# zalo/TetSim

Measured on AMD Instinct MI355X. Metric: tet_solves_per_sec, higher is better.
Workload: dtype f32; 1 GPU; Kuhn-6 cube lattice 55x55x55 cells (998250 tets, 175616 particles), polar-decomposition Jacobi, 20 substeps/frame, dt=1/1200 s; solver=polar_jacobi, arithmetic=fast, formulation=reference (rest shape carried from substep to substep, 148 B/tet), tets=998250, particles=175616, parallelism=single GPU

## Files before the change

### include/tetsim.h

```cpp
#ifndef TETSIM_H
#define TETSIM_H

#include <stdint.h>

#ifdef __cplusplus
extern "C" {
#endif

#define TETSIM_ABI_VERSION 5

typedef struct tetsim_body *tetsim_handle;

enum {
    TETSIM_OK = 0,
    TETSIM_EINVAL = 1,
    TETSIM_ENODEVICE = 2,
    TETSIM_EHIP = 3,
    TETSIM_ENOMEM = 4,
    TETSIM_ECOMM = 5,
    TETSIM_ESTATE = 6
};

enum {
    TETSIM_SOLVER_POLAR_JACOBI = 0,
// ... 170 lines not shown
int tetsim_set_body_params_device(tetsim_handle h, const void *rows, uint64_t row_stride, const void *body_mask, void *caller_stream);


enum { TETSIM_FIELD_POSITIONS = 0, TETSIM_FIELD_VELOCITIES = 1, TETSIM_FIELD_PREV_POSITIONS = 2,
       TETSIM_FIELD_QUATS = 3, TETSIM_FIELD_VISUAL_POSITIONS = 4, TETSIM_FIELD_VISUAL_NORMALS = 5,
       TETSIM_FIELD_VISUAL_VERTEX_NORMALS = 6 };
#define TETSIM_MAX_EXPORT_FIELDS 8
typedef struct TetSimDeviceField {
    int32_t field, reserved;
    void *dst;
    uint64_t row_stride;
} TetSimDeviceField;
int tetsim_export_device(tetsim_handle h, const TetSimDeviceField *fields, uint32_t count, void *consumer_stream);
int tetsim_import_device(tetsim_handle h, const void *pos, uint64_t pos_stride,
                         const void *vel, uint64_t vel_stride, void *producer_stream);


typedef struct tetsim_snapshot_s *tetsim_snapshot;
int tetsim_snapshot_create(tetsim_handle h, tetsim_snapshot *out);
int tetsim_snapshot_capture(tetsim_handle h, tetsim_snapshot s, const void *body_mask, void *caller_stream);
int tetsim_snapshot_restore(tetsim_handle h, tetsim_snapshot s, const void *body_mask, void *caller_stream);
void tetsim_snapshot_destroy(tetsim_snapshot s);


#define TETSIM_PLACE_WIDTH 16
enum { TETSIM_PLACE_Q = 0 , TETSIM_PLACE_PIVOT = 4 , TETSIM_PLACE_OFFSET = 7 ,
       TETSIM_PLACE_LINEAR = 10 , TETSIM_PLACE_ANGULAR = 13  };
enum { TETSIM_PLACE_KEEP_VELOCITY = 1u << 0 };
int tetsim_place_bodies_device(tetsim_handle h, const void *rows, uint64_t row_stride,
                               const void *body_mask, uint32_t flags, void *caller_stream);
int tetsim_place_bodies(tetsim_handle h, const float *rows, const uint8_t *body_mask, uint32_t flags);


#define TETSIM_OBS_WIDTH 20
enum { TETSIM_OBS_MASS = 0, TETSIM_OBS_COM = 1 , TETSIM_OBS_VCOM = 4 , TETSIM_OBS_VOLUME = 7,
       TETSIM_OBS_REST_VOLUME = 8, TETSIM_OBS_MIN_VOLUME_RATIO = 9, TETSIM_OBS_INVERTED_TETS = 10,
       TETSIM_OBS_AABB_MIN = 11 , TETSIM_OBS_AABB_MAX = 14 , TETSIM_OBS_MAX_SPEED2 = 17,
       TETSIM_OBS_NONFINITE = 18, TETSIM_OBS_RESERVED = 19  };
int tetsim_observe_bodies_device(tetsim_handle h, void *dst, uint64_t row_stride, void *caller_stream);
int tetsim_read_body_observations(tetsim_handle h, double *out);


#define TETSIM_POSE_WIDTH 48
#define TETSIM_POSE_SWEEPS 5
enum { TETSIM_POSE_MASS = 0, TETSIM_POSE_MX = 1 , TETSIM_POSE_MV = 4 , TETSIM_POSE_A = 7 ,
       TETSIM_POSE_L0 = 16 , TETSIM_POSE_G = 19 , TETSIM_POSE_Q0 = 25,
       TETSIM_POSE_COM = 26 , TETSIM_POSE_VCOM = 29 , TETSIM_POSE_Q = 32 , TETSIM_POSE_OMEGA = 36 ,
       TETSIM_POSE_L = 39 , TETSIM_POSE_RESIDUAL = 42, TETSIM_POSE_GAP = 43, TETSIM_POSE_RESERVED = 44  };
int tetsim_body_poses_device(tetsim_handle h, void *dst, uint64_t row_stride, void *caller_stream);
int tetsim_read_body_poses(tetsim_handle h, double *out);
int tetsim_prep_pose_table(const float *verts, uint32_t nv, const int32_t *tets, uint32_t nt,
                           const uint32_t *body_first_vert, const uint32_t *body_first_tet, uint32_t num_bodies,
                           double density, void *records_out, double *centres_out);


#define TETSIM_TOUCH_WIDTH 100
#define TETSIM_TOUCH_SLOT_WIDTH 12
#define TETSIM_TOUCH_PARTICLE_WIDTH 8
enum { TETSIM_TOUCH_TOUCHING = 0, TETSIM_TOUCH_MIN_SD = 1, TETSIM_TOUCH_MIN_SLOT = 2, TETSIM_TOUCH_SLOTS = 3,
       TETSIM_TOUCH_SLOT0 = 4  };
enum { TETSIM_TOUCH_SLOT_KIND = 0, TETSIM_TOUCH_SLOT_COUNT = 1, TETSIM_TOUCH_SLOT_MIN_SD = 2, TETSIM_TOUCH_SLOT_CENTROID = 3 ,
       TETSIM_TOUCH_SLOT_NORMAL = 6 , TETSIM_TOUCH_SLOT_REL_VEL = 9  };
enum { TETSIM_TOUCH_P_SD = 0, TETSIM_TOUCH_P_NORMAL = 1 , TETSIM_TOUCH_P_SLOT = 4, TETSIM_TOUCH_P_TOUCHES = 5,
       TETSIM_TOUCH_P_RESERVED = 6  };
int tetsim_touch_bodies_device(tetsim_handle h, double margin, void *dst, uint64_t row_stride, void *caller_stream);
int tetsim_read_body_touch(tetsim_handle h, double margin, double *out);
int tetsim_touch_particles_device(tetsim_handle h, double margin, void *dst, uint64_t row_stride, void *caller_stream);


#define TETSIM_RAY_INVALID (-1)
int tetsim_raycast_visual_device(tetsim_handle h,
        const void *rays,     uint64_t ray_stride,
        const void *ray_body,
        uint32_t count,
        void *hits,           uint64_t hit_stride,
        void *caller_stream);
int tetsim_visual_bounding_spheres_device(tetsim_handle h, void *dst, uint64_t row_stride, void *caller_stream);


int tetsim_raycast_visual_bvh_device(tetsim_handle h,
        const void *rays,     uint64_t ray_stride,
        const void *ray_body,
        uint32_t count,
        void *hits,           uint64_t hit_stride,
        void *caller_stream);


typedef struct TetSimPointQuery { double point[3], max_distance; } TetSimPointQuery;
typedef struct TetSimClosest    { int32_t found, body, triangle, region;
                                  double distance, point[3], v, w; } TetSimClosest;
#define TETSIM_CLOSEST_INVALID (-1)
int tetsim_closest_visual_device(tetsim_handle h,
        const void *queries,  uint64_t query_stride,
        const void *query_body,
        uint32_t count,
        void *out,            uint64_t out_stride,
        void *caller_stream);
int tetsim_closest_visual(tetsim_handle h, const TetSimPointQuery *queries, const int32_t *query_body, uint32_t count, TetSimClosest *out);


#define TETSIM_STRAIN_WIDTH 16
#define TETSIM_STRAIN_BODY_WIDTH 8
#define TETSIM_STRAIN_SWEEPS 4
enum { TETSIM_STRAIN_F = 0 , TETSIM_STRAIN_J = 9, TETSIM_STRAIN_DEV = 10,
       TETSIM_STRAIN_STRETCH = 11 , TETSIM_STRAIN_GREEN = 14, TETSIM_STRAIN_RESERVED = 15  };
int tetsim_tet_strain_device(tetsim_handle h, void *dst, uint64_t row_stride, void *caller_stream);
int tetsim_read_tet_strain(tetsim_handle h, float *out);
int tetsim_body_strain_device(tetsim_handle h, void *dst, uint64_t row_stride, void *caller_stream);
int tetsim_visual_strain_device(tetsim_handle h, int32_t channel, void *dst, uint64_t row_stride, void *caller_stream);
int tetsim_prep_strain_table(const float *verts, uint32_t nv, const int32_t *tets, uint32_t nt, double density, void *records_out);


int tetsim_profile(tetsim_handle h, uint32_t n, double dt, const TetSimParams *params, TetSimProfile *out);
int tetsim_time_kernels(tetsim_handle h, uint32_t reps, double dt, const TetSimParams *params, TetSimProfile *out);
int tetsim_time_step_n(tetsim_handle h, uint32_t n, double dt, const TetSimParams *params, double *ms_out);
int tetsim_measure_copy_bandwidth(int32_t device, uint64_t bytes, uint32_t reps, double *gbps_out);
int tetsim_measure_stream_bandwidth(int32_t device, uint64_t bytes, uint32_t reps, int32_t kind, double *gbps_out);


int tetsim_comm_unique_id(void *id128);
int tetsim_comm_init(tetsim_handle h, const void *id128, int32_t rank, int32_t nranks);
typedef struct TetSimCommInfo {
    int32_t rccl_ranks, rccl_rank;
    uint32_t neighbours;
    uint64_t send_bytes_per_substep, recv_bytes_per_substep, max_message_bytes;
    int32_t loopback;
    int32_t p2p;
} TetSimCommInfo;
int tetsim_comm_info(tetsim_handle h, TetSimCommInfo *out);
int tetsim_comm_selftest(tetsim_handle h);
int tetsim_comm_probe(tetsim_handle h, uint64_t bytes, uint32_t reps, int32_t use_graph, uint32_t per_graph,
                      double *host_us, double *total_us);
int tetsim_halo_probe(tetsim_handle h, uint32_t reps, double *min_us, double *median_us, double *max_us);
#define TETSIM_P2P_BLOB_BYTES 512
int tetsim_halo_p2p_export(tetsim_handle h, void *blob);
int tetsim_halo_p2p_connect(tetsim_handle h, const void *blobs, uint32_t count);
int tetsim_halo_p2p_probe(tetsim_handle h, uint32_t reps, double *min_us, double *median_us, double *max_us);
int tetsim_group_step_n(tetsim_handle *handles, uint32_t count, uint32_t n, double dt, const TetSimParams *params);
int tetsim_halo_exchange_local(tetsim_handle *handles, uint32_t count);
int tetsim_get_halo_plan(tetsim_handle h, int32_t *neigh ,
                         int32_t *send_counts, int32_t *recv_counts,
                         int32_t *send_ids, int32_t *recv_ids);
int tetsim_halo_export(tetsim_handle h, uint32_t n, float *out_xyzw);
int tetsim_halo_import(tetsim_handle h, uint32_t n, const float *in_xyzw);


int tetsim_prep_levels(const int32_t *tets, uint32_t nt, uint32_t nv, int32_t *level, uint32_t *num_levels);
int tetsim_prep_colours(const int32_t *tets, uint32_t nt, uint32_t nv, int32_t *colour, uint32_t *num_colours);
int tetsim_prep_clusters(const int32_t *tets, uint32_t nt, uint32_t nv, int32_t *order, int32_t *launch, int32_t *lane,
                         int32_t *step, uint32_t *num_launches, uint32_t *num_clusters);
int tetsim_prep_tiles(const float *verts, uint32_t nv, const int32_t *tets, uint32_t nt, const uint32_t *body_first_tet,
                      const uint32_t *body_first_vert, uint32_t bodies, int32_t *tile_tets, uint32_t *tile_off,
                      uint8_t *corner_slot, uint32_t *num_tiles);
int tetsim_prep_bvh(const float *positions, uint32_t nvis, const int32_t *tri_ids, uint32_t ntri, const int32_t *tri_body, uint32_t bodies,
                    uint32_t *tri_first, uint32_t *order, uint32_t *node_first, uint32_t *depth, uint32_t *node_range);
int tetsim_prep_slot_table(const int32_t *tets, uint32_t nt, uint32_t nv, int32_t ref_quirk,
                           int32_t *slots , uint32_t *dropped);
int tetsim_prep_call_tiles(const float *verts, uint32_t nv, const int32_t *tets, uint32_t nt, uint32_t sizes[4],
                           uint32_t *blk_vert_off, int32_t *blk_verts, uint32_t *vp_ell);
int tetsim_prep_call_schedule(const int32_t *blk_verts, const uint32_t *blk_vert_off, uint32_t nb, const uint32_t *vp_ell,
                              uint32_t vp_cols, uint32_t nv_pad, uint32_t nv_owned, uint32_t lag, uint32_t *entry,
                              uint32_t capacity, uint32_t *period, uint32_t *tail, int32_t *fell_back);
int tetsim_prep_check_call_schedule(const int32_t *blk_verts, const uint32_t *blk_vert_off, uint32_t nb, const uint32_t *vp_ell,
                                    uint32_t vp_cols, uint32_t nv_pad, uint32_t nv_owned, const uint32_t *entry, uint32_t period,
                                    uint32_t tail);
int tetsim_prep_ref_grab_texels(int32_t grab_id, uint32_t num_elems, uint32_t num_particles, int32_t out[2]);
int tetsim_prep_boundary_surface(const float *verts ,
                                 const int32_t *tets, uint32_t nt, uint32_t nv,
                                 float *vis_verts , int32_t *tri_ids ,
                                 uint32_t *nrows, uint32_t *ntri);
int tetsim_prep_rest(const float *verts, uint32_t nv, const int32_t *tets, uint32_t nt, double density,
                     float *inv_mass, float *inv_rest_pose, float *inv_rest_volume);

int tetsim_prep_partition(const float *verts , uint32_t nv, const int32_t *tets, uint32_t nt,
                          int32_t part_count, int32_t *vert_owner_out);
typedef struct TetSimPartQuality {
    uint32_t owned_particles;
    uint32_t ghost_particles;
    uint32_t boundary_particles;
    uint32_t local_elems;
    uint32_t owned_elems;
    uint32_t num_neighbours;
} TetSimPartQuality;
int tetsim_prep_partition_quality(const int32_t *tets, uint32_t nt, uint32_t nv, int32_t part_count,
                                  const int32_t *vert_owner, TetSimPartQuality *out);

typedef struct tetsim_plan_s *tetsim_plan;
typedef struct TetSimPlanSizes {
    uint32_t owned_particles, boundary_particles, local_particles, local_elems, owned_elems, num_neighbours;
} TetSimPlanSizes;
int tetsim_plan_create(const int32_t *tets, uint32_t nt, uint32_t nv, int32_t part_count, int32_t part_index,
                       const int32_t *vert_owner, tetsim_plan *out);
int tetsim_plan_create_deep(const int32_t *tets, uint32_t nt, uint32_t nv, int32_t part_count, int32_t part_index,
                            const int32_t *vert_owner, int32_t depth, tetsim_plan *out);
int tetsim_plan_layers(tetsim_plan p, uint32_t *first_layer_ghosts, uint8_t *tet_layer);
int tetsim_plan_neighbour_layer2(tetsim_plan p, uint32_t i, uint32_t *send_count, uint32_t *recv_start, uint32_t *recv_count);
int tetsim_plan_neighbour_layer2_ids(tetsim_plan p, uint32_t i, int32_t *send_local, int32_t *send_global, int32_t *recv_global);
void tetsim_plan_destroy(tetsim_plan p);
int tetsim_plan_sizes(tetsim_plan p, TetSimPlanSizes *out);
int tetsim_plan_arrays(tetsim_plan p, int32_t *local_to_global_vert, int32_t *local_to_global_tet, int32_t *local_tets);
int tetsim_plan_neighbour(tetsim_plan p, uint32_t i, int32_t *rank, uint32_t *send_count, uint32_t *recv_start,
                          uint32_t *recv_count, int32_t *send_is_contiguous);
int tetsim_plan_neighbour_ids(tetsim_plan p, uint32_t i, int32_t *send_local, int32_t *send_global, int32_t *recv_global);

int tetsim_abi_version(void);
typedef struct TetSimLibraryInfo {
    int32_t abi;
    int32_t ablation;
    uint32_t debug_env;
    char source_sha[20];
    char kernel_sha[20];
} TetSimLibraryInfo;
int tetsim_library_info(TetSimLibraryInfo *out);

typedef struct TetSimMeshArrays {
    uint32_t num_particles;
    uint32_t num_elems;
    uint32_t num_edges;
    uint32_t num_vis_verts;
    uint32_t num_vis_tris;
    uint32_t part_count;
    const float *verts;
    const int32_t *tets;
    const int32_t *edge_ids;
    const float *vis_verts;
    const int32_t *vis_tri_ids;
    const int32_t *tet_colour;
    const int32_t *vert_owner;
} TetSimMeshArrays;
typedef struct tetsim_mesh_file *tetsim_mesh;

int tetsim_mesh_write(const char *path, const TetSimMeshArrays *a);
int tetsim_mesh_open(const char *path, tetsim_mesh *out);
int tetsim_mesh_arrays(tetsim_mesh m, TetSimMeshArrays *out);
int tetsim_mesh_close(tetsim_mesh m);
int tetsim_create_from_file(const char *path, const TetSimOptions *opts, tetsim_handle *out);

#ifdef __cplusplus
}
#endif
#endif
```

### tetsim_amd/_capi.py

```python
import ctypes as C
import os

_HERE = os.path.dirname(os.path.abspath(__file__))
LIB_PATH = os.environ.get("TETSIM_HIP_LIB") or os.path.join(_HERE, "libtetsim_hip.so")

OK, EINVAL, ENODEVICE, EHIP, ENOMEM, ECOMM, ESTATE = range(7)
RAY_INVALID = -1
CLOSEST_INVALID = -1
SOLVER_POLAR_JACOBI, SOLVER_NEOHOOKEAN_GS = 0, 1
PRECISE, FAST = 0, 1
ORDER_ORIGINAL, ORDER_COLOURED, ORDER_CLUSTERED = 0, 1, 2
FLAG_REF_SLOT_TABLE, FLAG_REF_FIXED_BOUNDS, FLAG_GATHER_FORMULATION, FLAG_CONSTANT_REST_SHAPE, FLAG_REF_GRAB_TEXEL, FLAG_DEEP_GHOSTS = 1, 2, 4, 8, 16, 32
FLAG_REF_ROTATION_EXIT = 64
FLAG_LEAN_STATE = 128
K_TET, K_VERTEX, K_HALO, K_COUNT = 0, 1, 2, 3
COLLIDER_SPHERE, COLLIDER_CAPSULE, COLLIDER_BOX, COLLIDER_PLANE = 0, 1, 2, 3
MAX_COLLIDERS = 8
BODY_COLLIDER_FLOATS = 24
BODY_PARAMS_WIDTH = 10
BP_GRAVITY, BP_FRICTION, BP_DEV_COMPLIANCE, BP_VOL_COMPLIANCE, BP_BOUNDS_LO, BP_BOUNDS_HI = 0, 1, 2, 3, 4, 7
FIELD_POSITIONS, FIELD_VELOCITIES, FIELD_PREV_POSITIONS, FIELD_QUATS, FIELD_VISUAL_POSITIONS, FIELD_VISUAL_NORMALS, FIELD_VISUAL_VERTEX_NORMALS = range(7)
MAX_EXPORT_FIELDS = 8
OBS_WIDTH = 20
(OBS_MASS, OBS_COM, OBS_VCOM, OBS_VOLUME, OBS_REST_VOLUME, OBS_MIN_VOLUME_RATIO, OBS_INVERTED_TETS, OBS_AABB_MIN, OBS_AABB_MAX, OBS_MAX_SPEED2,
 OBS_NONFINITE, OBS_RESERVED) = 0, 1, 4, 7, 8, 9, 10, 11, 14, 17, 18, 19
POSE_WIDTH, POSE_SWEEPS = 48, 5
(POSE_MASS, POSE_MX, POSE_MV, POSE_A, POSE_L0, POSE_G, POSE_Q0, POSE_COM, POSE_VCOM, POSE_Q, POSE_OMEGA, POSE_L, POSE_RESIDUAL, POSE_GAP,
 POSE_RESERVED) = 0, 1, 4, 7, 16, 19, 25, 26, 29, 32, 36, 39, 42, 43, 44
TOUCH_WIDTH, TOUCH_SLOT_WIDTH, TOUCH_PARTICLE_WIDTH = 100, 12, 8
TOUCH_TOUCHING, TOUCH_MIN_SD, TOUCH_MIN_SLOT, TOUCH_SLOTS, TOUCH_SLOT0 = 0, 1, 2, 3, 4
TOUCH_SLOT_KIND, TOUCH_SLOT_COUNT, TOUCH_SLOT_MIN_SD, TOUCH_SLOT_CENTROID, TOUCH_SLOT_NORMAL, TOUCH_SLOT_REL_VEL = 0, 1, 2, 3, 6, 9
TOUCH_P_SD, TOUCH_P_NORMAL, TOUCH_P_SLOT, TOUCH_P_TOUCHES, TOUCH_P_RESERVED = 0, 1, 4, 5, 6
STRAIN_WIDTH, STRAIN_BODY_WIDTH, STRAIN_SWEEPS = 16, 8, 4
STRAIN_F, STRAIN_J, STRAIN_DEV, STRAIN_STRETCH, STRAIN_GREEN, STRAIN_RESERVED = 0, 9, 10, 11, 14, 15
PLACE_WIDTH = 16
PLACE_Q, PLACE_PIVOT, PLACE_OFFSET, PLACE_LINEAR, PLACE_ANGULAR = 0, 4, 7, 10, 13
PLACE_KEEP_VELOCITY = 1


class TetSimParams(C.Structure):
    _fields_ = [("gravity", C.c_double), ("friction", C.c_double), ("devCompliance", C.c_double),
                ("volCompliance", C.c_double), ("worldBounds", C.c_double * 6)]


class TetSimOptions(C.Structure):
    _fields_ = [("solver", C.c_int32), ("precision", C.c_int32), ("order", C.c_int32), ("flags", C.c_uint32),
                ("device", C.c_int32), ("density", C.c_double), ("part_count", C.c_int32),
                ("part_index", C.c_int32), ("vert_owner", C.POINTER(C.c_int32)), ("tet_colour", C.POINTER(C.c_int32))]


class TetSimMeshArrays(C.Structure):
    _fields_ = [("num_particles", C.c_uint32), ("num_elems", C.c_uint32), ("num_edges", C.c_uint32),
                ("num_vis_verts", C.c_uint32), ("num_vis_tris", C.c_uint32), ("part_count", C.c_uint32),
                ("verts", C.POINTER(C.c_float)), ("tets", C.POINTER(C.c_int32)), ("edge_ids", C.POINTER(C.c_int32)),
                ("vis_verts", C.POINTER(C.c_float)), ("vis_tri_ids", C.POINTER(C.c_int32)),
                ("tet_colour", C.POINTER(C.c_int32)), ("vert_owner", C.POINTER(C.c_int32))]


class TetSimInfo(C.Structure):
    _fields_ = [("num_particles", C.c_uint32), ("num_elems", C.c_uint32), ("owned_particles", C.c_uint32),
                ("local_particles", C.c_uint32), ("local_elems", C.c_uint32), ("owned_elems", C.c_uint32),
                ("num_levels", C.c_uint32), ("max_valence", C.c_uint32), ("dropped_slots", C.c_uint32),
                ("num_neighbours", C.c_uint32), ("device_bytes", C.c_uint64), ("solver", C.c_int32),
                ("precision", C.c_int32), ("order", C.c_int32), ("device", C.c_int32), ("flags", C.c_uint32),
                ("num_vis_verts", C.c_uint32), ("num_bodies", C.c_uint32), ("fused_particle_pass", C.c_uint32), ("total_vis_verts", C.c_uint32)]


class TetSimProfile(C.Structure):
    _fields_ = [("total_ms", C.c_double), ("kernel_ms", C.c_double * K_COUNT), ("launches", C.c_uint32 * K_COUNT),
                ("substeps", C.c_uint32), ("tets_per_tet_launch", C.c_uint32)]


class TetSimLibraryInfo(C.Structure):
    _fields_ = [("abi", C.c_int32), ("ablation", C.c_int32), ("debug_env", C.c_uint32), ("source_sha", C.c_char * 20),
                ("kernel_sha", C.c_char * 20)]


DEBUG_ENV_NAMES = ["TETSIM_DEBUG_LOOPBACK_HALO", "TETSIM_DEBUG_LOOPBACK_COPY", "TETSIM_DEBUG_ONE_STREAM", "TETSIM_DEBUG_GROUP_SYNC",
                   "TETSIM_DEBUG_HOSTPROF", "TETSIM_DEBUG_TRACE", "TETSIM_HALO_SYNC", "TETSIM_HALO_GRAPH", "TETSIM_DEBUG_LOOPBACK_DELAY_US", "TETSIM_NH_QUADS", "TETSIM_FUSED_PARTICLE_PASS",
                   "TETSIM_FRAME_KERNEL", "TETSIM_FRAME_LOCAL", "TETSIM_NH_FOLD", "TETSIM_HALO_ALIGNED_TILES", "TETSIM_HALO_FOLD_WAIT", "TETSIM_QUAD", "TETSIM_QUAD_POLL_DELAY", "TETSIM_NH_FRAME",
                   "TETSIM_NH_ONE_LAUNCH", "TETSIM_PJ_ONE_LAUNCH", "TETSIM_PJ_CALL_LAG"]


LAB_ENV_NAMES = ["TETSIM_DEBUG_TRACE", "TETSIM_NH_QUADS", "TETSIM_FRAME_LOCAL", "TETSIM_NH_FOLD", "TETSIM_HALO_ALIGNED_TILES", "TETSIM_QUAD_POLL_DELAY", "TETSIM_NH_FRAME"]


class TetSimCommInfo(C.Structure):
    _fields_ = [("rccl_ranks", C.c_int32), ("rccl_rank", C.c_int32), ("neighbours", C.c_uint32), ("send_bytes_per_substep", C.c_uint64),
                ("recv_bytes_per_substep", C.c_uint64), ("max_message_bytes", C.c_uint64), ("loopback", C.c_int32), ("p2p", C.c_int32)]


class TetSimPlanSizes(C.Structure):
    _fields_ = [("owned_particles", C.c_uint32), ("boundary_particles", C.c_uint32), ("local_particles", C.c_uint32),
                ("local_elems", C.c_uint32), ("owned_elems", C.c_uint32), ("num_neighbours", C.c_uint32)]


class TetSimPartQuality(C.Structure):
    _fields_ = [("owned_particles", C.c_uint32), ("ghost_particles", C.c_uint32), ("boundary_particles", C.c_uint32),
                ("local_elems", C.c_uint32), ("owned_elems", C.c_uint32), ("num_neighbours", C.c_uint32)]


class TetSimError(RuntimeError):
    def __init__(self, code, msg):
        super().__init__("tetsim error %d: %s" % (code, msg))
        self.code = code


class TetSimCollider(C.Structure):
    _fields_ = [("kind", C.c_int32), ("reserved", C.c_int32), ("a", C.c_double * 3), ("b", C.c_double * 3), ("axes", C.c_double * 9),
                ("radius", C.c_double), ("friction", C.c_double), ("velocity", C.c_double * 3)]


class TetSimRay(C.Structure):
    _fields_ = [("origin", C.c_double * 3), ("direction", C.c_double * 3), ("near", C.c_double), ("far", C.c_double)]


class TetSimRayHit(C.Structure):
    _fields_ = [("hit", C.c_int32), ("body", C.c_int32), ("triangle", C.c_int32), ("reserved", C.c_int32), ("distance", C.c_double),
                ("point", C.c_double * 3)]


class TetSimPointQuery(C.Structure):
    _fields_ = [("point", C.c_double * 3), ("max_distance", C.c_double)]


class TetSimClosest(C.Structure):
    _fields_ = [("found", C.c_int32), ("body", C.c_int32), ("triangle", C.c_int32), ("region", C.c_int32), ("distance", C.c_double),
                ("point", C.c_double * 3), ("v", C.c_double), ("w", C.c_double)]


class TetSimDeviceField(C.Structure):
    _fields_ = [("field", C.c_int32), ("reserved", C.c_int32), ("dst", C.c_void_p), ("row_stride", C.c_uint64)]


SYMBOLS = [
    "tetsim_abi_version", "tetsim_default_options", "tetsim_default_params", "tetsim_create", "tetsim_create_batch", "tetsim_get_batch_layout", "tetsim_destroy",
    "tetsim_last_error", "tetsim_get_info", "tetsim_step", "tetsim_step_n", "tetsim_sync",
    "tetsim_library_info", "tetsim_read_quats_pinned", "tetsim_state_size", "tetsim_save_state", "tetsim_load_state",
    "tetsim_read_positions", "tetsim_read_positions_pinned", "tetsim_read_prev_positions", "tetsim_read_velocities", "tetsim_read_quats",
    "tetsim_read_vol_error", "tetsim_write_state", "tetsim_get_owned_ids", "tetsim_get_local_tets",
    "tetsim_get_tet_order", "tetsim_get_level_offsets", "tetsim_read_inv_mass", "tetsim_set_visual_mesh", "tetsim_get_visual_ids", "tetsim_halo_refresh_final", "tetsim_group_refresh_final", "tetsim_halo_probe", "tetsim_halo_p2p_probe",
    "tetsim_read_visual_mesh", "tetsim_set_visual_triangles", "tetsim_read_visual_vertex_normals", "tetsim_visual_vertex_normals_from", "tetsim_group_read_visual_vertex_normals", "tetsim_set_grab", "tetsim_set_colliders",
    "tetsim_start_grab", "tetsim_nearest_particle", "tetsim_profile", "tetsim_time_kernels", "tetsim_time_step_n", "tetsim_measure_copy_bandwidth", "tetsim_measure_stream_bandwidth",
    "tetsim_comm_unique_id", "tetsim_comm_init", "tetsim_comm_info", "tetsim_comm_selftest", "tetsim_comm_probe", "tetsim_group_step_n", "tetsim_halo_exchange_local", "tetsim_get_halo_plan",
    "tetsim_halo_p2p_export", "tetsim_halo_p2p_connect",
    "tetsim_halo_export", "tetsim_halo_import", "tetsim_prep_levels", "tetsim_prep_colours", "tetsim_prep_clusters",
    "tetsim_prep_tiles", "tetsim_prep_slot_table", "tetsim_prep_call_tiles", "tetsim_prep_call_schedule", "tetsim_prep_check_call_schedule", "tetsim_prep_ref_grab_texels", "tetsim_prep_rest", "tetsim_prep_partition", "tetsim_prep_partition_quality", "tetsim_plan_create", "tetsim_plan_destroy", "tetsim_plan_sizes",
    "tetsim_plan_arrays", "tetsim_plan_neighbour", "tetsim_plan_neighbour_ids",
    "tetsim_plan_create_deep", "tetsim_plan_layers", "tetsim_plan_neighbour_layer2", "tetsim_plan_neighbour_layer2_ids",
    "tetsim_raycast_visual", "tetsim_start_grab_ray", "tetsim_read_visual_bounding_sphere", "tetsim_prep_boundary_surface",
    "tetsim_export_device", "tetsim_import_device",
    "tetsim_snapshot_create", "tetsim_snapshot_capture", "tetsim_snapshot_restore", "tetsim_snapshot_destroy",
    "tetsim_observe_bodies_device", "tetsim_read_body_observations",
    "tetsim_body_poses_device", "tetsim_read_body_poses", "tetsim_prep_pose_table",
    "tetsim_touch_bodies_device", "tetsim_read_body_touch", "tetsim_touch_particles_device",
    "tetsim_raycast_visual_device", "tetsim_visual_bounding_spheres_device", "tetsim_raycast_visual_bvh_device", "tetsim_prep_bvh",
    "tetsim_closest_visual_device", "tetsim_closest_visual",
    "tetsim_tet_strain_device", "tetsim_read_tet_strain", "tetsim_body_strain_device", "tetsim_visual_strain_device", "tetsim_prep_strain_table",
    "tetsim_set_body_grabs", "tetsim_set_body_grabs_device", "tetsim_nearest_particles_device",
    "tetsim_set_body_colliders", "tetsim_set_body_colliders_device",
    "tetsim_set_body_params", "tetsim_set_body_params_device",
    "tetsim_place_bodies_device", "tetsim_place_bodies",
    "tetsim_mesh_write", "tetsim_mesh_open", "tetsim_mesh_arrays", "tetsim_mesh_close", "tetsim_create_from_file",
]

OPTIONAL_SYMBOLS = ("tetsim_set_colliders", "tetsim_raycast_visual", "tetsim_start_grab_ray", "tetsim_read_visual_bounding_sphere", "tetsim_prep_boundary_surface",
                    "tetsim_export_device", "tetsim_import_device",
                    "tetsim_snapshot_create", "tetsim_snapshot_capture", "tetsim_snapshot_restore", "tetsim_snapshot_destroy",
                    "tetsim_observe_bodies_device", "tetsim_read_body_observations",
                    "tetsim_raycast_visual_device", "tetsim_visual_bounding_spheres_device",
                    "tetsim_tet_strain_device", "tetsim_read_tet_strain", "tetsim_body_strain_device", "tetsim_visual_strain_device", "tetsim_prep_strain_table",
                    "tetsim_set_body_grabs", "tetsim_set_body_grabs_device", "tetsim_nearest_particles_device",
                    "tetsim_set_body_colliders", "tetsim_set_body_colliders_device",
                    "tetsim_set_body_params", "tetsim_set_body_params_device",
                    "tetsim_place_bodies_device", "tetsim_place_bodies",
                    "tetsim_body_poses_device", "tetsim_read_body_poses", "tetsim_prep_pose_table",
                    "tetsim_raycast_visual_bvh_device", "tetsim_prep_bvh",
                    "tetsim_closest_visual_device", "tetsim_closest_visual",
                    "tetsim_touch_bodies_device", "tetsim_read_body_touch", "tetsim_touch_particles_device")

_lib = None


def lib():
    global _lib
    if _lib is not None:
        return _lib
    if not os.path.exists(LIB_PATH):
        raise ImportError("libtetsim_hip.so is not built: run `python -m tetsim_amd.build` "
                          "(the HIP extension is mandatory; there is no CPU fallback)")
    L = C.CDLL(LIB_PATH)
    H, fp, ip, dp = C.c_void_p, C.POINTER(C.c_float), C.POINTER(C.c_int32), C.POINTER(C.c_double)
    u32, i32, dbl = C.c_uint32, C.c_int32, C.c_double
    PP = C.POINTER(TetSimParams)
    L.tetsim_abi_version.restype = C.c_int
    L.tetsim_default_options.argtypes = [C.POINTER(TetSimOptions)]
    L.tetsim_default_options.restype = None
    L.tetsim_default_params.argtypes = [PP]
    L.tetsim_default_params.restype = None
    L.tetsim_create.argtypes = [fp, u32, ip, u32, C.POINTER(TetSimOptions), C.POINTER(H)]
    L.tetsim_create_batch.argtypes = [C.POINTER(fp), C.POINTER(u32), C.POINTER(ip), C.POINTER(u32), u32, C.POINTER(TetSimOptions), C.POINTER(H)]
    L.tetsim_get_batch_layout.argtypes = [H, C.POINTER(u32), C.POINTER(u32)]
    L.tetsim_destroy.argtypes = [H]
    L.tetsim_destroy.restype = None
    L.tetsim_comm_probe.argtypes = [H, C.c_uint64, u32, i32, u32, dp, dp]
    L.tetsim_nearest_particle.argtypes = [H, fp, ip, dp]
    L.tetsim_mesh_write.argtypes = [C.c_char_p, C.POINTER(TetSimMeshArrays)]
    L.tetsim_mesh_open.argtypes = [C.c_char_p, C.POINTER(H)]
    L.tetsim_mesh_arrays.argtypes = [H, C.POINTER(TetSimMeshArrays)]
    L.tetsim_mesh_close.argtypes = [H]
    L.tetsim_create_from_file.argtypes = [C.c_char_p, C.POINTER(TetSimOptions), C.POINTER(H)]
    L.tetsim_last_error.argtypes = [H]
    L.tetsim_last_error.restype = C.c_char_p
    L.tetsim_get_info.argtypes = [H, C.POINTER(TetSimInfo)]
    L.tetsim_step.argtypes = [H, dbl, PP]
    L.tetsim_step_n.argtypes = [H, u32, dbl, PP]
    L.tetsim_sync.argtypes = [H]
    for n in ("positions", "prev_positions", "velocities", "quats", "inv_mass"):
        getattr(L, "tetsim_read_" + n).argtypes = [H, fp]
    L.tetsim_read_positions_pinned.argtypes = [H, C.POINTER(fp)]
    L.tetsim_read_quats_pinned.argtypes = [H, C.POINTER(fp)]
    L.tetsim_library_info.argtypes = [C.POINTER(TetSimLibraryInfo)]
    L.tetsim_state_size.argtypes = [H, C.POINTER(C.c_uint64)]
    L.tetsim_save_state.argtypes = [H, C.c_void_p, C.c_uint64]
    L.tetsim_load_state.argtypes = [H, C.c_void_p, C.c_uint64]
    L.tetsim_read_vol_error.argtypes = [H, dp]
    L.tetsim_write_state.argtypes = [H, fp, fp]
    for n in ("owned_ids", "local_tets", "tet_order", "level_offsets"):
        getattr(L, "tetsim_get_" + n).argtypes = [H, ip]
    L.tetsim_set_visual_mesh.argtypes = [H, fp, u32, fp]
    L.tetsim_read_visual_mesh.argtypes = [H, fp, fp]
    L.tetsim_get_visual_ids.argtypes = [H, C.POINTER(C.c_int32)]
    L.tetsim_halo_refresh_final.argtypes = [H]
    L.tetsim_halo_probe.argtypes = [H, u32, C.POINTER(C.c_double), C.POINTER(C.c_double), C.POINTER(C.c_double)]
    L.tetsim_halo_p2p_probe.argtypes = [H, u32, C.POINTER(C.c_double), C.POINTER(C.c_double), C.POINTER(C.c_double)]
    L.tetsim_group_refresh_final.argtypes = [C.POINTER(H), u32]
    L.tetsim_set_visual_triangles.argtypes = [H, ip, u32]
    L.tetsim_read_visual_vertex_normals.argtypes = [H, fp]
    L.tetsim_visual_vertex_normals_from.argtypes = [H, fp, fp]
    L.tetsim_group_read_visual_vertex_normals.argtypes = [C.POINTER(H), u32, fp, fp]
    L.tetsim_set_grab.argtypes = [H, i32, fp]
    if hasattr(L, "tetsim_set_colliders"):
        L.tetsim_set_colliders.argtypes = [H, C.POINTER(TetSimCollider), u32]
    L.tetsim_start_grab.argtypes = [H, fp, ip]
    if hasattr(L, "tetsim_raycast_visual"):
        L.tetsim_raycast_visual.argtypes = [H, C.c_void_p, u32, C.c_void_p]
        L.tetsim_start_grab_ray.argtypes = [H, C.POINTER(TetSimRay), C.POINTER(TetSimRayHit), ip]
        L.tetsim_read_visual_bounding_sphere.argtypes = [H, dp, dp]
        L.tetsim_prep_boundary_surface.argtypes = [fp, ip, u32, u32, fp, ip, C.POINTER(u32), C.POINTER(u32)]
    if hasattr(L, "tetsim_export_device"):
        L.tetsim_export_device.argtypes = [H, C.POINTER(TetSimDeviceField), u32, C.c_void_p]
        L.tetsim_import_device.argtypes = [H, C.c_void_p, C.c_uint64, C.c_void_p, C.c_uint64, C.c_void_p]
    if hasattr(L, "tetsim_snapshot_create"):
        L.tetsim_snapshot_create.argtypes = [H, C.POINTER(H)]
        L.tetsim_snapshot_capture.argtypes = [H, H, C.c_void_p, C.c_void_p]
        L.tetsim_snapshot_restore.argtypes = [H, H, C.c_void_p, C.c_void_p]
        L.tetsim_snapshot_destroy.argtypes = [H]
        L.tetsim_snapshot_destroy.restype = None
    if hasattr(L, "tetsim_observe_bodies_device"):
        L.tetsim_observe_bodies_device.argtypes = [H, C.c_void_p, C.c_uint64, C.c_void_p]
        L.tetsim_read_body_observations.argtypes = [H, dp]
    if hasattr(L, "tetsim_raycast_visual_device"):
        L.tetsim_raycast_visual_device.argtypes = [H, C.c_void_p, C.c_uint64, C.c_void_p, u32, C.c_void_p, C.c_uint64, C.c_void_p]
        L.tetsim_visual_bounding_spheres_device.argtypes = [H, C.c_void_p, C.c_uint64, C.c_void_p]
    if hasattr(L, "tetsim_raycast_visual_bvh_device"):
        L.tetsim_raycast_visual_bvh_device.argtypes = [H, C.c_void_p, C.c_uint64, C.c_void_p, u32, C.c_void_p, C.c_uint64, C.c_void_p]
        L.tetsim_prep_bvh.argtypes = [fp, u32, ip, u32, ip, u32] + [C.POINTER(u32)] * 5
    if hasattr(L, "tetsim_closest_visual_device"):
        L.tetsim_closest_visual_device.argtypes = [H, C.c_void_p, C.c_uint64, C.c_void_p, u32, C.c_void_p, C.c_uint64, C.c_void_p]
        L.tetsim_closest_visual.argtypes = [H, C.c_void_p, C.c_void_p, u32, C.c_void_p]
    if hasattr(L, "tetsim_tet_strain_device"):
        L.tetsim_tet_strain_device.argtypes = [H, C.c_void_p, C.c_uint64, C.c_void_p]
        L.tetsim_read_tet_strain.argtypes = [H, fp]
        L.tetsim_body_strain_device.argtypes = [H, C.c_void_p, C.c_uint64, C.c_void_p]
        L.tetsim_visual_strain_device.argtypes = [H, i32, C.c_void_p, C.c_uint64, C.c_void_p]
        L.tetsim_prep_strain_table.argtypes = [fp, u32, ip, u32, dbl, C.c_void_p]
    if hasattr(L, "tetsim_set_body_grabs"):
        L.tetsim_set_body_grabs.argtypes = [H, ip, fp]
        L.tetsim_set_body_grabs_device.argtypes = [H, C.c_void_p, C.c_void_p, C.c_uint64, C.c_void_p, C.c_void_p]
        L.tetsim_nearest_particles_device.argtypes = [H, C.c_void_p, C.c_uint64, C.c_void_p, C.c_void_p, C.c_void_p]
    if hasattr(L, "tetsim_set_body_colliders"):
        L.tetsim_set_body_colliders.argtypes = [H, fp, u32]
        L.tetsim_set_body_colliders_device.argtypes = [H, C.c_void_p, C.c_uint64, u32, C.c_void_p, C.c_void_p]
    if hasattr(L, "tetsim_set_body_params"):
        L.tetsim_set_body_params.argtypes = [H, C.POINTER(C.c_double)]
        L.tetsim_set_body_params_device.argtypes = [H, C.c_void_p, C.c_uint64, C.c_void_p, C.c_void_p]
    if hasattr(L, "tetsim_place_bodies_device"):
        L.tetsim_place_bodies_device.argtypes = [H, C.c_void_p, C.c_uint64, C.c_void_p, u32, C.c_void_p]
        L.tetsim_place_bodies.argtypes = [H, fp, C.POINTER(C.c_uint8), u32]
    if hasattr(L, "tetsim_body_poses_device"):
        L.tetsim_body_poses_device.argtypes = [H, C.c_void_p, C.c_uint64, C.c_void_p]
        L.tetsim_read_body_poses.argtypes = [H, dp]
        L.tetsim_prep_pose_table.argtypes = [fp, u32, ip, u32, C.POINTER(u32), C.POINTER(u32), u32, dbl, C.c_void_p, dp]
    if hasattr(L, "tetsim_touch_bodies_device"):
        L.tetsim_touch_bodies_device.argtypes = [H, dbl, C.c_void_p, C.c_uint64, C.c_void_p]
        L.tetsim_read_body_touch.argtypes = [H, dbl, dp]
        L.tetsim_touch_particles_device.argtypes = [H, dbl, C.c_void_p, C.c_uint64, C.c_void_p]
    L.tetsim_profile.argtypes = [H, u32, dbl, PP, C.POINTER(TetSimProfile)]
    L.tetsim_time_kernels.argtypes = [H, u32, dbl, PP, C.POINTER(TetSimProfile)]
    L.tetsim_time_step_n.argtypes = [H, u32, dbl, PP, dp]
    L.tetsim_measure_copy_bandwidth.argtypes = [i32, C.c_uint64, u32, dp]
    L.tetsim_measure_stream_bandwidth.argtypes = [i32, C.c_uint64, u32, i32, dp]
    L.tetsim_comm_unique_id.argtypes = [C.c_void_p]
    L.tetsim_comm_init.argtypes = [H, C.c_void_p, i32, i32]
    L.tetsim_comm_selftest.argtypes = [H]
    L.tetsim_comm_info.argtypes = [H, C.POINTER(TetSimCommInfo)]
    L.tetsim_group_step_n.argtypes = [C.POINTER(H), u32, u32, dbl, PP]
    L.tetsim_halo_exchange_local.argtypes = [C.POINTER(H), u32]
    L.tetsim_halo_p2p_export.argtypes = [H, C.c_void_p]
    L.tetsim_halo_p2p_connect.argtypes = [H, C.c_void_p, u32]
    L.tetsim_get_halo_plan.argtypes = [H, ip, ip, ip, ip, ip]
    L.tetsim_halo_export.argtypes = [H, u32, fp]
    L.tetsim_halo_import.argtypes = [H, u32, fp]
    L.tetsim_prep_levels.argtypes = [ip, u32, u32, ip, C.POINTER(u32)]
    L.tetsim_prep_colours.argtypes = [ip, u32, u32, ip, C.POINTER(u32)]
    L.tetsim_prep_clusters.argtypes = [ip, u32, u32, ip, ip, ip, ip, C.POINTER(u32), C.POINTER(u32)]
    L.tetsim_prep_tiles.argtypes = [fp, u32, ip, u32, C.POINTER(u32), C.POINTER(u32), u32, ip, C.POINTER(u32), C.POINTER(C.c_uint8), C.POINTER(u32)]
    L.tetsim_prep_slot_table.argtypes = [ip, u32, u32, i32, ip, C.POINTER(u32)]
    up = C.POINTER(u32)
    L.tetsim_prep_call_tiles.argtypes = [fp, u32, ip, u32, up, up, ip, up]
    L.tetsim_prep_call_schedule.argtypes = [ip, up, u32, up, u32, u32, u32, u32, up, u32, up, up, ip]
    L.tetsim_prep_check_call_schedule.argtypes = [ip, up, u32, up, u32, u32, u32, up, u32, u32]
    L.tetsim_prep_ref_grab_texels.argtypes = [i32, u32, u32, ip]
    L.tetsim_prep_rest.argtypes = [fp, u32, ip, u32, dbl, fp, fp, fp]
    L.tetsim_prep_partition.argtypes = [fp, u32, ip, u32, i32, ip]
    L.tetsim_prep_partition_quality.argtypes = [ip, u32, u32, i32, ip, C.POINTER(TetSimPartQuality)]
    L.tetsim_plan_create.argtypes = [ip, u32, u32, i32, i32, ip, C.POINTER(H)]
    L.tetsim_plan_destroy.argtypes = [H]
    L.tetsim_plan_destroy.restype = None
    L.tetsim_plan_sizes.argtypes = [H, C.POINTER(TetSimPlanSizes)]
    L.tetsim_plan_arrays.argtypes = [H, ip, ip, ip]
    L.tetsim_plan_neighbour.argtypes = [H, u32, ip, C.POINTER(u32), C.POINTER(u32), C.POINTER(u32), ip]
    L.tetsim_plan_neighbour_ids.argtypes = [H, u32, ip, ip, ip]
    L.tetsim_plan_create_deep.argtypes = [ip, u32, u32, i32, i32, ip, i32, C.POINTER(H)]
    L.tetsim_plan_layers.argtypes = [H, C.POINTER(u32), C.POINTER(C.c_uint8)]
    L.tetsim_plan_neighbour_layer2.argtypes = [H, u32, C.POINTER(u32), C.POINTER(u32), C.POINTER(u32)]
    L.tetsim_plan_neighbour_layer2_ids.argtypes = [H, u32, ip, ip, ip]
    for s in SYMBOLS:
        if s in OPTIONAL_SYMBOLS and not hasattr(L, s):
            continue
        f = getattr(L, s)
        if s not in ("tetsim_default_options", "tetsim_default_params", "tetsim_destroy", "tetsim_last_error",
                     "tetsim_plan_destroy", "tetsim_snapshot_destroy"):
            f.restype = C.c_int
    _lib = L
    return L


def library_info():
    li = TetSimLibraryInfo()
    check(lib().tetsim_library_info(C.byref(li)))
    return {"abi": li.abi, "ablation": bool(li.ablation), "source_sha": li.source_sha.decode(), "kernel_sha": li.kernel_sha.decode(),
            "debug_env": [n for i, n in enumerate(DEBUG_ENV_NAMES) if li.debug_env >> i & 1], "path": LIB_PATH}


def check(rc, handle=None):
    if rc != OK:
        msg = lib().tetsim_last_error(handle)
        raise TetSimError(rc, msg.decode("utf-8", "replace") if msg else "")
```

### tetsim_amd/csrc/dev_common.h

```cpp
#pragma once
#include <hip/hip_ext.h>
#include <hip/hip_runtime.h>

#include "host_prep.h"

#include <cstddef>
#include <cstdint>

namespace tetsim {

constexpr uint32_t kMaxColliders = 8;
struct DevColliderF {
    float a[3], b[3], u[9], radius, friction, v[3];
    int32_t kind, pad;
};
struct DevColliderD {
    double a[3], b[3], u[9], radius, friction, v[3];
    int32_t kind, pad;
};

__host__ __device__ inline float ref_fixed_lo(int c) { return c == 1 ? -1.0f : -2.5f; }
__host__ __device__ inline float ref_fixed_hi(int c) { return c == 1 ? 10.0f : 2.5f; }
struct BodyParamsF { float gravity, friction, dev_compliance, vol_compliance, lo[3], hi[3], pad[2]; };
struct BodyParamsD { double gravity, friction, dev_compliance, vol_compliance, lo[3], hi[3]; };
static_assert(sizeof(BodyParamsF) == 48 && sizeof(BodyParamsD) == 80, "body parameter rows");

struct DevParams {
    float dt, gravity, friction;
    uint32_t body_grabs;
    float lo[3];
    uint32_t body_colliders;
    float hi[3];
    uint32_t body_params;
    float grab[3];
    int32_t grab_local;
    int32_t grab_local2;
    uint32_t epoch;
    int32_t poll_delay;
    uint32_t n_colliders;
    double d_dt, d_gravity, d_friction, d_dev_compliance, d_vol_compliance;
    double d_lo[3], d_hi[3];
    const uint32_t* grab_body;
    const int4* grab_rows;
    const uint32_t* bcol_count;
    const DevColliderF* bcol_f;
    const DevColliderD* bcol_d;
    const BodyParamsF* bp_f;
    const BodyParamsD* bp_d;
    const uint32_t* tet_body;
    DevColliderF col[kMaxColliders];
    DevColliderD d_col[kMaxColliders];
};
constexpr size_t kDevParamsHead = offsetof(DevParams, col);
static_assert(kDevParamsHead % 8 == 0 && offsetof(DevParams, d_col) % 8 == 0, "DevParams layout");
constexpr size_t kKernelArgLimit = 4096;
static_assert(sizeof(DevParams) <= 2560, "DevParams must leave room for the other by-value arguments of a launch");
__device__ __forceinline__ void store_params(DevParams* dst, const DevParams& v) {
    const uint2* s = reinterpret_cast<const uint2*>(&v);
    uint2* d = reinterpret_cast<uint2*>(dst);
#pragma unroll
    for (size_t i = 0; i < kDevParamsHead / 8; i++) d[i] = s[i];
    for (uint32_t k = 0; k < v.n_colliders && k < kMaxColliders; k++) { dst->col[k] = v.col[k]; dst->d_col[k] = v.d_col[k]; }
}

__device__ __forceinline__ void body_grab_pick(const DevParams& P, uint32_t v, bool& held, float& x, float& y, float& z) {
    if (P.body_grabs) {
        const int4 row = P.grab_rows[P.grab_body[v]];
        held = row.x == static_cast<int32_t>(v);
        if (held) { x = __int_as_float(row.y); y = __int_as_float(row.z); z = __int_as_float(row.w); }
    }
}
__device__ __forceinline__ uint32_t body_colliders_body(const DevParams& P, uint32_t v) { return P.body_colliders ? P.grab_body[v] : 0u; }
__device__ __forceinline__ void body_colliders_pick(const DevParams& P, uint32_t body, const DevColliderF** list, uint32_t* count) {
    *list = P.col; *count = P.n_colliders;
    if (P.body_colliders) { *list = P.bcol_f + static_cast<size_t>(body) * kMaxColliders; *count = P.bcol_count[body]; }
}
__device__ __forceinline__ void body_colliders_pick(const DevParams& P, uint32_t body, const DevColliderD** list, uint32_t* count) {
    *list = P.d_col; *count = P.n_colliders;
    if (P.body_colliders) { *list = P.bcol_d + static_cast<size_t>(body) * kMaxColliders; *count = P.bcol_count[body]; }
}

__device__ __forceinline__ const BodyParamsF* body_params_row(const DevParams& P, uint32_t body, float) { return P.bp_f + body; }
__device__ __forceinline__ const BodyParamsD* body_params_row(const DevParams& P, uint32_t body, double) { return P.bp_d + body; }
__device__ __forceinline__ uint32_t body_params_uniform(uint32_t body) { return static_cast<uint32_t>(__builtin_amdgcn_readfirstlane(static_cast<int32_t>(body))); }
struct PolarBodyParams { float gravity, friction, lo[3], hi[3]; };
template <bool kUniform>
__device__ __forceinline__ PolarBodyParams body_params_polar(const DevParams& P, uint32_t v) {
    PolarBodyParams o = {P.gravity, P.friction, {P.lo[0], P.lo[1], P.lo[2]}, {P.hi[0], P.hi[1], P.hi[2]}};
    if (P.body_params) {
        uint32_t body = P.grab_body[v];
        if constexpr (kUniform) body = body_params_uniform(body);
        const BodyParamsF* const r = body_params_row(P, body, 0.0f);
        o.gravity = r->gravity; o.friction = r->friction;
        for (int k = 0; k < 3; k++) { o.lo[k] = r->lo[k]; o.hi[k] = r->hi[k]; }
    }
    return o;
}

struct PJDev {
    uint32_t nv_local = 0, nv_owned = 0, nv_boundary = 0, nt = 0;
    uint32_t nt_pad = 0;
    uint32_t nv_pad = 0;
    uint32_t max_valence = 0;
    float4* pos_pred = nullptr;
    float4* pos_final = nullptr;
    float4* vel = nullptr;
    int4* tet_idx = nullptr;
    float4* elem = nullptr;
    float4* quat = nullptr;
    int32_t* slot_tab = nullptr;
    uint32_t* slot_cnt = nullptr;
    const DevParams* params = nullptr;
    float rot_exit_w2 = 1.0e-18f;
};

struct PJBlk {
    uint32_t nb = 0, nb_interior = 0, nt = 0, nv_local = 0, nv_owned = 0, nv_boundary = 0;
    const uint32_t* blk_tet_off = nullptr;
    const uint32_t* blk_vert_off = nullptr;
    const int32_t* blk_verts = nullptr;
    const uchar4* tet_lidx = nullptr;
    float4* rest_a = nullptr;
    float4* rest_b = nullptr;
    float4* rest_c = nullptr;
    float* rest_c1 = nullptr;
    const float* vol = nullptr;
    float4* quat = nullptr;
    const uint32_t* lc_range = nullptr;
    const uint2* lc_ent = nullptr;
    float4* partial = nullptr;
    const float* wsum = nullptr;
    const uint32_t* vp_ell = nullptr;
    uint32_t vp_cols = 0, nv_pad = 0;
    float4* pos_pred = nullptr;
    float4* pos_final = nullptr;
    float4* vel = nullptr;
    const float4* partial_prev = nullptr;
    const float4* fin_in = nullptr;
    float4* fin_out = nullptr;
    const uint32_t* slot_src = nullptr;
    const uint32_t* blk_maxsrc = nullptr;
    uint32_t ns_pad = 0;
    const DevParams* params = nullptr;
    const float4* ghost_alt = nullptr;
    const float4* ghost2 = nullptr;
    uint32_t n_ghost1 = 0xffffffffu;
    bool lean = false;
    bool lean_state = false;
    float rot_exit_w2 = 1.0e-18f;
    uint32_t epoch = 0;
    unsigned long long* trace = nullptr;
    unsigned long long* iter_hist = nullptr;
};

struct NHDev {
    uint32_t nv = 0, nt = 0;
    float4* pos = nullptr;
    float4* prev = nullptr;
    float4* vel = nullptr;
    int4* tet_idx = nullptr;
    float4* irp_a = nullptr;
    float4* irp_b = nullptr;
    float4* irp_c = nullptr;
    double* vol_err = nullptr;
    int32_t* order = nullptr;
    uint32_t* corner_slots = nullptr;
    const DevParams* params = nullptr;
};
constexpr uint32_t max_grid_blocks(uint32_t threads) { return 0xffffffffu / threads; }
struct PJCallSched { const uint32_t* entry = nullptr; uint32_t period = 0, tail = 0; };
constexpr uint32_t pjb_call_chunk(uint32_t period, uint32_t tail, uint32_t threads, uint32_t cap) {
    const uint32_t room = max_grid_blocks(threads) > tail ? max_grid_blocks(threads) - tail : 0u;
    const uint32_t fit = period ? room / period : cap;
    return fit < 1u ? 1u : fit < cap ? fit : cap;
}
constexpr uint32_t nh_call_blocks_per_sub(uint32_t blocks) { return (blocks + 7u) & ~7u; }
constexpr uint32_t call_chunk(uint32_t per_sub, uint32_t threads, uint32_t cap) {
    const uint32_t fit = per_sub ? max_grid_blocks(threads) / per_sub : cap;
    return fit < 1u ? 1u : fit < cap ? fit : cap;
}
static_assert(pjb_call_chunk(pjb_call_blocks_per_sub(2282u, 103823u, 256u), 0u, 256u, 8192u) == 6223u, "46-cell lattice: 2,696 blocks per substep");
static_assert(pjb_call_chunk(pjb_call_blocks_per_sub(2282u, 103823u, 256u), 2696u, 256u, 8192u) == 6222u, "... and a tail of a whole period takes one substep's room");
static_assert(call_chunk(nh_call_blocks_per_sub(2601u), 256u, 65000u / 8u) == 6432u, "55-cell lattice, clustered: 2,608 blocks per substep");

constexpr uint32_t kNHClusterVerts = 8, kNHClusterTets = 8;
struct NHClusterLaunch {
    uint32_t nsteps = 0, clusters = 0;
    uint32_t first[kNHClusterTets] = {}, count[kNHClusterTets] = {};
    const int32_t* slot_vid = nullptr;
    const uint8_t* first_mask = nullptr;
};

struct NHSweepColour {
    NHClusterLaunch L;
    const float* slot_im = nullptr;
    const uint2* delta = nullptr;
    const uint8_t* last_mask = nullptr;
    const uint2* delta_first = nullptr;
    uint32_t first_block = 0;
    uint32_t pad = 0;
};
struct NHSweep {
    const NHSweepColour* colours = nullptr;
    uint32_t ncolours = 0, blocks = 0;
    float4* exchange = nullptr;
    uint32_t* error = nullptr;
    uint32_t timeout_ms = 0;
};
void nh_launch_sweep1_fast(hipStream_t s, const NHDev& d, const NHSweep& w, bool fold, uint32_t sub_index, uint32_t epoch);
void nh_launch_call_fast(hipStream_t s, const NHDev& d, const NHSweep& w, uint32_t n);

void pj_launch_tet_precise(hipStream_t s, const PJDev& d, hipEvent_t e0 = nullptr, hipEvent_t e1 = nullptr);
void pj_launch_tet_fast(hipStream_t s, const PJDev& d, hipEvent_t e0 = nullptr, hipEvent_t e1 = nullptr);
void pj_launch_vertex_precise(hipStream_t s, const PJDev& d, uint32_t first, uint32_t count, hipEvent_t e0 = nullptr, hipEvent_t e1 = nullptr);
void pj_launch_vertex_fast(hipStream_t s, const PJDev& d, uint32_t first, uint32_t count, hipEvent_t e0 = nullptr, hipEvent_t e1 = nullptr);
void pj_launch_repredict_precise(hipStream_t s, const PJDev& d);
void pj_launch_repredict_fast(hipStream_t s, const PJDev& d);

void nh_launch_post_predict_precise(hipStream_t s, const NHDev& d);
void nh_launch_post_predict_fast(hipStream_t s, const NHDev& d);
void nh_launch_cluster_precise(hipStream_t s, const NHDev& d, const NHClusterLaunch& L, bool fold = false);
void nh_launch_cluster_fast(hipStream_t s, const NHDev& d, const NHClusterLaunch& L, bool fold = false);
struct NHFrameLaunch {
    const uint32_t* seg = nullptr;
    const uint32_t* first_vert = nullptr;
    uint32_t levels = 0, bodies = 0, block = 512;
    uint32_t max_body_particles = 0;
};
void nh_launch_frame_precise(hipStream_t s, const NHDev& d, const NHFrameLaunch& f, uint32_t n, const DevParams& params, DevParams* params_dev);
void nh_launch_frame_fast(hipStream_t s, const NHDev& d, const NHFrameLaunch& f, uint32_t n, const DevParams& params, DevParams* params_dev);
constexpr uint32_t kNHQuadLevelFast = 128, kNHQuadLevelPrecise = 64;
void nh_launch_level4_fast(hipStream_t s, const NHDev& d, uint32_t first, uint32_t count);
void nh_launch_level4_precise(hipStream_t s, const NHDev& d, uint32_t first, uint32_t count);
uint32_t nh_frame_lds_limit_precise();
uint32_t nh_frame_lds_limit_fast();
void nh_launch_post_predict_list_precise(hipStream_t s, const NHDev& d, const uint32_t* list, uint32_t n);
void nh_launch_post_predict_list_fast(hipStream_t s, const NHDev& d, const uint32_t* list, uint32_t n);
void pjb_launch_tet(hipStream_t s, const PJBlk& d, uint32_t tile_first, uint32_t tile_count, hipEvent_t e0 = nullptr,
                    hipEvent_t e1 = nullptr, uint32_t* raise_word = nullptr, uint32_t* clear_word = nullptr);
void pjb_launch_call(hipStream_t s, const PJBlk& d, const PJCallSched& sched, uint32_t n, uint32_t* err, uint32_t timeout_ms, const DevParams& params, DevParams* params_dev);
void pjb_launch_tet_fused(hipStream_t s, const PJBlk& d, hipEvent_t e0 = nullptr, hipEvent_t e1 = nullptr);
void pjb_launch_vertex(hipStream_t s, const PJBlk& d, uint32_t first, uint32_t count, hipEvent_t e0 = nullptr, hipEvent_t e1 = nullptr,
                       uint32_t* raise_word = nullptr, uint32_t* clear_word = nullptr);
void pjb_launch_repredict(hipStream_t s, const PJBlk& d);
void pjb_launch_recover_quats(hipStream_t s, const PJBlk& d, const float4* rest0_a, const float4* rest0_b, const float4* rest0_c);
void pjb_launch_frame(hipStream_t s, const PJBlk& d, uint32_t n, const int32_t* block_tile, uint32_t blocks, bool local, float4* pbuf0, float4* pbuf1,
                      uint32_t* err, uint32_t timeout_ms, const DevParams& params, DevParams* params_dev, hipEvent_t e0 = nullptr, hipEvent_t e1 = nullptr);
void pjq_launch_frame(hipStream_t s, const PJBlk& d, uint32_t n, const int32_t* block_tile, uint32_t blocks, bool local, float4* pbuf0, float4* pbuf1,
                      uint32_t* err, uint32_t timeout_ms, const DevParams& params, DevParams* params_dev, hipEvent_t e0 = nullptr, hipEvent_t e1 = nullptr);
void pjq_launch_tet(hipStream_t s, const PJBlk& d, hipEvent_t e0 = nullptr, hipEvent_t e1 = nullptr);
void pjq_launch_vertex(hipStream_t s, const PJBlk& d, hipEvent_t e0 = nullptr, hipEvent_t e1 = nullptr);
uint32_t pjq_frame_capacity(uint32_t* compute_units);
uint32_t pjb_frame_capacity(int mode, uint32_t* compute_units);
void pjb_wait_capacity(int mode, uint32_t* vertex_waves, uint32_t* hwait_blocks);
inline int pjb_mode(const PJBlk& d) { return d.lean ? 1 : d.lean_state ? 2 : 0; }
uint32_t pjb_probe_xcd(hipStream_t s, uint32_t blocks);
struct PJSync {
    uint32_t* flag = nullptr;
    uint32_t* error = nullptr;
    uint32_t timeout_ms = 0;
};
constexpr uint32_t kMaxPeers = 8;
struct PJPeer {
    float4* ghost[kMaxPeers] = {};
    const uint32_t* slots = nullptr;
    uint32_t cols = 0, stride = 0, n = 0;
    float4* fin[kMaxPeers] = {};
    float4* ghost2[kMaxPeers] = {};
    const uint32_t* slots2 = nullptr;
    uint32_t cols2 = 0;
};
struct PJPeerSync {
    uint32_t* raise[kMaxPeers] = {};
    uint32_t* wait[kMaxPeers] = {};
    uint32_t n_raise = 0, n_wait = 0;
    uint32_t delay_us = 0;
};
void pjb_launch_wait(hipStream_t s, const PJSync& y);
void pjb_launch_wait_peers(hipStream_t s, const PJSync& y, const PJPeerSync& w);
struct PJClear { uint32_t* word[kMaxPeers + 1] = {}; uint32_t n = 0; };
void pjb_launch_vertex_peer(hipStream_t s, const PJBlk& d, uint32_t first, uint32_t count, const PJPeer& peer, uint32_t* raise_word, const PJClear& clr = PJClear());
void pjb_launch_tet_hwait(hipStream_t s, const PJBlk& d, uint32_t tile_first, uint32_t tile_count, const PJSync& yv, const PJPeerSync& w, const float4* ghosts);
// ... 66 lines not shown
```

### tetsim_amd/csrc/host_prep.cpp

```cpp
#include "host_prep.h"

#include <algorithm>
#include <cmath>
#include <numeric>

namespace tetsim {

namespace {
inline float fround(double x) { return static_cast<float>(x); }

inline void edge_matrix(const float* verts, const int32_t* t, float m[9]) {
    for (int k = 0; k < 3; k++)
        for (int c = 0; c < 3; c++)
            m[3 * k + c] = fround(static_cast<double>(verts[3 * t[k + 1] + c]) - static_cast<double>(verts[3 * t[0] + c]));
}
inline double det3(const float* A) {
    double a11 = A[0], a12 = A[3], a13 = A[6];
    double a21 = A[1], a22 = A[4], a23 = A[7];
    double a31 = A[2], a32 = A[5], a33 = A[8];
    return a11 * a22 * a33 + a12 * a23 * a31 + a13 * a21 * a32 - a13 * a22 * a31 - a12 * a21 * a33 - a11 * a23 * a32;
}
}

void prep_rest(const float* verts, uint32_t nv, const int32_t* tets, uint32_t nt, double density,
// ... 237 lines not shown
            kept++;
        }
    inc.dropped = static_cast<uint32_t>(4ull * nt - kept);
    return inc;
}

uint32_t prep_slot_table(const int32_t* tets, uint32_t nt, uint32_t nv, bool ref_quirk, int32_t* slots) {
    std::fill(slots, slots + static_cast<size_t>(nv) * kRefSlots, -1);
    uint32_t dropped = 0;
    for (uint32_t e = 0; e < nt; e++)
        for (int k = 0; k < 4; k++) {
            int32_t* row = &slots[static_cast<size_t>(tets[4 * e + k]) * kRefSlots];
            bool placed = false;
            for (int s = 0; s < kRefSlots; s++) {
                const bool empty = ref_quirk ? (row[s] <= 0) : (row[s] < 0);
                if (empty) {
                    if (row[s] == 0) dropped++;
                    row[s] = static_cast<int32_t>(4 * e + k);
                    placed = true;
                    break;
                }
            }
            if (!placed) dropped++;
        }
    return dropped;
}

namespace {
inline uint32_t spread3(uint32_t x) {
    x &= 0x3ffu;
    x = (x | (x << 16)) & 0x030000ffu;
    x = (x | (x << 8)) & 0x0300f00fu;
    x = (x | (x << 4)) & 0x030c30c3u;
    x = (x | (x << 2)) & 0x09249249u;
    return x;
}
}

namespace {
struct Quantiser {
    float lo[3], inv;
    Quantiser(const float* xyz, uint32_t n) {
        float hi[3] = {-1e30f, -1e30f, -1e30f};
        lo[0] = lo[1] = lo[2] = 1e30f;
        for (uint32_t v = 0; v < n; v++)
            for (int c = 0; c < 3; c++) { lo[c] = std::min(lo[c], xyz[3 * v + c]); hi[c] = std::max(hi[c], xyz[3 * v + c]); }
        float ext = 1e-30f;
        for (int c = 0; c < 3; c++) ext = std::max(ext, hi[c] - lo[c]);
        inv = 1024.0f / ext;
    }
    uint32_t code(float x, float y, float z) const {
        const float p[3] = {x, y, z};
        uint32_t c = 0;
        for (int a = 0; a < 3; a++) {
            const uint32_t qv = static_cast<uint32_t>(std::min(1023.0f, std::max(0.0f, (p[a] - lo[a]) * inv)));
            c |= spread3(qv) << a;
        }
        return c;
    }
};
}

std::vector<uint32_t> morton_vertex_order(const float* xyz, uint32_t n, uint32_t first, uint32_t count) {
    std::vector<uint32_t> order(n);
    std::iota(order.begin(), order.end(), 0u);
    if (count < 2) return order;
    const Quantiser Q(xyz, n);
    std::vector<uint64_t> key(count);
    for (uint32_t i = 0; i < count; i++) {
        const uint32_t v = first + i;
        key[i] = (static_cast<uint64_t>(Q.code(xyz[3 * v], xyz[3 * v + 1], xyz[3 * v + 2])) << 32) | v;
    }
    std::sort(key.begin(), key.end());
    for (uint32_t i = 0; i < count; i++) order[first + i] = static_cast<uint32_t>(key[i] & 0xffffffffu);
    return order;
}

void build_blocks(const float* verts, const int32_t* tets, uint32_t nt, uint32_t nv, uint32_t nv_sum,
                  const Incidence& inc, BlockPlan* out, const uint32_t* body_first_tet, const uint32_t* body_first_vert, uint32_t bodies,
                  uint32_t nv_boundary, const uint8_t* tet_class, uint32_t nv_owned, uint32_t tile) {
    BlockPlan& B = *out;
    B = BlockPlan();
    B.tile = tile;
    if (nv_owned > nv_sum) nv_owned = nv_sum;
    const uint32_t kMaxTets = tile, kMaxVerts = tile;
    const uint32_t one_t[2] = {0u, nt}, one_v[2] = {0u, nv};
    if (!body_first_tet || !body_first_vert || bodies == 0) { body_first_tet = one_t; body_first_vert = one_v; bodies = 1; }
    std::vector<uint64_t> key(nt);
    std::vector<uint32_t> body_of_pos(nt);
    B.tet_perm.resize(nt);
    for (uint32_t b = 0; b < bodies; b++) {
        const uint32_t tb = body_first_tet[b], te = body_first_tet[b + 1], vb = body_first_vert[b], ve = body_first_vert[b + 1];
        const Quantiser Q(verts + 3ull * vb, ve - vb);
        for (uint32_t e = tb; e < te; e++) {
            float m[3] = {0.0f, 0.0f, 0.0f};
            for (int k = 0; k < 4; k++)
                for (int c = 0; c < 3; c++) m[c] += verts[3 * tets[4 * e + k] + c];
            key[e] = (static_cast<uint64_t>(Q.code(0.25f * m[0], 0.25f * m[1], 0.25f * m[2])) << 32) | (e - tb);
            if (tet_class) key[e] |= static_cast<uint64_t>(tet_class[e] & 3u) << 62;
        }
        std::sort(key.begin() + tb, key.begin() + te);
        for (uint32_t i = tb; i < te; i++) { B.tet_perm[i] = static_cast<int32_t>(tb + (key[i] & 0xffffffffu)); body_of_pos[i] = b; }
    }

    std::vector<uint8_t> live(4ull * nt, 0);
    for (int32_t enc : inc.slot) live[enc] = 1;

    std::vector<int32_t> slot_of(nv, -1);
    std::vector<int32_t> touched;
    struct Run { uint32_t begin, end; bool ghost; uint8_t cls; };
    auto cls_of = [&](uint32_t sorted_pos) -> uint8_t { return tet_class ? tet_class[B.tet_perm[sorted_pos]] : 0; };
    std::vector<Run> runs;
    {
        uint32_t i = 0;
        while (i < nt) {
            const uint32_t t0 = i;
            touched.clear();
            bool ghost = false;
            while (i < nt && i - t0 < kMaxTets && body_of_pos[i] == body_of_pos[t0] && cls_of(i) == cls_of(t0)) {
                const int32_t* t = &tets[4 * B.tet_perm[i]];
                uint32_t fresh = 0;
                for (int k = 0; k < 4; k++) {
                    bool seen = slot_of[t[k]] >= 0;
                    for (int j = 0; j < k && !seen; j++) seen = t[j] == t[k];
                    if (!seen) fresh++;
                }
                if (touched.size() + fresh > kMaxVerts) break;
                for (int k = 0; k < 4; k++)
                    if (slot_of[t[k]] < 0) {
                        slot_of[t[k]] = 0; touched.push_back(t[k]);
                        ghost |= static_cast<uint32_t>(t[k]) >= nv_owned || static_cast<uint32_t>(t[k]) < nv_boundary;
                    }
                i++;
            }
            for (int32_t v : touched) slot_of[v] = -1;
            runs.push_back({t0, i, ghost, cls_of(t0)});
        }
    }
    std::stable_sort(runs.begin(), runs.end(), [](const Run& a, const Run& b) { return a.cls != b.cls ? a.cls < b.cls : a.ghost < b.ghost; });
    {
        std::vector<int32_t> perm2(nt);
        uint32_t o = 0;
        for (Run& r : runs) {
            std::copy(B.tet_perm.begin() + r.begin, B.tet_perm.begin() + r.end, perm2.begin() + o);
            const uint32_t len = r.end - r.begin;
            r.begin = o; r.end = o + len;
            o += len;
        }
        B.tet_perm.swap(perm2);
    }

    B.tet_lidx.resize(4ull * nt);
    B.lc_ent.resize(4ull * nt);
    B.blk_tet_off.push_back(0);
    B.blk_vert_off.push_back(0);
    std::vector<std::vector<uint32_t>> vert_partials(nv_sum);
    std::vector<std::vector<uint32_t>> vert_staged(nv_sum);
    for (const Run& r : runs) {
        const uint32_t t0 = r.begin, i = r.end;
        if (!r.ghost && r.cls == 0) B.num_interior_blocks++;
        if (r.cls <= 1) B.num_first_blocks++;
        touched.clear();
        for (uint32_t j = t0; j < i; j++)
            for (int k = 0; k < 4; k++) {
                const int32_t v = tets[4 * B.tet_perm[j] + k];
                if (slot_of[v] < 0) { slot_of[v] = 0; touched.push_back(v); }
            }
        std::sort(touched.begin(), touched.end());
        for (size_t u = 0; u < touched.size(); u++) slot_of[touched[u]] = static_cast<int32_t>(u);
        for (uint32_t j = t0; j < i; j++)
            for (int k = 0; k < 4; k++) B.tet_lidx[4ull * j + k] = static_cast<uint8_t>(slot_of[tets[4 * B.tet_perm[j] + k]]);
        const uint32_t ntb = i - t0, nu = static_cast<uint32_t>(touched.size());
        const uint32_t v0 = B.blk_vert_off.back();
        std::vector<uint32_t> cnt(nu + 1, 0);
        for (uint32_t j = 0; j < ntb; j++)
            for (int k = 0; k < 4; k++)
                if (live[4ull * B.tet_perm[t0 + j] + k]) cnt[B.tet_lidx[4ull * (t0 + j) + k] + 1]++;
        for (uint32_t u = 0; u < nu; u++) cnt[u + 1] += cnt[u];
        for (uint32_t u = 0; u < nu; u++) B.lc_range.push_back(cnt[u] | (cnt[u + 1] << 16));
        std::vector<uint32_t> fillp(cnt.begin(), cnt.end() - 1);
        for (uint32_t j = 0; j < ntb; j++)
            for (int k = 0; k < 4; k++)
                if (live[4ull * B.tet_perm[t0 + j] + k]) {
                    const uint32_t u = B.tet_lidx[4ull * (t0 + j) + k];
                    B.lc_ent[4ull * t0 + fillp[u]++] = static_cast<uint16_t>(kMaxTets * k + j);
                }
        for (uint32_t u = 0; u < nu; u++) {
            const int32_t v = touched[u];
            B.blk_verts.push_back(v);
            if (static_cast<uint32_t>(v) < nv_sum && cnt[u + 1] > cnt[u]) vert_partials[v].push_back(v0 + u);
            else if (static_cast<uint32_t>(v) < nv_sum) vert_staged[v].push_back(v0 + u);
            slot_of[v] = -1;
        }
        B.blk_tet_off.push_back(i);
        B.blk_vert_off.push_back(v0 + nu);
        B.max_tile_verts = std::max(B.max_tile_verts, nu);
    }
    B.num_blocks = static_cast<uint32_t>(B.blk_tet_off.size() - 1);
    B.vp_off.assign(nv_sum + 1, 0);
    for (uint32_t v = 0; v < nv_sum; v++) {
        B.vp_off[v + 1] = B.vp_off[v] + static_cast<uint32_t>(vert_partials[v].size());
        B.max_partials = std::max<uint32_t>(B.max_partials, static_cast<uint32_t>(vert_partials[v].size()));
    }
    B.vp_idx.reserve(B.vp_off[nv_sum]);
    for (uint32_t v = 0; v < nv_sum; v++) B.vp_idx.insert(B.vp_idx.end(), vert_partials[v].begin(), vert_partials[v].end());
    B.nv_pad = (nv_sum + 63u) & ~63u;
    B.vp_cols = 0;
    for (uint32_t v = 0; v < nv_sum; v++) B.vp_cols = std::max<uint32_t>(B.vp_cols, static_cast<uint32_t>(vert_partials[v].size() + vert_staged[v].size()));
    B.vp_ell.assign(static_cast<size_t>(std::max(B.vp_cols, 1u)) * B.nv_pad, 0xffffffffu);
    for (uint32_t v = 0; v < nv_sum; v++) {
        const size_t live = vert_partials[v].size();
        for (size_t j = 0; j < live; j++) B.vp_ell[j * B.nv_pad + v] = vert_partials[v][j];
        for (size_t j = 0; j < vert_staged[v].size(); j++) B.vp_ell[(live + j) * B.nv_pad + v] = vert_staged[v][j];
    }
    const uint32_t ns = static_cast<uint32_t>(B.blk_verts.size());
    B.ns_pad = (ns + 63u) & ~63u;
    B.slot_src.assign(static_cast<size_t>(std::max(B.max_partials, 1u)) * B.ns_pad, 0xffffffffu);
    B.blk_maxsrc.assign(B.num_blocks, 0);
    for (uint32_t v = 0; v < nv_sum; v++)
        if (vert_partials[v].empty()) B.every_owned_particle_has_a_partial = false;
    for (uint32_t b = 0; b < B.num_blocks; b++)
        for (uint32_t g = B.blk_vert_off[b]; g < B.blk_vert_off[b + 1]; g++) {
            const uint32_t v = static_cast<uint32_t>(B.blk_verts[g]);
            if (v >= nv_sum) continue;
            const std::vector<uint32_t>& list = vert_partials[v];
            for (size_t j = 0; j < list.size(); j++) B.slot_src[j * B.ns_pad + g] = list[j];
            B.blk_maxsrc[b] = std::max<uint32_t>(B.blk_maxsrc[b], static_cast<uint32_t>(list.size()));
            if (!list.empty() && list[0] == g) B.lc_range[g] |= 1u << 15;
        }
}

namespace {
struct SchedDeps {
    uint32_t per_xcd = 0, tet_blocks = 0, npb = 0, plain_period = 0;
    std::vector<std::vector<uint32_t>> tiles_of_pb, pbs_of_tile;
};
SchedDeps sched_deps(const int32_t* blk_verts, const uint32_t* blk_vert_off, uint32_t nb, const uint32_t* vp_ell, uint32_t vp_cols, uint32_t nv_pad,
                     uint32_t nv_owned, uint32_t tile) {
    SchedDeps D;
    D.per_xcd = (nb + 7u) / 8u; D.tet_blocks = D.per_xcd * 8u; D.npb = (nv_owned + tile - 1u) / tile;
    D.plain_period = pjb_call_blocks_per_sub(nb, nv_owned, tile);
    D.tiles_of_pb.resize(D.npb); D.pbs_of_tile.resize(nb);
    for (uint32_t v = 0; v < nv_owned; v++)
        for (uint32_t j = 0; j < vp_cols; j++) {
            const uint32_t idx = vp_ell[static_cast<size_t>(j) * nv_pad + v];
            if (idx == 0xffffffffu) continue;
            const uint32_t b = static_cast<uint32_t>(std::upper_bound(blk_vert_off, blk_vert_off + nb + 1, idx) - blk_vert_off) - 1u;
            if (b < nb) D.tiles_of_pb[v / tile].push_back(b);
        }
    for (uint32_t b = 0; b < nb; b++)
        for (uint32_t g = blk_vert_off[b]; g < blk_vert_off[b + 1]; g++)
            if (static_cast<uint32_t>(blk_verts[g]) < nv_owned) D.pbs_of_tile[b].push_back(static_cast<uint32_t>(blk_verts[g]) / tile);
    auto uniq = [](std::vector<uint32_t>& v) { std::sort(v.begin(), v.end()); v.erase(std::unique(v.begin(), v.end()), v.end()); };
    for (auto& v : D.tiles_of_pb) uniq(v);
    for (auto& v : D.pbs_of_tile) uniq(v);
    return D;
}
inline uint32_t sched_tile_of(uint32_t r, uint32_t per_xcd) { return (r & 7u) * per_xcd + (r >> 3); }
void sched_plain(const SchedDeps& D, uint32_t nb, CallSchedule* out) {
    out->period = D.plain_period;
    out->tail = 0; out->lag = 0;
    out->entry.assign(out->period, sched_entry(kSchedEmpty, 0));
    for (uint32_t r = 0; r < D.tet_blocks; r++)
        if (sched_tile_of(r, D.per_xcd) < nb) out->entry[r] = sched_entry(kSchedTile, r);
    for (uint32_t k = 0; k < D.npb; k++) out->entry[D.tet_blocks + k] = sched_entry(kSchedParticles, k);
}
struct SchedPass { std::vector<uint32_t> entry, ready, left; uint32_t head_end = 0; bool stuck = false; };
SchedPass sched_pass(const SchedDeps& D, uint32_t nb, uint32_t lag, const std::vector<uint32_t>& head_at) {
    constexpr uint32_t none = 0xffffffffu;
    SchedPass R;
    R.ready.assign(D.npb, none);
    std::vector<uint32_t> need(D.npb), head, queue;
    std::vector<uint8_t> head_placed(D.npb, 0);
    for (uint32_t k = 0; k < D.npb; k++) {
        need[k] = static_cast<uint32_t>(D.tiles_of_pb[k].size());
        if (head_at[k] != none) head.push_back(k);
        if (need[k] == 0) { R.ready[k] = 0; if (head_at[k] == none) queue.push_back(k); }
    }
    std::stable_sort(head.begin(), head.end(), [&](uint32_t a, uint32_t b) { return head_at[a] < head_at[b]; });
    std::vector<std::vector<uint32_t>> pbs_by_tile(nb);
    for (uint32_t k = 0; k < D.npb; k++) for (uint32_t b : D.tiles_of_pb[k]) pbs_by_tile[b].push_back(k);
    size_t hi = 0, qi = 0;
    uint32_t col_next[8] = {}, tiles_left = D.tet_blocks;
    const uint64_t limit = 4ull * (D.tet_blocks + D.npb) + 64ull * (static_cast<uint64_t>(lag) + 1ull) + 64ull;
    for (uint32_t p = 0;; p++) {
        if (tiles_left == 0 && hi == head.size() && (p & 7u) == 0u) break;
        if (p >= limit) { R.stuck = true; break; }
        const uint32_t x = p & 7u;
        if (hi < head.size() && head_at[head[hi]] <= p) {
            const uint32_t k = head[hi++];
            R.entry.push_back(sched_entry(kSchedParticles, k, true));
            head_placed[k] = 1; R.head_end = p + 1u;
            continue;
        }
        if (qi < queue.size() && R.ready[queue[qi]] <= p) { R.entry.push_back(sched_entry(kSchedParticles, queue[qi++])); continue; }
        if (col_next[x] < D.per_xcd) {
            const uint32_t r = 8u * col_next[x] + x, b = sched_tile_of(r, D.per_xcd);
            bool held = false;
            if (b < nb) for (uint32_t k : D.pbs_of_tile[b]) held = held || (head_at[k] != none && !head_placed[k]);
            if (!held) {
                col_next[x]++; tiles_left--;
                R.entry.push_back(b < nb ? sched_entry(kSchedTile, r) : sched_entry(kSchedEmpty, 0));
                if (b < nb) for (uint32_t k : pbs_by_tile[b])
                    if (--need[k] == 0) { R.ready[k] = p + 8u * lag; if (head_at[k] == none) queue.push_back(k); }
                continue;
            }
        }
        R.entry.push_back(sched_entry(kSchedEmpty, 0));
    }
    R.left.assign(queue.begin() + static_cast<std::ptrdiff_t>(qi), queue.end());
    return R;
}
}

std::string check_call_schedule(const int32_t* blk_verts, const uint32_t* blk_vert_off, uint32_t nb, const uint32_t* vp_ell, uint32_t vp_cols,
                                uint32_t nv_pad, uint32_t nv_owned, const uint32_t* entry, uint32_t period, uint32_t tail, uint32_t tile) {
    constexpr uint32_t none = 0xffffffffu;
    const SchedDeps D = sched_deps(blk_verts, blk_vert_off, nb, vp_ell, vp_cols, nv_pad, nv_owned, tile);
    if (period == 0 || period % 8u != 0u) return "the period is not a positive multiple of 8";
    if (period < D.plain_period) return "the period is shorter than a substep's blocks";
    std::vector<uint64_t> at_tile(nb, none), at_pb(D.npb, none);
    uint32_t col_seen[8] = {}, wrapped_end = 0;
    for (uint32_t p = 0; p < period; p++) {
        const uint32_t kind = entry[p] >> 30, index = entry[p] & kSchedIndexMask;
        const bool wrapped = (entry[p] & kSchedWrapped) != 0u;
        if (kind == kSchedEmpty) continue;
        if (kind == kSchedTile) {
            const uint32_t b = sched_tile_of(index, D.per_xcd);
            if (index >= D.tet_blocks || b >= nb) return "entry " + std::to_string(p) + " names a tile that does not exist";
            if ((index & 7u) != (p & 7u)) return "tile block " + std::to_string(index) + " is not on its XCD";
            if (wrapped) return "tile block " + std::to_string(index) + " is wrapped";
            if ((index >> 3) < col_seen[p & 7u]) return "tile block " + std::to_string(index) + " is out of its XCD's order";
            col_seen[p & 7u] = (index >> 3) + 1u;
            if (at_tile[b] != none) return "tile " + std::to_string(b) + " appears twice";
            at_tile[b] = p;
        } else if (kind == kSchedParticles) {
            if (index >= D.npb) return "entry " + std::to_string(p) + " names a particle block that does not exist";
            if (at_pb[index] != none) return "particle block " + std::to_string(index) + " appears twice";
            at_pb[index] = static_cast<uint64_t>(p) + (wrapped ? period : 0u);
            if (wrapped) wrapped_end = p + 1u;
        } else return "entry " + std::to_string(p) + " has no kind";
    }
    for (uint32_t b = 0; b < nb; b++) if (at_tile[b] == none) return "tile " + std::to_string(b) + " is missing";
    for (uint32_t k = 0; k < D.npb; k++) if (at_pb[k] == none) return "particle block " + std::to_string(k) + " is missing";
    if (tail < wrapped_end || tail > period) return "the tail does not cover the wrapped entries";
    for (uint32_t k = 0; k < D.npb; k++)
        for (uint32_t b : D.tiles_of_pb[k])
            if (!(at_tile[b] < at_pb[k])) return "particle block " + std::to_string(k) + " does not follow tile " + std::to_string(b) + " of its lists";
    for (uint32_t b = 0; b < nb; b++)
        for (uint32_t k : D.pbs_of_tile[b])
            if (!(at_pb[k] < at_tile[b] + period)) return "tile " + std::to_string(b) + " of the next substep does not follow particle block " + std::to_string(k);
    return "";
}

void build_call_schedule(const int32_t* blk_verts, const uint32_t* blk_vert_off, uint32_t nb, const uint32_t* vp_ell, uint32_t vp_cols,
                         uint32_t nv_pad, uint32_t nv_owned, uint32_t lag, CallSchedule* out, uint32_t tile) {
    constexpr uint32_t none = 0xffffffffu;
    const SchedDeps D = sched_deps(blk_verts, blk_vert_off, nb, vp_ell, vp_cols, nv_pad, nv_owned, tile);
    *out = CallSchedule();
    auto plain = [&](const std::string& why) {
        sched_plain(D, nb, out);
        out->fell_back = !why.empty(); out->why = why;
    };
    if (lag == 0 || nb == 0) return plain("");
    if (static_cast<uint64_t>(lag) * 8u >= D.plain_period) return plain("lag " + std::to_string(lag) + ": a whole substep or more");
    std::vector<uint32_t> head_at(D.npb, none);
    SchedPass R;
    bool settled = false;
    for (int pass = 0; pass < 64 && !settled; pass++) {
        R = sched_pass(D, nb, lag, head_at);
        if (R.stuck) return plain("lag " + std::to_string(lag) + ": the layout does not close");
        const uint32_t period = static_cast<uint32_t>(R.entry.size());
        settled = R.left.empty();
        for (uint32_t k : R.left) head_at[k] = 0;
        for (uint32_t k = 0; k < D.npb; k++)
            if (head_at[k] != none && !settled) head_at[k] = R.ready[k] != none && R.ready[k] > period ? R.ready[k] - period : 0u;
    }
    if (!settled) return plain("lag " + std::to_string(lag) + ": the wrapped blocks do not settle");
    out->entry = R.entry;
    out->period = static_cast<uint32_t>(R.entry.size());
    out->tail = R.head_end;
// ... 138 lines not shown
```

### tetsim_amd/csrc/host_prep.h

```cpp
#pragma once
#include <cstdint>
#include <string>
#include <vector>

namespace tetsim {

constexpr int kRefSlots = 36;

void prep_rest(const float* verts, uint32_t nv, const int32_t* tets, uint32_t nt, double density,
               float* inv_mass, float* inv_rest_pose, float* inv_rest_volume);

float pj_inv_rest_volume(const float* verts, const int32_t* tet);

uint32_t prep_levels(const int32_t* tets, uint32_t nt, uint32_t nv, int32_t* level);
uint32_t prep_colours(const int32_t* tets, uint32_t nt, uint32_t nv, int32_t* colour);
constexpr uint32_t kClusterTets = 8, kClusterVerts = 8;
struct ClusterPlan {
    std::vector<int32_t> pre;
    std::vector<uint32_t> exec_pos;
    std::vector<uint32_t> corner_slots;
    std::vector<uint32_t> launch_off;
    std::vector<uint32_t> step_off;
    std::vector<uint32_t> step_first, step_count;
    std::vector<uint32_t> vid_off;
    std::vector<int32_t> slot_vid;
    uint32_t num_clusters = 0;
};
ClusterPlan prep_clusters(const int32_t* tets, uint32_t nt, uint32_t nv);
uint32_t prep_slot_table(const int32_t* tets, uint32_t nt, uint32_t nv, bool ref_quirk, int32_t* slots);

struct Incidence {
    std::vector<uint32_t> offset;
    std::vector<int32_t> slot;
    uint32_t max_valence = 0;
    uint32_t dropped = 0;
};
Incidence build_incidence(const int32_t* tets, uint32_t nt, uint32_t nv, bool ref_quirk, bool ref_cap);

struct Partition {
    uint32_t nv_global = 0, nt_global = 0;
    int part_count = 1, part_index = 0;
    std::vector<int32_t> local_to_global_vert;
    uint32_t n_owned = 0, n_boundary = 0;
    std::vector<int32_t> local_to_global_tet;
    std::vector<int32_t> local_tets;
    uint32_t owned_tets = 0;
    struct Neighbour {
        int rank;
        std::vector<int32_t> send_local;
        std::vector<int32_t> send_global;
        uint32_t recv_start = 0, recv_count = 0;
        std::vector<int32_t> recv_global;
        bool send_contiguous = false;
        std::vector<int32_t> send2_local, send2_global;
        uint32_t recv2_start = 0, recv2_count = 0;
        std::vector<int32_t> recv2_global;
    };
    std::vector<Neighbour> neigh;
    int depth = 1;
    uint32_t n_ghost1 = 0;
    std::vector<uint8_t> tet_layer;
};
std::string prep_partition(const float* verts, uint32_t nv, const int32_t* tets, uint32_t nt, int parts, int32_t* out_owner);
struct PartQuality {
    uint32_t owned_particles = 0, ghost_particles = 0, boundary_particles = 0;
    uint32_t local_elems = 0, owned_elems = 0;
    uint32_t num_neighbours = 0;
};
std::string partition_quality(const int32_t* tets, uint32_t nt, uint32_t nv, int parts, const int32_t* owner, PartQuality* out);
std::string build_partition(const int32_t* tets, uint32_t nt, uint32_t nv, int part_count, int part_index,
                            const int32_t* vert_owner, Partition* out, int depth = 1);

std::vector<uint32_t> morton_vertex_order(const float* xyz, uint32_t n, uint32_t first, uint32_t count);

#ifndef TETSIM_TILE
#define TETSIM_TILE 256
#endif
constexpr uint32_t kBlockTile = TETSIM_TILE;
constexpr uint32_t kQuadTile = 64;
constexpr int32_t kQuadPollDelay = 0;
constexpr uint32_t kQuadMaxPartials = 12;
struct BlockPlan {
    uint32_t num_blocks = 0;
    uint32_t tile = kBlockTile;
    std::vector<int32_t> tet_perm;
    std::vector<uint32_t> blk_tet_off;
    std::vector<uint32_t> blk_vert_off;
    std::vector<int32_t> blk_verts;
    std::vector<uint8_t> tet_lidx;
    std::vector<uint32_t> lc_range;
    std::vector<uint16_t> lc_ent;
    std::vector<uint32_t> vp_off;
    std::vector<uint32_t> vp_idx;
    std::vector<uint32_t> vp_ell;
    uint32_t vp_cols = 0;
    std::vector<uint32_t> slot_src;
    std::vector<uint32_t> blk_maxsrc;
    uint32_t ns_pad = 0;
    bool every_owned_particle_has_a_partial = true;
    uint32_t nv_pad = 0;
    uint32_t max_tile_verts = 0, max_partials = 0;
    uint32_t num_interior_blocks = 0;
    uint32_t num_first_blocks = 0;
};
void build_blocks(const float* verts, const int32_t* tets, uint32_t nt, uint32_t nv, uint32_t nv_sum,
                  const Incidence& inc, BlockPlan* out, const uint32_t* body_first_tet = nullptr,
                  const uint32_t* body_first_vert = nullptr, uint32_t bodies = 1, uint32_t nv_boundary = 0,
                  const uint8_t* tet_class = nullptr, uint32_t nv_owned = 0xffffffffu, uint32_t tile = kBlockTile);

constexpr uint32_t kSchedTile = 0u, kSchedParticles = 1u, kSchedEmpty = 2u, kSchedWrapped = 1u << 29, kSchedIndexMask = (1u << 29) - 1u;
constexpr uint32_t sched_entry(uint32_t kind, uint32_t index, bool wrapped = false) { return kind << 30 | (wrapped ? kSchedWrapped : 0u) | index; }
constexpr uint32_t pjb_call_blocks_per_sub(uint32_t nb, uint32_t nv_owned, uint32_t threads) {
    return (((nb + 7u) & ~7u) + (nv_owned + threads - 1u) / threads + 7u) & ~7u;
}
constexpr uint32_t kPJCallLagDefault = 0;
struct CallSchedule {
    std::vector<uint32_t> entry;
    uint32_t period = 0, tail = 0;
    uint32_t lag = 0;
    bool fell_back = false;
    std::string why;
};
void build_call_schedule(const int32_t* blk_verts, const uint32_t* blk_vert_off, uint32_t nb, const uint32_t* vp_ell, uint32_t vp_cols,
                         uint32_t nv_pad, uint32_t nv_owned, uint32_t lag, CallSchedule* out, uint32_t tile = kBlockTile);
std::string check_call_schedule(const int32_t* blk_verts, const uint32_t* blk_vert_off, uint32_t nb, const uint32_t* vp_ell, uint32_t vp_cols,
                                uint32_t nv_pad, uint32_t nv_owned, const uint32_t* entry, uint32_t period, uint32_t tail, uint32_t tile = kBlockTile);

std::string validate_mesh(const float* verts, uint32_t nv, const int32_t* tets, uint32_t nt, bool forbid_repeats);

}
```

### tetsim_amd/csrc/pj_blocked.hip

```cpp
#define TETSIM_FAST 1
#include <cstdio>
#include <algorithm>
#include <cstdlib>
#include <type_traits>
#include <vector>

#include "collide.h"
#include "dev_common.h"
#include "dev_store.h"
#include "host_prep.h"
#include "pj_lab.h"

namespace tetsim {
namespace {

#include "pj_math.inc"
#include "pj_blocked_lab.inc"


__device__ __forceinline__ uint32_t xcd_tile(uint32_t b, uint32_t tiles_per_xcd) { return (b & 7u) * tiles_per_xcd + (b >> 3); }

struct VertexOut { f3 p, vel, pred; };
template <bool kUniformBody, bool kTable = true>
__device__ __forceinline__ VertexOut pjb_vertex_update(f3 acc, float wsum, f3 prev, const DevParams& P, uint32_t v) {
    const float rw = __builtin_amdgcn_rcpf(wsum);
    f3 p = F3(acc.x * rw, acc.y * rw, acc.z * rw);
    bool grabbed = static_cast<int32_t>(v) == P.grab_local || static_cast<int32_t>(v) == P.grab_local2;
    if (grabbed) p = F3(P.grab[0], P.grab[1], P.grab[2]);
    body_grab_pick(P, v, grabbed, p.x, p.y, p.z);
    PolarBodyParams B = {P.gravity, P.friction, {P.lo[0], P.lo[1], P.lo[2]}, {P.hi[0], P.hi[1], P.hi[2]}};
    if constexpr (kTable) B = body_params_polar<kUniformBody>(P, v);
    p.x = fminf(fmaxf(p.x, B.lo[0]), B.hi[0]);
    p.y = fminf(fmaxf(p.y, B.lo[1]), B.hi[1]);
    p.z = fminf(fmaxf(p.z, B.lo[2]), B.hi[2]);
    if (p.y < 0.0f) {
        p.y = 0.0f;
        const float Fx = prev.x - p.x, Fz = prev.z - p.z;
        const float fr = fminf(1.0f, P.dt * B.friction);
        p.x = fmaf(Fx, fr, p.x);
        p.z = fmaf(Fz, fr, p.z);
    }
    if (any_colliders(P)) collide_particle_f32<true>(p.x, p.y, p.z, prev.x, prev.y, prev.z, P, v, !grabbed);
    const float dt = P.dt;
    const float rdt = __builtin_amdgcn_rcpf(dt);
    VertexOut o;
    o.p = p;
    const float gx = dt * 0.0f, gy = dt * B.gravity, gz = dt * 0.0f;
    o.vel = F3(fmaf(rdt, p.x - prev.x, gx), fmaf(rdt, p.y - prev.y, gy), fmaf(rdt, p.z - prev.z, gz));
    o.pred = F3(fmaf(dt, o.vel.x, p.x), fmaf(dt, o.vel.y, p.y), fmaf(dt, o.vel.z, p.z));
    return o;
}

constexpr uint32_t kTile = kBlockTile;

__device__ __forceinline__ f3 lean_fourth_corner(const f3 r[4]) {
    return F3(-((r[0].x + r[1].x) + r[2].x), -((r[0].y + r[1].y) + r[2].y), -((r[0].z + r[1].z) + r[2].z));
}
struct PJHaloWait { const PJPeerSync* w; const uint32_t* vflag; uint32_t* error; uint32_t timeout_ms; const float4* ghosts; };
constexpr int kModeCarried = 0, kModeConstantRest = 1, kModeLeanState = 2;
inline int blk_mode(const PJBlk& d) { return pjb_mode(d); }
struct PJPoll { uint32_t block, want; uint32_t* error; uint32_t timeout_ms; };
template <int kMode, bool kFused, bool kAlt = false, bool kHaloWait = false, bool kPoll = false>
__device__ __forceinline__ void pjb_tet_body(const PJBlk& d, uint32_t tile_first, uint32_t tile_count, uint32_t tiles_per_xcd TETSIM_DBG_PARAM,
                                             [[maybe_unused]] const PJHaloWait* hw = nullptr, const uint32_t stamp = 0u, [[maybe_unused]] const PJPoll* poll = nullptr) {
    __shared__ float4 s_pos[kTile];
    __shared__ float s_gx[4 * kTile];
    __shared__ float s_gy[4 * kTile];
    __shared__ float s_gz[4 * kTile];
    __shared__ uint2 s_ent[kTile];

    constexpr bool kLean = kMode == kModeConstantRest;
    uint32_t block_index = blockIdx.x;
    if constexpr (kPoll) block_index = poll->block;
    const uint32_t rel = xcd_tile(block_index, tiles_per_xcd);
    if (rel >= tile_count) return;
    const uint32_t b = tile_first + rel;
    const uint32_t tid = threadIdx.x;
    TETSIM_LAB_TILE_BEGIN();
    TETSIM_POLL_TILE(0);
    const uint32_t t0 = d.blk_tet_off[b], ntb = d.blk_tet_off[b + 1] - t0;
    const uint32_t v0 = d.blk_vert_off[b], nu = d.blk_vert_off[b + 1] - v0;

    const bool has_slot = tid < nu, has_tet = tid < ntb;
    const uint32_t slot = v0 + (has_slot ? tid : 0u), e = t0 + (has_tet ? tid : 0u);
    const uint32_t vid = static_cast<uint32_t>(d.blk_verts[slot]);
    const uint32_t range = has_slot ? d.lc_range[slot] : 0u;
    uint32_t src[8];
    uint32_t src8 = 0xffffffffu;
    [[maybe_unused]] uint32_t maxsrc = 0;
    if constexpr (kFused) {
        maxsrc = d.blk_maxsrc[b];
        const uint32_t* col = d.slot_src + slot;
#pragma unroll
        for (uint32_t j = 0; j < 8u; j++) src[j] = (j < maxsrc) ? col[static_cast<size_t>(j) * d.ns_pad] : 0xffffffffu;
        if (maxsrc > 8u) src8 = col[8ull * d.ns_pad];
    }
    const uchar4 li = d.tet_lidx[e];
    auto rec4 = [](const float4* a, uint32_t i) { if constexpr (kPoll) return load_coherent(a, i); else return a[i]; };
    float4 ra = make_float4(0.0f, 0.0f, 0.0f, 0.0f), rb = ra, rc = ra, q_old = make_float4(0.0f, 0.0f, 0.0f, 1.0f);
    auto load_record = [&]() {
        ra = rec4(d.rest_a, e); rb = rec4(d.rest_b, e);
        if constexpr (kMode == kModeLeanState) { if constexpr (kPoll) rc.x = load_coherent1(d.rest_c1, e); else rc.x = d.rest_c1[e]; }
        else { rc = rec4(d.rest_c, e); q_old = rec4(d.quat, e); }
    };
    bool record_late = false;
    if constexpr (kPoll) record_late = poll->want != 0u;
    if (!record_late) load_record();
    const float V = d.vol[e];
    const uint2 ent_row = d.lc_ent[e];
    float4 pos_stage;
    if constexpr (kFused) {
        f3 g[8];
#pragma unroll
        for (uint32_t j = 0; j < 8u; j++) {
            const float4 t = d.partial_prev[src[j] == 0xffffffffu ? 0u : src[j]];
            g[j] = src[j] == 0xffffffffu ? F3(0.0f, 0.0f, 0.0f) : xyz(t);
        }
        const float4 t8 = d.partial_prev[src8 == 0xffffffffu ? 0u : src8];
        const float4 prev4 = d.fin_in[vid];
        const float wsum = d.wsum[vid];
        f3 acc = F3(0.0f, 0.0f, 0.0f);
#pragma unroll
        for (uint32_t j = 0; j < 8u; j++) { acc.x += g[j].x; acc.y += g[j].y; acc.z += g[j].z; }
        if (src8 != 0xffffffffu) { acc.x += t8.x; acc.y += t8.y; acc.z += t8.z; }
        if (maxsrc > 9u) {
            const uint32_t* col = d.slot_src + slot;
            for (uint32_t j = 9u; j < maxsrc; j++) {
                const uint32_t sj = col[static_cast<size_t>(j) * d.ns_pad];
                const float4 tj = d.partial_prev[sj == 0xffffffffu ? 0u : sj];
                if (sj != 0xffffffffu) { acc.x += tj.x; acc.y += tj.y; acc.z += tj.z; }
            }
        }
        const VertexOut o = pjb_vertex_update<true>(acc, wsum, xyz(prev4), *d.params, vid);
        pos_stage = make_float4(o.pred.x, o.pred.y, o.pred.z, 0.0f);
        if (has_slot && ((range >> 15) & 1u)) {
            store_wt(d.fin_out, vid, make_float4(o.p.x, o.p.y, o.p.z, 0.0f));
            if (d.vel) store_wt(d.vel, vid, make_float4(o.vel.x, o.vel.y, o.vel.z, 0.0f));
        }
    } else if constexpr (kHaloWait) {
        if (tid < 64u) {
            const PJPeerSync& w = *hw->w;
            const uint32_t* word = tid == 0u ? hw->vflag : (tid <= w.n_wait ? w.wait[tid - 1u] : nullptr);
            bool pending = word != nullptr;
            const long long t0 = wall_clock64(), limit = 100000ll * hw->timeout_ms;
            while (true) {
                if (pending) pending = __hip_atomic_load(word, __ATOMIC_RELAXED, __HIP_MEMORY_SCOPE_SYSTEM) == 0u;
                if (__builtin_amdgcn_ballot_w64(pending) == 0ull) break;
                __builtin_amdgcn_s_sleep(16);
                if (limit && wall_clock64() - t0 > limit) { if (tid == 0) __hip_atomic_store(hw->error, 1u, __ATOMIC_RELAXED, __HIP_MEMORY_SCOPE_SYSTEM); break; }
            }
            if (w.delay_us && w.n_wait) { const long long d0 = wall_clock64(); while (wall_clock64() - d0 < 100ll * w.delay_us) __builtin_amdgcn_s_sleep(8); }
        }
        __syncthreads();
        const bool ghost = vid >= d.nv_owned;
        const float4 own = load_coherent(d.pos_pred, ghost ? 0u : vid), gh = load_coherent(hw->ghosts, ghost ? vid - d.nv_owned : 0u);
        pos_stage = ghost ? gh : own;
    } else if constexpr (kAlt) {
        const uint32_t g = vid - d.nv_owned;
        const float4* src = vid >= d.nv_owned ? (g < d.n_ghost1 ? d.ghost_alt + g : d.ghost2 + (g - d.n_ghost1)) : d.pos_pred + vid;
        pos_stage = *src;
    } else if constexpr (kPoll) {
        TETSIM_POLL_BEGIN();
        TETSIM_POLL_TILE(1);
        pos_stage = load_coherent(d.pos_pred, vid);
        if (poll->want != 0u) {
            bool pend = has_slot && __float_as_uint(pos_stage.w) != poll->want;
            if (__builtin_amdgcn_ballot_w64(pend) != 0ull) {
                const long long t0 = wall_clock64(), limit = 100000ll * poll->timeout_ms;
                do {
                    __builtin_amdgcn_s_sleep(TETSIM_POLL_SLEEP);
                    TETSIM_POLL_LOOK();
                    asm volatile("" ::: "memory");
                    if (pend) { pos_stage = load_coherent(d.pos_pred, vid); pend = __float_as_uint(pos_stage.w) != poll->want; }
                    if (limit && pend && wall_clock64() - t0 > limit) { __hip_atomic_store(poll->error, 1u, __ATOMIC_RELAXED, __HIP_MEMORY_SCOPE_SYSTEM); pend = false; }
                } while (__builtin_amdgcn_ballot_w64(pend) != 0ull);
            }
            TETSIM_POLL_TILE(2);
            __syncthreads();
            TETSIM_POLL_TILE(3);
            load_record();
        }
        TETSIM_POLL_TILE_SAVE();
    } else {
        pos_stage = d.pos_pred[vid];
    }
    if (has_slot) s_pos[tid] = pos_stage;
    if (has_tet) s_ent[tid] = ent_row;
    TETSIM_STAMP(1);
    __builtin_amdgcn_s_waitcnt(0x0F70);
    __syncthreads();
    TETSIM_STAMP(2);

    if (has_tet) {
        f3 cur[4], rest[4], goal[4];
        cur[0] = xyz(s_pos[li.x]); cur[1] = xyz(s_pos[li.y]); cur[2] = xyz(s_pos[li.z]); cur[3] = xyz(s_pos[li.w]);
        rest[0] = F3(ra.x, ra.y, ra.z); rest[1] = F3(ra.w, rb.x, rb.y);
        rest[2] = F3(rb.z, rb.w, rc.x); rest[3] = F3(rc.y, rc.z, rc.w);
        if constexpr (kMode == kModeLeanState) rest[3] = lean_fourth_corner(rest);
        float4 q_new;
        f3 cc;
        TETSIM_LAB_SOLVE_TET(cur, rest, q_old, q_new, goal, cc);
        TETSIM_STAMP(3);
        const f3 vcc = cc * V;
#pragma unroll
        for (int k = 0; k < 4; k++) {
            s_gx[k * kTile + tid] = fmaf(goal[k].x, V, vcc.x);
            s_gy[k * kTile + tid] = fmaf(goal[k].y, V, vcc.y);
            s_gz[k * kTile + tid] = fmaf(goal[k].z, V, vcc.z);
        }
        if constexpr (kMode != kModeLeanState) store_wt(d.quat, e, q_new);
        if (!kLean && TETSIM_DBG_STORE_REST) {
            store_wt(d.rest_a, e, make_float4(goal[0].x, goal[0].y, goal[0].z, goal[1].x));
            store_wt(d.rest_b, e, make_float4(goal[1].y, goal[1].z, goal[2].x, goal[2].y));
            if constexpr (kMode == kModeLeanState) store_wt1(d.rest_c1, e, goal[2].z);
            else store_wt(d.rest_c, e, make_float4(goal[2].z, goal[3].x, goal[3].y, goal[3].z));
        }
    }
    TETSIM_STAMP(4);
    if constexpr (kPoll) __builtin_amdgcn_s_waitcnt(0x0F70);
    __syncthreads();
    TETSIM_STAMP(5);

    if (tid < nu) {
        const uint32_t first = range & 0x7ffu, last = range >> 16;
        const uint16_t* ent = reinterpret_cast<const uint16_t*>(s_ent);
        auto plane = [](const float* base, uint32_t byte_off) { return *reinterpret_cast<const float*>(reinterpret_cast<const char*>(base) + byte_off); };
        float4 acc = make_float4(0.0f, 0.0f, 0.0f, 0.0f);
        uint32_t i = first;
        for (; i + 4u <= last; i += 4u) {
            uint32_t o[4];
            float gx[4], gy[4], gz[4];
#pragma unroll
            for (uint32_t j = 0; j < 4u; j++) o[j] = static_cast<uint32_t>(ent[i + j]) << 2;
#pragma unroll
            for (uint32_t j = 0; j < 4u; j++) { gx[j] = plane(s_gx, o[j]); gy[j] = plane(s_gy, o[j]); gz[j] = plane(s_gz, o[j]); }
#pragma unroll
            for (uint32_t j = 0; j < 4u; j++) { acc.x += gx[j]; acc.y += gy[j]; acc.z += gz[j]; }
        }
        for (; i < last; i++) {
            const uint32_t o = static_cast<uint32_t>(ent[i]) << 2;
            acc.x += plane(s_gx, o); acc.y += plane(s_gy, o); acc.z += plane(s_gz, o);
        }
        acc.w = __uint_as_float(stamp);
        store_wt(d.partial, v0 + tid, acc);
    }
    TETSIM_STAMP(6);
    TETSIM_POLL_TILE(4);
}

__global__ __launch_bounds__(kTile, 2) void pjb_tet_kernel(PJBlk d, uint32_t tile_first, uint32_t tile_count,
                                                        uint32_t tiles_per_xcd TETSIM_DBG_PARAM) {
    pjb_tet_body<kModeCarried, false>(d, tile_first, tile_count, tiles_per_xcd TETSIM_DBG_ARG);
}
__global__ __launch_bounds__(kTile, 2) void pjb_tet_kernel_constant_rest(PJBlk d, uint32_t tile_first, uint32_t tile_count,
                                                                      uint32_t tiles_per_xcd TETSIM_DBG_PARAM) {
    pjb_tet_body<kModeConstantRest, false>(d, tile_first, tile_count, tiles_per_xcd TETSIM_DBG_ARG);
}
__global__ __launch_bounds__(kTile, 2) void pjb_tet_kernel_lean(PJBlk d, uint32_t tile_first, uint32_t tile_count,
                                                             uint32_t tiles_per_xcd TETSIM_DBG_PARAM) {
    pjb_tet_body<kModeLeanState, false>(d, tile_first, tile_count, tiles_per_xcd TETSIM_DBG_ARG);
}
__device__ __forceinline__ void clear_then_raise(uint32_t* clear, uint32_t* sig) {
    if (blockIdx.x == 0 && threadIdx.x == 0) {
        if (clear) __hip_atomic_store(clear, 0u, __ATOMIC_RELAXED, __HIP_MEMORY_SCOPE_AGENT);
        if (sig) __hip_atomic_store(sig, 1u, __ATOMIC_RELEASE, __HIP_MEMORY_SCOPE_AGENT);
    }
}
struct TetRaise { uint32_t* sig; uint32_t* clear; };
struct TetAlt { uint32_t unused; };
struct TetHwait { PJPeerSync w; const uint32_t* vflag; uint32_t* error; uint32_t timeout_ms; const float4* ghosts; };
struct TetFused { uint32_t unused; };
template <int kMode, class Extra>
__global__ __launch_bounds__(kTile, 2) void pjb_tet_kernel_x(PJBlk d, uint32_t tile_first, uint32_t tile_count, uint32_t tiles_per_xcd, Extra x TETSIM_DBG_PARAM) {
    if constexpr (std::is_same_v<Extra, TetRaise>) {
        clear_then_raise(x.clear, x.sig);
        pjb_tet_body<kMode, false>(d, tile_first, tile_count, tiles_per_xcd TETSIM_DBG_ARG);
    } else if constexpr (std::is_same_v<Extra, TetAlt>) {
        pjb_tet_body<kMode, false, true>(d, tile_first, tile_count, tiles_per_xcd TETSIM_DBG_ARG);
    } else if constexpr (std::is_same_v<Extra, TetHwait>) {
        if (blockIdx.x == 0 && threadIdx.x < x.w.n_raise) __hip_atomic_store(x.w.raise[threadIdx.x], 1u, __ATOMIC_RELEASE, __HIP_MEMORY_SCOPE_SYSTEM);
        const PJHaloWait hw = {&x.w, x.vflag, x.error, x.timeout_ms, x.ghosts};
        pjb_tet_body<kMode, false, false, true>(d, tile_first, tile_count, tiles_per_xcd TETSIM_DBG_ARG, &hw);
    } else {
        pjb_tet_body<kMode, true>(d, tile_first, tile_count, tiles_per_xcd TETSIM_DBG_ARG);
    }
}
template <class Extra>
void launch_tet_x(hipStream_t s, const PJBlk& d, uint32_t tile_first, uint32_t tile_count, const Extra& x, hipEvent_t e0 = nullptr, hipEvent_t e1 = nullptr) {
    if (tile_count == 0) return;
    const uint32_t per_xcd = (tile_count + 7u) / 8u;
    const int mode = blk_mode(d);
    auto* kernel = mode == kModeConstantRest ? pjb_tet_kernel_x<kModeConstantRest, Extra> : mode == kModeLeanState ? pjb_tet_kernel_x<kModeLeanState, Extra> : pjb_tet_kernel_x<kModeCarried, Extra>;
    if (e0) hipExtLaunchKernelGGL(kernel, dim3(per_xcd * 8u), dim3(kTile), 0, s, e0, e1, 0, d, tile_first, tile_count, per_xcd, x TETSIM_DBG_LAUNCH);
    else hipLaunchKernelGGL(kernel, dim3(per_xcd * 8u), dim3(kTile), 0, s, d, tile_first, tile_count, per_xcd, x TETSIM_DBG_LAUNCH);
}

constexpr int kFrameIters = TETSIM_LAB_FRAME_ITERS;
template <int kMode, bool kLocal>
__device__ __forceinline__ void pjb_frame_body(const PJBlk& d, const DevParams& P, const uint32_t n, const int32_t* const block_tile, float4* const pbuf0, float4* const pbuf1,
                                               uint32_t* const err, const uint32_t timeout_ms) {
    __shared__ float4 s_pos[kTile];
    __shared__ float s_gx[4 * kTile];
    __shared__ float s_gy[4 * kTile];
    __shared__ float s_gz[4 * kTile];
    __shared__ uint2 s_ent[kTile];

    constexpr bool kLean = kMode == kModeConstantRest;
    const int32_t bt = block_tile[blockIdx.x];
    if (bt < 0) return;
    const uint32_t b = static_cast<uint32_t>(bt);
    const uint32_t tid = threadIdx.x;
    TETSIM_LAB_FRAME_BEGIN();
    const uint32_t t0 = d.blk_tet_off[b], ntb = d.blk_tet_off[b + 1] - t0;
    const uint32_t v0 = d.blk_vert_off[b], nu = d.blk_vert_off[b + 1] - v0;
    const bool has_slot = tid < nu, has_tet = tid < ntb;
    const uint32_t slot = v0 + (has_slot ? tid : 0u), e = t0 + (has_tet ? tid : 0u);
    const uint32_t vid = static_cast<uint32_t>(d.blk_verts[slot]);
    const uint32_t range = has_slot ? d.lc_range[slot] : 0u;
    const uint32_t maxsrc = d.blk_maxsrc[b];
    uint32_t src[9];
    {
        const uint32_t* col = d.slot_src + slot;
#pragma unroll
        for (uint32_t j = 0; j < 9u; j++) src[j] = (has_slot && j < maxsrc) ? col[static_cast<size_t>(j) * d.ns_pad] : 0xffffffffu;
    }
    const uchar4 li = d.tet_lidx[e];
    const float4 ra = d.rest_a[e], rb = d.rest_b[e];
    float4 rc = make_float4(0.0f, 0.0f, 0.0f, 0.0f), q = make_float4(0.0f, 0.0f, 0.0f, 1.0f);
    if constexpr (kMode == kModeLeanState) rc.x = d.rest_c1[e];
    else { rc = d.rest_c[e]; q = d.quat[e]; }
    const float V = d.vol[e];
    s_ent[tid] = has_tet ? d.lc_ent[e] : make_uint2(0u, 0u);
    f3 rest[4];
    rest[0] = F3(ra.x, ra.y, ra.z); rest[1] = F3(ra.w, rb.x, rb.y);
    rest[2] = F3(rb.z, rb.w, rc.x); rest[3] = F3(rc.y, rc.z, rc.w);
    f3 prev = xyz(d.pos_final[vid]);
    const float wsum = d.wsum[vid];
    f3 stage = xyz(d.pos_pred[vid]);
    const uint32_t epoch = d.epoch ? d.epoch : P.epoch;
    const uint32_t first = range & 0x7ffu, last = range >> 16;
    const bool owner = has_slot && ((range >> 15) & 1u);
    float4* const pbuf[2] = {pbuf0, pbuf1};
    const long long limit = 100000ll * timeout_ms;

    auto gather_update = [&](const uint32_t s) -> VertexOut {
        const float4* buf = pbuf[s & 1u];
        const uint32_t expect = epoch + s;
        f3 g[9];
        uint32_t pend = 0;
#pragma unroll
        for (uint32_t j = 0; j < 9u; j++) { g[j] = F3(0.0f, 0.0f, 0.0f); pend |= (src[j] != 0xffffffffu ? 1u : 0u) << j; }
        const long long w0 = limit ? wall_clock64() : 0ll;
        while (__builtin_amdgcn_ballot_w64(pend != 0u) != 0ull) {
            float4 t[9];
#pragma unroll
            for (uint32_t j = 0; j < 9u; j++)
                if ((pend >> j) & 1u) t[j] = kLocal ? load_l2(buf, src[j]) : load_coherent(buf, src[j]);
            FRAME_POLL();
#pragma unroll
            for (uint32_t j = 0; j < 9u; j++)
                if (((pend >> j) & 1u) && __float_as_uint(t[j].w) == expect) { g[j] = xyz(t[j]); pend &= ~(1u << j); }
            if (limit && pend != 0u && wall_clock64() - w0 > limit) {
                __hip_atomic_store(err, 1u, __ATOMIC_RELAXED, __HIP_MEMORY_SCOPE_SYSTEM);
                pend = 0u;
            }
        }
        f3 acc = F3(0.0f, 0.0f, 0.0f);
#pragma unroll
        for (uint32_t j = 0; j < 8u; j++) { acc.x += g[j].x; acc.y += g[j].y; acc.z += g[j].z; }
        if (src[8] != 0xffffffffu) { acc.x += g[8].x; acc.y += g[8].y; acc.z += g[8].z; }
        if (maxsrc > 9u) {
            const uint32_t* col = d.slot_src + slot;
            for (uint32_t j = 9u; j < maxsrc; j++) {
                const uint32_t sj = has_slot ? col[static_cast<size_t>(j) * d.ns_pad] : 0xffffffffu;
                bool miss = sj != 0xffffffffu;
                f3 gj = F3(0.0f, 0.0f, 0.0f);
                while (__builtin_amdgcn_ballot_w64(miss) != 0ull) {
                    if (miss) {
                        const float4 t = kLocal ? load_l2(buf, sj) : load_coherent(buf, sj);
                        if (__float_as_uint(t.w) == expect) { gj = xyz(t); miss = false; }
                    }
                    if (limit && miss && wall_clock64() - w0 > limit) {
                        __hip_atomic_store(err, 1u, __ATOMIC_RELAXED, __HIP_MEMORY_SCOPE_SYSTEM);
                        miss = false;
                    }
                }
                acc.x += gj.x; acc.y += gj.y; acc.z += gj.z;
            }
        }
        return pjb_vertex_update<true>(acc, wsum, prev, P, vid);
    };

    for (uint32_t s = 0; s < n; s++) {
        FRAME_STAMP(0);
        if (s > 0u) {
            const VertexOut o = gather_update(s - 1u);
            prev = o.p;
            stage = o.pred;
        }
        FRAME_STAMP(1);
        if (has_slot) s_pos[tid] = make_float4(stage.x, stage.y, stage.z, 0.0f);
        __syncthreads();
        FRAME_STAMP(2);
        if (has_tet) {
            f3 cur[4], r[4], goal[4];
            cur[0] = xyz(s_pos[li.x]); cur[1] = xyz(s_pos[li.y]); cur[2] = xyz(s_pos[li.z]); cur[3] = xyz(s_pos[li.w]);
#pragma unroll
            for (int k = 0; k < 4; k++) r[k] = rest[k];
            if constexpr (kMode == kModeLeanState) r[3] = lean_fourth_corner(rest);
            float4 q_new;
            f3 cc;
            pj_solve_tet(cur, r, q, q_new, goal, kFrameIters, true, kLean, !kLean, &cc, d.rot_exit_w2);
            if constexpr (kMode != kModeLeanState) q = q_new;
            if (!kLean) {
#pragma unroll
                for (int k = 0; k < 4; k++) rest[k] = goal[k];
            }
            const f3 vcc = cc * V;
#pragma unroll
            for (int k = 0; k < 4; k++) {
                s_gx[k * kTile + tid] = fmaf(goal[k].x, V, vcc.x);
                s_gy[k * kTile + tid] = fmaf(goal[k].y, V, vcc.y);
                s_gz[k * kTile + tid] = fmaf(goal[k].z, V, vcc.z);
            }
        }
        FRAME_STAMP(3);
        __syncthreads();
        FRAME_STAMP(4);
        if (has_slot) {
            const uint16_t* ent = reinterpret_cast<const uint16_t*>(s_ent);
            auto plane = [](const float* base, uint32_t byte_off) { return *reinterpret_cast<const float*>(reinterpret_cast<const char*>(base) + byte_off); };
            float4 acc = make_float4(0.0f, 0.0f, 0.0f, 0.0f);
            uint32_t i = first;
            for (; i + 4u <= last; i += 4u) {
                uint32_t o[4];
                float gx[4], gy[4], gz[4];
#pragma unroll
                for (uint32_t j = 0; j < 4u; j++) o[j] = static_cast<uint32_t>(ent[i + j]) << 2;
#pragma unroll
                for (uint32_t j = 0; j < 4u; j++) { gx[j] = plane(s_gx, o[j]); gy[j] = plane(s_gy, o[j]); gz[j] = plane(s_gz, o[j]); }
#pragma unroll
                for (uint32_t j = 0; j < 4u; j++) { acc.x += gx[j]; acc.y += gy[j]; acc.z += gz[j]; }
            }
            for (; i < last; i++) {
                const uint32_t o = static_cast<uint32_t>(ent[i]) << 2;
                acc.x += plane(s_gx, o); acc.y += plane(s_gy, o); acc.z += plane(s_gz, o);
            }
            acc.w = __uint_as_float(epoch + s);
            if constexpr (kLocal) store_plain(pbuf[s & 1u], v0 + tid, acc);
            else store_wt(pbuf[s & 1u], v0 + tid, acc);
        }
        FRAME_STAMP(5);
    }
    const VertexOut o = gather_update(n - 1u);
    TETSIM_LAB_FRAME_END();
    if (owner) {
        store_wt(d.pos_final, vid, make_float4(o.p.x, o.p.y, o.p.z, 0.0f));
        store_wt(d.vel, vid, make_float4(o.vel.x, o.vel.y, o.vel.z, 0.0f));
        store_wt(d.pos_pred, vid, make_float4(o.pred.x, o.pred.y, o.pred.z, 0.0f));
    }
    if (has_tet) {
        if constexpr (kMode != kModeLeanState) store_wt(d.quat, e, q);
        if (!kLean) {
            store_wt(d.rest_a, e, make_float4(rest[0].x, rest[0].y, rest[0].z, rest[1].x));
            store_wt(d.rest_b, e, make_float4(rest[1].y, rest[1].z, rest[2].x, rest[2].y));
            if constexpr (kMode == kModeLeanState) store_wt1(d.rest_c1, e, rest[2].z);
            else store_wt(d.rest_c, e, make_float4(rest[2].z, rest[3].x, rest[3].y, rest[3].z));
        }
    }
}
#define TETSIM_FRAME_KERNEL(name, mode, local)                                                                                         \
    __global__ __launch_bounds__(kTile, 2) void name(PJBlk d, uint32_t n, const int32_t* block_tile, float4* pbuf0, float4* pbuf1, uint32_t* err, \
                                                     uint32_t timeout_ms, DevParams pv, DevParams* pdev) {                             \
        if (blockIdx.x == 0u && threadIdx.x == 0u) store_params(pdev, pv);              \
        pjb_frame_body<mode, local>(d, pv, n, block_tile, pbuf0, pbuf1, err, timeout_ms);                                              \
    }
TETSIM_FRAME_KERNEL(pjb_frame_kernel, kModeCarried, false)
TETSIM_FRAME_KERNEL(pjb_frame_kernel_constant_rest, kModeConstantRest, false)
TETSIM_FRAME_KERNEL(pjb_frame_kernel_lean, kModeLeanState, false)
TETSIM_FRAME_KERNEL(pjb_frame_kernel_local, kModeCarried, true)
TETSIM_FRAME_KERNEL(pjb_frame_kernel_constant_rest_local, kModeConstantRest, true)
TETSIM_FRAME_KERNEL(pjb_frame_kernel_lean_local, kModeLeanState, true)
#undef TETSIM_FRAME_KERNEL
__global__ void pjb_probe_xcd_kernel(uint32_t* out) {
    if (threadIdx.x == 0) out[blockIdx.x] = __builtin_amdgcn_s_getreg(20 | (0 << 6) | (3 << 11));
}

__device__ __forceinline__ void await_done(const PJSync& y) {
    if (threadIdx.x == 0) {
        const long long t0 = wall_clock64(), limit = 100000ll * y.timeout_ms;
        while (__hip_atomic_load(y.flag, __ATOMIC_ACQUIRE, __HIP_MEMORY_SCOPE_AGENT) == 0u) {
            __builtin_amdgcn_s_sleep(4);
            if (limit && wall_clock64() - t0 > limit) {
                __hip_atomic_store(y.error, 1u, __ATOMIC_RELAXED, __HIP_MEMORY_SCOPE_SYSTEM);
                return;
            }
        }
        __hip_atomic_store(y.flag, 0u, __ATOMIC_RELAXED, __HIP_MEMORY_SCOPE_AGENT);
    }
}

template <bool kPeer = false, bool kCoherent = false>
__device__ __forceinline__ void pjb_vertex_body(const PJBlk& d, uint32_t first, uint32_t count, const PJPeer* peer = nullptr) {
    const uint32_t i = blockIdx.x * 64u + threadIdx.x;
    if (i >= count) return;
    const uint32_t v = first + i;

    float4 acc = make_float4(0.0f, 0.0f, 0.0f, 0.0f);
    const uint32_t* col = d.vp_ell + v;
    for (uint32_t j0 = 0; j0 < d.vp_cols; j0 += 8u) {
        uint32_t idx[8];
        float4 g[8];
#pragma unroll
        for (uint32_t j = 0; j < 8u; j++) idx[j] = (j0 + j < d.vp_cols) ? col[static_cast<size_t>(j0 + j) * d.nv_pad] : 0xffffffffu;
#pragma unroll
        for (uint32_t j = 0; j < 8u; j++) {
            if constexpr (kCoherent) { const float4 t = load_coherent(d.partial, idx[j] != 0xffffffffu ? idx[j] : 0u); g[j] = idx[j] != 0xffffffffu ? t : make_float4(0.0f, 0.0f, 0.0f, 0.0f); }
            else g[j] = idx[j] != 0xffffffffu ? d.partial[idx[j]] : make_float4(0.0f, 0.0f, 0.0f, 0.0f);
        }
#pragma unroll
        for (uint32_t j = 0; j < 8u; j++) { acc.x += g[j].x; acc.y += g[j].y; acc.z += g[j].z; }
        if (__all(idx[7] == 0xffffffffu)) break;
    }
    const VertexOut o = pjb_vertex_update<false>(xyz(acc), d.wsum[v], xyz(d.fin_in[v]), *d.params, v);
    store_wt(d.fin_out, v, make_float4(o.p.x, o.p.y, o.p.z, 0.0f));
    if (d.vel) store_wt(d.vel, v, make_float4(o.vel.x, o.vel.y, o.vel.z, 0.0f));
    store_wt(d.pos_pred, v, make_float4(o.pred.x, o.pred.y, o.pred.z, 0.0f));
    if constexpr (kPeer) {
        const float4 pred4 = make_float4(o.pred.x, o.pred.y, o.pred.z, 0.0f), fin4 = make_float4(o.p.x, o.p.y, o.p.z, 0.0f);
        const uint32_t* col = peer->slots + v;
        for (uint32_t c = 0; c < peer->cols; c++) {
            const uint32_t e = col[static_cast<size_t>(c) * peer->stride];
            for (uint32_t k = 0; k < peer->n; k++) {
                if (peer->ghost[k] && e != 0xffffffffu && (e >> 24) == k) store_wt(peer->ghost[k], e & 0xffffffu, pred4);
                if (peer->fin[k] && e != 0xffffffffu && (e >> 24) == k) store_wt(peer->fin[k], e & 0xffffffu, fin4);
            }
        }
        if (peer->slots2) {
            const uint32_t* col2 = peer->slots2 + v;
            for (uint32_t c = 0; c < peer->cols2; c++) {
                const uint32_t e = col2[static_cast<size_t>(c) * peer->stride];
                for (uint32_t k = 0; k < peer->n; k++)
                    if (peer->ghost2[k] && e != 0xffffffffu && (e >> 24) == k) store_wt(peer->ghost2[k], e & 0xffffffu, pred4);
            }
        }
    }
}

__global__ __launch_bounds__(64) void pjb_vertex_kernel(PJBlk d, uint32_t first, uint32_t count) { pjb_vertex_body(d, first, count); }

template <int kMode>
__global__ __launch_bounds__(kTile, 2) void pjb_call_kernel(PJBlk d, uint32_t n_sub, uint32_t tile_count, uint32_t tiles_per_xcd, const uint32_t* __restrict__ sched, uint32_t period,
                                                           uint32_t* err, uint32_t timeout_ms, DevParams pv, DevParams* pdev TETSIM_DBG_PARAM) {
    const uint32_t turn = blockIdx.x / period, entry = sched[blockIdx.x - turn * period];
    if (blockIdx.x == 0u && threadIdx.x == 0u) store_params(pdev, pv);
    const uint32_t back = (entry & kSchedWrapped) ? 1u : 0u, kind = entry >> 30, r = entry & kSchedIndexMask;
    if (kind == kSchedEmpty || turn < back || turn - back >= n_sub) return;
    const uint32_t sub = turn - back;
    const uint32_t stamp = (d.epoch ? d.epoch : pv.epoch) + sub + 1u;
    TETSIM_LAB_CALL_MARK(sub, n_sub);
    if (kind == kSchedTile) {
        const PJPoll poll = {r, sub ? stamp - 1u : 0u, err, timeout_ms};
        pjb_tet_body<kMode, false, false, false, true>(d, 0u, tile_count, tiles_per_xcd TETSIM_DBG_ARG, nullptr, stamp, &poll);
        return;
    }
    const uint32_t v = r * kTile + threadIdx.x;
    if (v >= d.nv_owned) return;
    TETSIM_POLL_BEGIN();
    TETSIM_POLL_PB(0);
    float4 acc = make_float4(0.0f, 0.0f, 0.0f, 0.0f);
    const uint32_t* col = d.vp_ell + v;
    const long long limit = 100000ll * timeout_ms;
    const float wsum = d.wsum[v];
    float4 prev = load_coherent(d.fin_in, v);
    for (uint32_t j0 = 0; j0 < d.vp_cols; j0 += 8u) {
        uint32_t idx[8];
        float4 g[8];
#pragma unroll
        for (uint32_t j = 0; j < 8u; j++) idx[j] = (j0 + j < d.vp_cols) ? col[static_cast<size_t>(j0 + j) * d.nv_pad] : 0xffffffffu;
        uint32_t pend = 0;
        TETSIM_POLL_PB_FIRST(j0);
#pragma unroll
        for (uint32_t j = 0; j < 8u; j++) {
            const float4 t = load_coherent(d.partial, idx[j] != 0xffffffffu ? idx[j] : 0u);
            g[j] = idx[j] != 0xffffffffu ? t : make_float4(0.0f, 0.0f, 0.0f, 0.0f);
            pend |= (idx[j] != 0xffffffffu && __float_as_uint(t.w) != stamp ? 1u : 0u) << j;
        }
        if (__builtin_amdgcn_ballot_w64(pend != 0u) != 0ull) {
            const long long t0 = wall_clock64();
            do {
                __builtin_amdgcn_s_sleep(TETSIM_POLL_SLEEP);
                TETSIM_POLL_LOOK();
                asm volatile("" ::: "memory");
#pragma unroll
                for (uint32_t j = 0; j < 8u; j++)
                    if ((pend >> j) & 1u) {
                        const float4 t = load_coherent(d.partial, idx[j]);
                        if (__float_as_uint(t.w) == stamp) { g[j] = t; pend &= ~(1u << j); }
                    }
                if (limit && pend != 0u && wall_clock64() - t0 > limit) {
// ... 223 lines not shown
```

### tetsim_amd/csrc/tetsim_create.hip

```cpp
#include "body.h"

namespace tetsim {

int create_polar(tetsim_body* h, const float* verts, uint32_t nv, const int32_t* tets, uint32_t nt) {
    const TetSimOptions& o = h->opt;
    const bool ref_table = (o.flags & TETSIM_FLAG_REF_SLOT_TABLE) != 0;
    std::vector<int32_t> ltets;
    std::vector<int32_t> l2g_v, l2g_t;
    uint32_t nvl = nv, nvo = nv, nvb = 0, ntl = nt;
    h->partitioned = o.part_count > 1;
    h->deep = h->partitioned && (o.flags & TETSIM_FLAG_DEEP_GHOSTS);
    {
        const char* sy = getenv("TETSIM_HALO_SYNC");
        const char* gr = getenv("TETSIM_HALO_GRAPH");
        h->halo_use_flags = !(sy && sy[0] == 'e');
        h->halo_use_graph = !(gr && gr[0] == '0');
    }
    if ((o.flags & TETSIM_FLAG_DEEP_GHOSTS) && !(h->partitioned && h->fast && !(o.flags & TETSIM_FLAG_GATHER_FORMULATION)))
        return fail(h, TETSIM_EINVAL, "TETSIM_FLAG_DEEP_GHOSTS needs a partitioned POLAR_JACOBI body in the blocked FAST formulation");
    uint32_t nvg1 = 0;
    if (h->partitioned) {
        std::string e = build_partition(tets, nt, nv, o.part_count, o.part_index, o.vert_owner, &h->part, h->deep ? 2 : 1);
        if (!e.empty()) return fail(h, TETSIM_EINVAL, e);
        if (h->deep) {
// ... 4 lines not shown
        }
        const Partition& P = h->part;
        ltets = P.local_tets;
        l2g_v = P.local_to_global_vert;
        l2g_t = P.local_to_global_tet;
        nvl = static_cast<uint32_t>(l2g_v.size());
        nvo = P.n_owned;
        nvb = P.n_boundary;
        ntl = static_cast<uint32_t>(l2g_t.size());
        h->g2l_owned.assign(nv, -1);
        for (uint32_t i = 0; i < nvo; i++) h->g2l_owned[l2g_v[i]] = static_cast<int32_t>(i);
        h->info.owned_elems = P.owned_tets;
    } else {
        ltets.assign(tets, tets + 4ull * nt);
        h->info.owned_elems = nt;
    }
    const bool batch = is_batch(h);
    const uint32_t bodies = batch ? static_cast<uint32_t>(h->batch_first_vert.size() - 1) : 1u;
    {
        std::vector<float> lv(3ull * nvl);
        for (uint32_t i = 0; i < nvl; i++) {
            const uint32_t g = h->partitioned ? static_cast<uint32_t>(l2g_v[i]) : i;
            lv[3 * i] = verts[3 * g]; lv[3 * i + 1] = verts[3 * g + 1]; lv[3 * i + 2] = verts[3 * g + 2];
        }
        if (!batch) h->dev2api = morton_vertex_order(lv.data(), nvl, nvb, nvo - nvb);
        else {
            h->dev2api.resize(nvl);
            for (uint32_t b = 0; b < bodies; b++) {
                const uint32_t vb = h->batch_first_vert[b], n = h->batch_first_vert[b + 1] - vb;
                const std::vector<uint32_t> ord = morton_vertex_order(lv.data() + 3ull * vb, n, 0, n);
                for (uint32_t i = 0; i < n; i++) h->dev2api[vb + i] = vb + ord[i];
            }
        }
        h->api2dev.resize(nvl);
        for (uint32_t dv = 0; dv < nvl; dv++) h->api2dev[h->dev2api[dv]] = dv;
        for (auto& id : ltets) id = static_cast<int32_t>(h->api2dev[id]);
    }
    Incidence inc;
    if (!batch) {
        const bool quirk_here = ref_table && ntl > 0 && (!h->partitioned || l2g_t[0] == 0);
        inc = build_incidence(ltets.data(), ntl, nvl, quirk_here, ref_table);
    } else {
        inc.offset.assign(nvl + 1, 0);
        for (uint32_t b = 0; b < bodies; b++) {
            const uint32_t vb = h->batch_first_vert[b], nvb_ = h->batch_first_vert[b + 1] - vb;
            const uint32_t tb = h->batch_first_tet[b], ntb_ = h->batch_first_tet[b + 1] - tb;
            std::vector<int32_t> bt(ltets.begin() + 4ull * tb, ltets.begin() + 4ull * (tb + ntb_));
            for (auto& id : bt) id -= static_cast<int32_t>(vb);
            const Incidence bi = build_incidence(bt.data(), ntb_, nvb_, ref_table && ntb_ > 0, ref_table);
            const uint32_t base = static_cast<uint32_t>(inc.slot.size());
            for (uint32_t v = 0; v < nvb_; v++) inc.offset[vb + v + 1] = base + bi.offset[v + 1];
            for (int32_t enc : bi.slot) inc.slot.push_back(enc + static_cast<int32_t>(4u * tb));
            inc.max_valence = std::max(inc.max_valence, bi.max_valence);
            inc.dropped += bi.dropped;
        }
    }
    uint32_t maxv = 0;
    for (uint32_t v = 0; v < nvo + nvg1; v++) maxv = std::max(maxv, inc.offset[v + 1] - inc.offset[v]);

    PJDev& d = h->pj;
    d.nv_local = nvl; d.nv_owned = nvo; d.nv_boundary = nvb; d.nt = ntl;
    d.nt_pad = (ntl + 63u) & ~63u;
    d.nv_pad = (nvo + 63u) & ~63u;
    d.max_valence = maxv;
    h->info.owned_particles = nvo;
    h->info.local_particles = nvl;
    h->info.local_elems = ntl;
    h->info.max_valence = maxv;
    h->info.dropped_slots = inc.dropped;

    int rc;
    if ((rc = dev_alloc(h, &d.pos_pred, nvl))) return rc;
    if ((rc = dev_alloc(h, &d.pos_final, nvl))) return rc;
    if ((rc = dev_alloc(h, &d.vel, nvl))) return rc;
    d.params = h->d_params;
    d.rot_exit_w2 = (h->fast && !(o.flags & TETSIM_FLAG_REF_ROTATION_EXIT)) ? 1.0e-12f : 1.0e-18f;

    std::vector<float4> pos(nvl);
    std::vector<float> lverts(3ull * nvl);
    for (uint32_t i = 0; i < nvl; i++) {
        const uint32_t a = h->dev2api[i];
        const uint32_t g = h->partitioned ? static_cast<uint32_t>(l2g_v[a]) : a;
        pos[i] = make_float4(verts[3 * g], verts[3 * g + 1], verts[3 * g + 2], 0.0f);
        lverts[3 * i] = verts[3 * g]; lverts[3 * i + 1] = verts[3 * g + 1]; lverts[3 * i + 2] = verts[3 * g + 2];
    }
    if ((rc = upload(h, d.pos_pred, pos))) return rc;
    if ((rc = upload(h, d.pos_final, pos))) return rc;
    h->final_ghosts_fresh = true;
    HIPCHK(h, hipMemset(d.vel, 0, std::max<size_t>(nvl, 1) * sizeof(float4)));

    auto rest_weight = [&](uint32_t local_tet) {
        const uint32_t ge = h->partitioned ? static_cast<uint32_t>(l2g_t[local_tet]) : local_tet;
        return 1.0f / pj_inv_rest_volume(verts, &tets[4 * ge]);
    };

    h->blocked = h->fast && !(o.flags & TETSIM_FLAG_GATHER_FORMULATION);
    if ((o.flags & TETSIM_FLAG_CONSTANT_REST_SHAPE) && !h->blocked)
        return fail(h, TETSIM_EINVAL, "TETSIM_FLAG_CONSTANT_REST_SHAPE needs POLAR_JACOBI + TETSIM_FAST without TETSIM_FLAG_GATHER_FORMULATION");
    if ((o.flags & TETSIM_FLAG_LEAN_STATE) && !h->blocked)
        return fail(h, TETSIM_EINVAL, "TETSIM_FLAG_LEAN_STATE needs POLAR_JACOBI + TETSIM_FAST without TETSIM_FLAG_GATHER_FORMULATION");
    const bool lean_state = (o.flags & TETSIM_FLAG_LEAN_STATE) != 0;
    if (h->blocked) {
        BlockPlan B;
        std::vector<uint8_t> tet_class;
        if (h->partitioned) {
            const char* e = lab_env("TETSIM_HALO_ALIGNED_TILES");
            const bool aligned = !(e && e[0] == '0');
            tet_class.assign(ntl, 0);
            for (uint32_t i = 0; i < ntl; i++) {
                if (h->deep && h->part.tet_layer[i]) { tet_class[i] = 2; continue; }
                if (!aligned) continue;
                for (int c = 0; c < 4; c++) {
                    const uint32_t v = static_cast<uint32_t>(ltets[4ull * i + c]);
                    if (v < nvb || v >= nvo) tet_class[i] = 1;
                }
            }
        }
        static const bool allow_quad = [] { const char* e = getenv("TETSIM_QUAD"); return !(e && e[0] == '0'); }();
        uint32_t quad_cus = 0, quad_per_cu = 0;
        bool quad = allow_quad && !h->partitioned && !(o.flags & (TETSIM_FLAG_CONSTANT_REST_SHAPE | TETSIM_FLAG_LEAN_STATE)) && ntl > 0 && nvo == nvl;
        if (quad) {
            quad_per_cu = pjq_frame_capacity(&quad_cus);
            quad = quad_per_cu != 0u && (static_cast<uint64_t>(ntl) + kQuadTile - 1u) / kQuadTile <= static_cast<uint64_t>(quad_per_cu) * quad_cus / 2u;
        }
        for (;;) {
            build_blocks(lverts.data(), ltets.data(), ntl, nvl, nvo + nvg1, inc, &B, batch ? h->batch_first_tet.data() : nullptr,
                         batch ? h->batch_first_vert.data() : nullptr, bodies, nvb, h->partitioned ? tet_class.data() : nullptr, nvo, quad ? kQuadTile : kBlockTile);
            if (!quad || (B.every_owned_particle_has_a_partial && B.max_partials <= kQuadMaxPartials && B.num_blocks <= quad_per_cu * quad_cus / 2u)) break;
            quad = false;
        }
        h->quad = quad;
        h->tet_perm = B.tet_perm;
        h->nb_first = B.num_first_blocks;
        for (uint32_t b = 0; b < B.num_interior_blocks; b++)
            for (uint32_t e = B.blk_tet_off[b]; e < B.blk_tet_off[b + 1]; e++)
                for (int c = 0; c < 4; c++) {
                    const uint32_t v = static_cast<uint32_t>(ltets[4ull * static_cast<uint32_t>(B.tet_perm[e]) + c]);
                    if (v < nvb || v >= nvo) return fail(h, TETSIM_ESTATE, "internal error in the tile plan: an interior tile touches a boundary or a ghost particle");
                }
        PJBlk& k = h->blk;
        h->interior_tets = B.blk_tet_off[B.num_interior_blocks];
        k.nb = B.num_blocks; k.nb_interior = B.num_interior_blocks; k.nt = ntl; k.nv_local = nvl; k.nv_owned = nvo; k.nv_boundary = nvb;
        {
            const char* fw = getenv("TETSIM_HALO_FOLD_WAIT");
            h->fold_possible = !(fw && fw[0] == '0') && h->partitioned && B.num_interior_blocks > 0 && B.num_interior_blocks < B.num_blocks && nvo > nvb;
            if (h->fold_possible) pjb_wait_capacity((o.flags & TETSIM_FLAG_CONSTANT_REST_SHAPE) ? 1 : lean_state ? 2 : 0, &h->fold_wave_limit, &h->fold_tile_limit);
            h->fold_wait = h->fold_possible && fw && fw[0] == '1';
            h->fold_halo = h->fold_wait;
        }
        k.pos_pred = d.pos_pred; k.pos_final = d.pos_final; k.vel = d.vel; k.params = h->d_params;
        k.lean = (o.flags & TETSIM_FLAG_CONSTANT_REST_SHAPE) != 0;
        k.lean_state = lean_state;
        k.rot_exit_w2 = d.rot_exit_w2;
        uint32_t *bto, *bvo, *lcr, *vpe;
        int32_t* bv;
        uchar4* lidx;
        float* vol;
        uint2* lce;
        const size_t nslots = B.blk_verts.size();
        if ((rc = dev_alloc(h, &bto, B.blk_tet_off.size()))) return rc;
        if ((rc = dev_alloc(h, &bvo, B.blk_vert_off.size()))) return rc;
        if ((rc = dev_alloc(h, &bv, nslots))) return rc;
        if (ntl >= kStoreWtMaxIndex || nslots >= kStoreWtMaxIndex || nvl >= kStoreWtMaxIndex)
            return fail(h, TETSIM_EINVAL, "body too large for one handle (2^27 tets / particles / partial sums: 32-bit store offsets, dev_store.h); partition it");
        if ((rc = dev_alloc(h, &lidx, ntl))) return rc;
        if ((rc = dev_alloc(h, &k.rest_a, ntl))) return rc;
        if ((rc = dev_alloc(h, &k.rest_b, ntl))) return rc;
        if (lean_state) {
            if ((rc = dev_alloc(h, &k.rest_c1, ntl))) return rc;
            if ((rc = dev_alloc(h, &h->rest0_a, ntl))) return rc;
            if ((rc = dev_alloc(h, &h->rest0_b, ntl))) return rc;
            if ((rc = dev_alloc(h, &h->rest0_c, ntl))) return rc;
        } else if ((rc = dev_alloc(h, &k.rest_c, ntl))) return rc;
        if ((rc = dev_alloc(h, &vol, ntl))) return rc;
        if ((rc = dev_alloc(h, &k.quat, ntl))) return rc;
        if ((rc = dev_alloc(h, &lcr, nslots))) return rc;
        if ((rc = dev_alloc(h, &lce, ntl))) return rc;
        if ((rc = dev_alloc(h, &k.partial, nslots))) return rc;
        if ((rc = dev_alloc(h, &vpe, B.vp_ell.size()))) return rc;
        std::vector<float4> ra(ntl), rb(ntl), rcv(ntl), quat(ntl, make_float4(0, 0, 0, 1));
        std::vector<float> volh(ntl);
        std::vector<uchar4> lidxh(ntl);
        std::vector<uint2> lceh(ntl);
        for (uint32_t i = 0; i < ntl; i++) {
            const uint32_t lt = static_cast<uint32_t>(B.tet_perm[i]);
            const int32_t* c = &ltets[4 * lt];
            const float4 p0 = pos[c[0]], p1 = pos[c[1]], p2 = pos[c[2]], p3 = pos[c[3]];
            float4 r0 = p0, r1 = p1, r2 = p2, r3 = p3;
            {
                const float cx = (((p0.x + p1.x) + p2.x) + p3.x) * 0.25f, cy = (((p0.y + p1.y) + p2.y) + p3.y) * 0.25f,
                            cz = (((p0.z + p1.z) + p2.z) + p3.z) * 0.25f;
                r0 = make_float4(p0.x - cx, p0.y - cy, p0.z - cz, 0.0f); r1 = make_float4(p1.x - cx, p1.y - cy, p1.z - cz, 0.0f);
                r2 = make_float4(p2.x - cx, p2.y - cy, p2.z - cz, 0.0f); r3 = make_float4(p3.x - cx, p3.y - cy, p3.z - cz, 0.0f);
            }
            ra[i] = make_float4(r0.x, r0.y, r0.z, r1.x);
            rb[i] = make_float4(r1.y, r1.z, r2.x, r2.y);
            rcv[i] = make_float4(r2.z, r3.x, r3.y, r3.z);
            volh[i] = rest_weight(lt);
            lidxh[i] = make_uchar4(B.tet_lidx[4ull * i], B.tet_lidx[4ull * i + 1], B.tet_lidx[4ull * i + 2], B.tet_lidx[4ull * i + 3]);
            const uint16_t* en = &B.lc_ent[4ull * i];
            lceh[i] = make_uint2(en[0] | (static_cast<uint32_t>(en[1]) << 16), en[2] | (static_cast<uint32_t>(en[3]) << 16));
        }
        std::vector<float> wsum(std::max<size_t>(B.nv_pad, 1), 0.0f);
        {
            std::vector<float> slot_w(nslots, 0.0f);
            for (uint32_t b = 0; b < B.num_blocks; b++) {
                const uint32_t t0 = B.blk_tet_off[b], v0 = B.blk_vert_off[b], nu = B.blk_vert_off[b + 1] - v0;
                for (uint32_t u = 0; u < nu; u++) {
                    const uint32_t first = B.lc_range[v0 + u] & 0x7ffu, last = B.lc_range[v0 + u] >> 16;
                    float w = 0.0f;
                    for (uint32_t i = first; i < last; i++) w += volh[t0 + (B.lc_ent[4ull * t0 + i] % B.tile)];
                    slot_w[v0 + u] = w;
                }
            }
            for (uint32_t v = 0; v < nvo + nvg1; v++) {
                float w = 0.0f;
                for (uint32_t j = 0; j < B.max_partials; j++) {
                    const uint32_t idx = B.vp_ell[static_cast<size_t>(j) * B.nv_pad + v];
                    if (idx != 0xffffffffu) w += slot_w[idx];
                }
                wsum[v] = w;
            }
        }
        float* dws;
        if ((rc = dev_alloc(h, &dws, wsum.size()))) return rc;
        if ((rc = upload(h, dws, wsum))) return rc;
        k.wsum = dws;
        static const bool allow_fused = [] { const char* e = getenv("TETSIM_FUSED_PARTICLE_PASS"); return !(e && e[0] == '0'); }();
        static const bool force_fused = [] { const char* e = getenv("TETSIM_FUSED_PARTICLE_PASS"); return e && e[0] == '1'; }();
        h->fused = allow_fused && !h->quad && !h->partitioned && nvo == nvl && B.every_owned_particle_has_a_partial && ntl > 0 &&
                   (B.num_blocks < 2048u || force_fused);
        k.fin_in = d.pos_final; k.fin_out = d.pos_final;
        h->info.fused_particle_pass = h->fused ? 1u : 0u;
        {
            const char* e = getenv("TETSIM_PJ_ONE_LAUNCH");
            h->pj_one_launch = !(e && e[0] == '0') && !h->fused && !h->quad && !h->partitioned && nvo == nvl && ntl > 0 && B.num_blocks > 0;
            if (h->pj_one_launch) {
                h->info.fused_particle_pass = 5u;
                if ((rc = dev_alloc(h, &h->d_substep_err, 1))) return rc;
                HIPCHK(h, hipMemset(h->d_substep_err, 0, sizeof(uint32_t)));
                const char* lag_env = getenv("TETSIM_PJ_CALL_LAG");
                const uint32_t lag = lag_env ? static_cast<uint32_t>(std::min<unsigned long>(strtoul(lag_env, nullptr, 10), 1ul << 24)) : kPJCallLagDefault;
                CallSchedule S;
                build_call_schedule(B.blk_verts.data(), B.blk_vert_off.data(), B.num_blocks, B.vp_ell.data(), B.vp_cols, B.nv_pad, nvo, lag, &S);
                if (S.fell_back) fprintf(stderr, "[tetsim] TETSIM_PJ_CALL_LAG=%u ignored (%s): the call runs in the plain order\n", lag, S.why.c_str());
                uint32_t* dsched;
                if ((rc = dev_alloc(h, &dsched, S.entry.size()))) return rc;
                if ((rc = upload(h, dsched, S.entry))) return rc;
                h->call_sched.entry = dsched; h->call_sched.period = S.period; h->call_sched.tail = S.tail;
            }
        }
        if (h->fused || h->quad) {
            uint32_t *dsrc, *dmax;
            if ((rc = dev_alloc(h, &dsrc, B.slot_src.size()))) return rc;
            if ((rc = dev_alloc(h, &dmax, B.blk_maxsrc.size()))) return rc;
            if ((rc = dev_alloc(h, &h->partial_b, nslots))) return rc;
            if ((rc = upload(h, dsrc, B.slot_src))) return rc;
            if ((rc = upload(h, dmax, B.blk_maxsrc))) return rc;
            HIPCHK(h, hipMemset(h->partial_b, 0, std::max<size_t>(nslots, 1) * sizeof(float4)));
            h->partial_slots = nslots;
            if (h->fused) {
                if ((rc = dev_alloc(h, &h->pos_final_b, nvl))) return rc;
                if ((rc = upload(h, h->pos_final_b, pos))) return rc;
            }
            k.slot_src = dsrc; k.blk_maxsrc = dmax; k.ns_pad = B.ns_pad;
            static const bool allow_frame = [] { const char* e = getenv("TETSIM_FRAME_KERNEL"); return !(e && e[0] == '0'); }();
            uint32_t cus = 0;
            const uint32_t per_cu = !allow_frame ? 0u : h->quad ? pjq_frame_capacity(&cus) : pjb_frame_capacity(pjb_mode(k), &cus);
            const uint32_t nbk = B.num_blocks;
            std::vector<int32_t> block_tile;
            const uint32_t slots = per_cu * cus, exclusive_max = slots - slots / 10u;
            if (per_cu != 0u && nbk != 0u && nbk <= (h->partitioned ? slots / 2u : exclusive_max)) {
                h->frame_exclusive = nbk > slots / 2u;
                static const bool allow_local = [] { const char* e = lab_env("TETSIM_FRAME_LOCAL"); return !(e && e[0] == '0'); }();
                static int xcd_rule[64] = {};
                int& rule = xcd_rule[o.device & 63];
                if (allow_local && rule == 0) rule = pjb_probe_xcd(h->stream, 256) == 8u ? 1 : 2;
                std::vector<std::vector<uint32_t>> groups(bodies);
                for (uint32_t b = 0; b < nbk; b++) {
                    const uint32_t body = batch ? body_of_tet(h, static_cast<uint32_t>(B.tet_perm[B.blk_tet_off[b]])) : 0u;
                    groups[std::min(body, bodies - 1u)].push_back(b);
                }
                const uint32_t budget = per_cu * (cus / 8u) / 2u;
                std::vector<uint32_t> by_size(bodies);
                for (uint32_t g = 0; g < bodies; g++) by_size[g] = g;
                std::stable_sort(by_size.begin(), by_size.end(), [&](uint32_t a, uint32_t c) { return groups[a].size() > groups[c].size(); });
                std::vector<std::vector<uint32_t>> on_xcd(8);
                bool local = allow_local && rule == 1 && cus % 8u == 0u;
                for (uint32_t g : by_size) {
                    if (!local) break;
                    uint32_t best = 0;
                    for (uint32_t x = 1; x < 8u; x++) if (on_xcd[x].size() < on_xcd[best].size()) best = x;
                    if (on_xcd[best].size() + groups[g].size() > budget) { local = false; break; }
                    on_xcd[best].insert(on_xcd[best].end(), groups[g].begin(), groups[g].end());
                }
                if (!local) {
                    for (auto& v : on_xcd) v.clear();
                    for (uint32_t b = 0; b < nbk; b++) on_xcd[b & 7u].push_back(b);
                }
                uint32_t most = 0;
                for (auto& v : on_xcd) most = std::max<uint32_t>(most, static_cast<uint32_t>(v.size()));
                block_tile.assign(8ull * most, -1);
                for (uint32_t x = 0; x < 8u; x++)
                    for (uint32_t j = 0; j < on_xcd[x].size(); j++) block_tile[8ull * j + x] = static_cast<int32_t>(on_xcd[x][j]);
                h->frame = true;
                frame_turn_enter(h);
                h->frame_local = local;
                h->frame_blocks = static_cast<uint32_t>(block_tile.size());
            }
            if (h->frame) {
                if ((rc = dev_alloc(h, &h->d_block_tile, block_tile.size()))) return rc;
                if ((rc = upload(h, h->d_block_tile, block_tile))) return rc;
                if ((rc = dev_alloc(h, &h->d_frame_err, 1))) return rc;
                HIPCHK(h, hipMemset(h->d_frame_err, 0, sizeof(uint32_t)));
                h->info.fused_particle_pass = h->quad ? 3u : 2u;
            }
        }
        if ((rc = upload(h, bto, B.blk_tet_off))) return rc;
        if ((rc = upload(h, bvo, B.blk_vert_off))) return rc;
        if ((rc = upload(h, bv, B.blk_verts))) return rc;
        if ((rc = upload(h, lidx, lidxh))) return rc;
        if ((rc = upload(h, k.rest_a, ra))) return rc;
        if ((rc = upload(h, k.rest_b, rb))) return rc;
        if (lean_state) {
            std::vector<float> rc1(ntl);
            for (uint32_t i = 0; i < ntl; i++) rc1[i] = rcv[i].x;
            if ((rc = upload(h, k.rest_c1, rc1))) return rc;
            if ((rc = upload(h, h->rest0_a, ra))) return rc;
            if ((rc = upload(h, h->rest0_b, rb))) return rc;
            if ((rc = upload(h, h->rest0_c, rcv))) return rc;
        } else if ((rc = upload(h, k.rest_c, rcv))) return rc;
        if ((rc = upload(h, vol, volh))) return rc;
        if ((rc = upload(h, k.quat, quat))) return rc;
        if ((rc = upload(h, lcr, B.lc_range))) return rc;
        if ((rc = upload(h, lce, lceh))) return rc;
        if ((rc = upload(h, vpe, B.vp_ell))) return rc;
        HIPCHK(h, hipMemset(k.partial, 0, std::max<size_t>(nslots, 1) * sizeof(float4)));
        k.blk_tet_off = bto; k.blk_vert_off = bvo; k.blk_verts = bv; k.tet_lidx = lidx; k.vol = vol;
        k.lc_range = lcr; k.lc_ent = lce; k.vp_ell = vpe; k.vp_cols = B.vp_cols; k.nv_pad = B.nv_pad;
        d.quat = k.quat;
#ifdef TETSIM_ABLATION
        if (lab_env("TETSIM_DEBUG_ITER_HIST")) {
            if ((rc = dev_alloc(h, &k.iter_hist, 278))) return rc;
            HIPCHK(h, hipMemset(k.iter_hist, 0, 278 * sizeof(unsigned long long)));
        }
#endif
        if (lab_env("TETSIM_DEBUG_TRACE") || lab_env("TETSIM_DEBUG_POLL_TRACE")) {
            const size_t rows = lab_env("TETSIM_DEBUG_POLL_TRACE") ? 2ull * B.num_blocks + (nvo + kBlockTile - 1u) / kBlockTile : B.num_blocks;
            if ((rc = dev_alloc(h, &k.trace, 8ull * rows))) return rc;
            HIPCHK(h, hipMemset(k.trace, 0, 8ull * rows * sizeof(unsigned long long)));
        }
    } else {
        if ((rc = dev_alloc(h, &d.tet_idx, ntl))) return rc;
        if ((rc = dev_alloc(h, &d.elem, 4ull * d.nt_pad))) return rc;
        if ((rc = dev_alloc(h, &d.quat, ntl))) return rc;
        if ((rc = dev_alloc(h, &d.slot_tab, static_cast<size_t>(std::max(maxv, 1u)) * d.nv_pad))) return rc;
        if ((rc = dev_alloc(h, &d.slot_cnt, d.nv_pad))) return rc;
        std::vector<int4> idx(ntl);
        std::vector<float4> elem(4ull * d.nt_pad, make_float4(0, 0, 0, 0)), quat(ntl, make_float4(0, 0, 0, 1));
        for (uint32_t e = 0; e < ntl; e++) {
            const int32_t* lt = &ltets[4 * e];
            idx[e] = make_int4(lt[0], lt[1], lt[2], lt[3]);
            const float w = rest_weight(e);
            for (int k = 0; k < 4; k++) {
                const float4 p = pos[lt[k]];
                elem[static_cast<size_t>(k) * d.nt_pad + e] = make_float4(p.x, p.y, p.z, w);
            }
        }
        if ((rc = upload(h, d.tet_idx, idx))) return rc;
        if ((rc = upload(h, d.elem, elem))) return rc;
        if ((rc = upload(h, d.quat, quat))) return rc;

        std::vector<int32_t> tab(static_cast<size_t>(std::max(maxv, 1u)) * d.nv_pad, 0);
        std::vector<uint32_t> cnt(d.nv_pad, 0);
        for (uint32_t v = 0; v < nvo; v++) {
            const uint32_t c = inc.offset[v + 1] - inc.offset[v];
            cnt[v] = c;
            for (uint32_t sl = 0; sl < c; sl++) {
                const int32_t enc = inc.slot[inc.offset[v] + sl];
                tab[static_cast<size_t>(sl) * d.nv_pad + v] = static_cast<int32_t>((enc & 3) * d.nt_pad + (enc >> 2));
            }
        }
        if ((rc = upload(h, d.slot_tab, tab))) return rc;
        if ((rc = upload(h, d.slot_cnt, cnt))) return rc;
    }

    if (h->partitioned) {
        for (const auto& nb : h->part.neigh) {
            NeighDev nd;
            nd.rank = nb.rank;
            nd.send_count = static_cast<uint32_t>(nb.send_local.size());
            nd.recv_start = nb.recv_start;
            nd.recv_count = nb.recv_count;
            nd.contiguous = nb.send_contiguous;
            nd.send_first = nd.send_count ? static_cast<uint32_t>(nb.send_local[0]) : 0;
            nd.send_global = nb.send_global;
            nd.recv_global = nb.recv_global;
            nd.send_local = nb.send_local;
            if (nd.send_count) {
                if ((rc = dev_alloc(h, &nd.send_idx, nd.send_count))) return rc;
                if ((rc = dev_alloc(h, &nd.send_buf, nd.send_count))) return rc;
                if ((rc = upload(h, nd.send_idx, nb.send_local))) return rc;
            }
            h->neigh.push_back(std::move(nd));
        }
        h->info.num_neighbours = static_cast<uint32_t>(h->neigh.size());
    }
    return 0;
}

int create_neohookean(tetsim_body* h, const float* verts, uint32_t nv, const int32_t* tets, uint32_t nt) {
    const TetSimOptions& o = h->opt;
    if (o.part_count > 1) return fail(h, TETSIM_EINVAL, "NEOHOOKEAN_GS does not partition (one halo per colour would be needed); use POLAR_JACOBI");
    std::vector<int32_t> pre(nt);
    for (uint32_t e = 0; e < nt; e++) pre[e] = static_cast<int32_t>(e);
    if (o.order == TETSIM_ORDER_COLOURED) {
        std::vector<int32_t> colour(nt);
        if (h->tet_colour.size() == nt) colour = h->tet_colour;
        else prep_colours(tets, nt, nv, colour.data());
        std::stable_sort(pre.begin(), pre.end(), [&](int32_t a, int32_t b) { return colour[a] < colour[b]; });
    }
    ClusterPlan plan;
    const bool clustered = o.order == TETSIM_ORDER_CLUSTERED;
    if (clustered) {
        plan = prep_clusters(tets, nt, nv);
        pre = plan.pre;
    }
    std::vector<int32_t> ptets(4ull * nt);
    for (uint32_t i = 0; i < nt; i++) std::memcpy(&ptets[4 * i], &tets[4 * pre[i]], 4 * sizeof(int32_t));
    std::vector<float> irp(9ull * nt), irv(nt);
    h->h_inv_mass.assign(nv, 0.0f);
    prep_rest(verts, nv, ptets.data(), nt, o.density, h->h_inv_mass.data(), irp.data(), irv.data());
    std::vector<int32_t> pos_in(nt);
    std::vector<uint32_t> body_of;
    uint32_t nl = 0;
    if (clustered) {
        nl = static_cast<uint32_t>(plan.launch_off.size() - 1);
        for (uint32_t i = 0; i < nt; i++) pos_in[i] = static_cast<int32_t>(plan.exec_pos[i]);
        h->level_off = plan.launch_off;
    } else {
        std::vector<int32_t> level(nt);
        nl = prep_levels(ptets.data(), nt, nv, level.data());
        for (uint32_t i = 0; i < nt; i++) pos_in[i] = static_cast<int32_t>(i);
        body_of.resize(nt);
        for (uint32_t i = 0; i < nt; i++) body_of[i] = body_of_tet(h, static_cast<uint32_t>(pre[i]));
        std::stable_sort(pos_in.begin(), pos_in.end(), [&](int32_t a, int32_t b) { return level[a] != level[b] ? level[a] < level[b] : body_of[a] < body_of[b]; });
        h->level_off.assign(nl + 1, 0);
        for (uint32_t i = 0; i < nt; i++) h->level_off[level[i] + 1]++;
        for (uint32_t l = 0; l < nl; l++) h->level_off[l + 1] += h->level_off[l];
    }
    h->order.resize(nt);
    std::vector<int32_t> seq(nt);
    for (uint32_t i = 0; i < nt; i++) seq[i] = pre[i];
    h->order = seq;
    h->info.num_levels = nl;
    h->info.owned_particles = h->info.local_particles = nv;
    h->info.local_elems = h->info.owned_elems = nt;

    if (nv >= kStoreWtMaxIndex) return fail(h, TETSIM_EINVAL, "more than 2^27 particles (32-bit store offsets, dev_store.h)");
    NHDev& d = h->nh;
    d.nv = nv; d.nt = nt;
    int rc;
    if ((rc = dev_alloc(h, &d.pos, nv))) return rc;
    if ((rc = dev_alloc(h, &d.prev, nv))) return rc;
    if ((rc = dev_alloc(h, &d.vel, nv))) return rc;
    if ((rc = dev_alloc(h, &d.tet_idx, nt))) return rc;
    if ((rc = dev_alloc(h, &d.irp_a, nt))) return rc;
    if ((rc = dev_alloc(h, &d.irp_b, nt))) return rc;
    if ((rc = dev_alloc(h, &d.irp_c, nt))) return rc;
    if ((rc = dev_alloc(h, &d.vol_err, nt))) return rc;
    if ((rc = dev_alloc(h, &d.order, nt))) return rc;
    d.params = h->d_params;

    std::vector<float4> pos(nv);
    for (uint32_t i = 0; i < nv; i++) pos[i] = make_float4(verts[3 * i], verts[3 * i + 1], verts[3 * i + 2], h->h_inv_mass[i]);
    if ((rc = upload(h, d.pos, pos))) return rc;
    if ((rc = upload(h, d.prev, pos))) return rc;
    HIPCHK(h, hipMemset(d.vel, 0, std::max<size_t>(nv, 1) * sizeof(float4)));
    HIPCHK(h, hipMemset(d.vol_err, 0, std::max<size_t>(nt, 1) * sizeof(double)));
    std::vector<int4> idx(nt);
    std::vector<float4> a(nt), b(nt), c(nt);
    std::vector<int32_t> ord(nt);
    for (uint32_t s = 0; s < nt; s++) {
        const uint32_t i = static_cast<uint32_t>(pos_in[s]);
        const int32_t* t = &ptets[4 * i];
        idx[s] = make_int4(t[0], t[1], t[2], t[3]);
        const float* m = &irp[9 * i];
        a[s] = make_float4(m[0], m[1], m[2], m[3]);
        b[s] = make_float4(m[4], m[5], m[6], m[7]);
        c[s] = make_float4(m[8], irv[i], 0.0f, 0.0f);
        ord[s] = static_cast<int32_t>(i);
// ... 167 lines not shown
```

### tetsim_amd/csrc/tetsim_host.cpp

```cpp
#include "body.h"

using namespace tetsim;

namespace tetsim {
void build_strain_table(const float* verts, uint32_t nv, const int32_t* tets, uint32_t nt, double density, StrainRec* out) {
    std::vector<float> inv_mass(nv), irp(9ull * nt), irv(nt);
    prep_rest(verts, nv, tets, nt, density, inv_mass.data(), irp.data(), irv.data());
    for (uint32_t e = 0; e < nt; e++) {
        StrainRec& r = out[e];
        const int32_t* t = &tets[4ull * e];
        const double v0 = rest_volume(verts, t);
        bool finite = true;
        for (uint32_t k = 0; k < 9u; k++) {
            r.b[k] = irp[9ull * e + k];
            finite = finite && std::isfinite(r.b[k]);
        }
        for (uint32_t k = 0; k < 4u; k++) r.id[k] = t[k];
        r.degenerate = (v0 == 0.0 || !finite) ? 1u : 0u;
        r.v0_abs = std::fabs(v0);
    }
}
void build_pose_table(const float* verts, uint32_t nv, const int32_t* tets, uint32_t nt, const uint32_t* first_vert, uint32_t bodies, double density,
                      PoseRec* out, double* centres) {
    for (uint32_t i = 0; i < nv; i++) out[i].m = 0.0;
    for (uint32_t e = 0; e < nt; e++) {
        const int32_t* t = &tets[4ull * e];
        const double w = (density * rest_volume(verts, t)) / 4.0;
        for (uint32_t k = 0; k < 4u; k++) out[t[k]].m = out[t[k]].m + w;
    }
    for (uint32_t b = 0; b < bodies; b++) {
        double m0 = 0.0, s[3] = {0.0, 0.0, 0.0}, c0[3] = {0.0, 0.0, 0.0};
        for (uint32_t i = first_vert[b]; i < first_vert[b + 1]; i++) {
            m0 = m0 + out[i].m;
            for (uint32_t k = 0; k < 3u; k++) s[k] = s[k] + out[i].m * static_cast<double>(verts[3ull * i + k]);
        }
        if (m0 != 0.0)
            for (uint32_t k = 0; k < 3u; k++) c0[k] = s[k] / m0;
        for (uint32_t i = first_vert[b]; i < first_vert[b + 1]; i++)
            for (uint32_t k = 0; k < 3u; k++) out[i].q[k] = static_cast<double>(verts[3ull * i + k]) - c0[k];
        if (centres)
            for (uint32_t k = 0; k < 3u; k++) centres[3ull * b + k] = c0[k];
    }
}
}

extern "C" {

struct tetsim_mesh_file { tetsim::MeshFile* m; };

int tetsim_mesh_write(const char* path, const TetSimMeshArrays* a) {
    if (!a) return fail(nullptr, TETSIM_EINVAL, "arrays is null");
    const std::string e = mesh_write(path, *a);
    return e.empty() ? TETSIM_OK : fail(nullptr, TETSIM_EINVAL, e);
}
int tetsim_mesh_open(const char* path, tetsim_mesh* out) {
    if (!out) return fail(nullptr, TETSIM_EINVAL, "out is null");
    *out = nullptr;
    tetsim::MeshFile* m = nullptr;
    const std::string e = mesh_open(path, &m);
    if (!e.empty()) return fail(nullptr, TETSIM_EINVAL, e);
    *out = new tetsim_mesh_file{m};
    return TETSIM_OK;
}
int tetsim_mesh_arrays(tetsim_mesh m, TetSimMeshArrays* out) {
    if (!m || !out) return fail(nullptr, TETSIM_EINVAL, "null argument");
    *out = mesh_arrays(m->m);
    return TETSIM_OK;
}
int tetsim_mesh_close(tetsim_mesh m) {
    if (!m) return TETSIM_OK;
    mesh_close(m->m);
    delete m;
    return TETSIM_OK;
}

int tetsim_prep_levels(const int32_t* tets, uint32_t nt, uint32_t nv, int32_t* level, uint32_t* num_levels) {
    if ((nt && (!tets || !level)) || !num_levels) return TETSIM_EINVAL;
    std::string e = validate_mesh(reinterpret_cast<const float*>(tets), nv ? nv : 1, tets, nt, false);
    if (!e.empty()) return fail(nullptr, TETSIM_EINVAL, e);
    *num_levels = prep_levels(tets, nt, nv, level);
    return 0;
}
int tetsim_prep_colours(const int32_t* tets, uint32_t nt, uint32_t nv, int32_t* colour, uint32_t* num_colours) {
    if ((nt && (!tets || !colour)) || !num_colours) return TETSIM_EINVAL;
    std::string e = validate_mesh(reinterpret_cast<const float*>(tets), nv ? nv : 1, tets, nt, false);
    if (!e.empty()) return fail(nullptr, TETSIM_EINVAL, e);
    *num_colours = prep_colours(tets, nt, nv, colour);
    return 0;
}
int tetsim_prep_clusters(const int32_t* tets, uint32_t nt, uint32_t nv, int32_t* order, int32_t* launch, int32_t* lane, int32_t* step,
                         uint32_t* num_launches, uint32_t* num_clusters) {
    if ((nt && (!tets || !order || !launch || !lane || !step)) || !num_launches) return TETSIM_EINVAL;
    std::string e = validate_mesh(reinterpret_cast<const float*>(tets), nv ? nv : 1, tets, nt, false);
    if (!e.empty()) return fail(nullptr, TETSIM_EINVAL, e);
    const ClusterPlan P = prep_clusters(tets, nt, nv);
    for (uint32_t i = 0; i < nt; i++) order[i] = P.pre[i];
    const uint32_t nl = static_cast<uint32_t>(P.launch_off.size() - 1);
    for (uint32_t l = 0; l < nl; l++)
        for (uint32_t j = P.step_off[l]; j < P.step_off[l + 1]; j++)
            for (uint32_t i = 0; i < P.step_count[j]; i++) {
                const uint32_t pos = P.exec_pos[P.step_first[j] + i];
                launch[pos] = static_cast<int32_t>(l);
                lane[pos] = static_cast<int32_t>(i);
                step[pos] = static_cast<int32_t>(j - P.step_off[l]);
            }
    *num_launches = nl;
    if (num_clusters) *num_clusters = P.num_clusters;
    return 0;
}
int tetsim_prep_tiles(const float* verts, uint32_t nv, const int32_t* tets, uint32_t nt, const uint32_t* body_first_tet,
                      const uint32_t* body_first_vert, uint32_t bodies, int32_t* tile_tets, uint32_t* tile_off, uint8_t* corner_slot,
                      uint32_t* num_tiles) {
    if (!num_tiles) return TETSIM_EINVAL;
    std::string e = validate_mesh(verts, nv, tets, nt, false);
    if (!e.empty()) return fail(nullptr, TETSIM_EINVAL, e);
    if (body_first_tet && body_first_vert && bodies) {
        if (body_first_tet[0] != 0 || body_first_vert[0] != 0 || body_first_tet[bodies] != nt || body_first_vert[bodies] != nv)
            return fail(nullptr, TETSIM_EINVAL, "body ranges must cover the whole mesh");
        for (uint32_t b = 0; b < bodies; b++) {
            if (body_first_tet[b] > body_first_tet[b + 1] || body_first_vert[b] >= body_first_vert[b + 1]) return fail(nullptr, TETSIM_EINVAL, "body ranges must ascend");
            for (uint64_t i = 4ull * body_first_tet[b]; i < 4ull * body_first_tet[b + 1]; i++)
                if (static_cast<uint32_t>(tets[i]) < body_first_vert[b] || static_cast<uint32_t>(tets[i]) >= body_first_vert[b + 1])
                    return fail(nullptr, TETSIM_EINVAL, "a tet references a particle of another body");
        }
    }
    const Incidence inc = build_incidence(tets, nt, nv, false, false);
    BlockPlan B;
    build_blocks(verts, tets, nt, nv, nv, inc, &B, body_first_tet, body_first_vert, bodies);
    *num_tiles = B.num_blocks;
    if (tile_tets) std::copy(B.tet_perm.begin(), B.tet_perm.end(), tile_tets);
    if (tile_off) std::copy(B.blk_tet_off.begin(), B.blk_tet_off.end(), tile_off);
    if (corner_slot) std::copy(B.tet_lidx.begin(), B.tet_lidx.end(), corner_slot);
    return 0;
}
int tetsim_prep_slot_table(const int32_t* tets, uint32_t nt, uint32_t nv, int32_t ref_quirk, int32_t* slots, uint32_t* dropped) {
    if ((nt && !tets) || !slots) return TETSIM_EINVAL;
    std::string e = validate_mesh(reinterpret_cast<const float*>(tets), nv ? nv : 1, tets, nt, false);
    if (!e.empty()) return fail(nullptr, TETSIM_EINVAL, e);
    const uint32_t d = prep_slot_table(tets, nt, nv, ref_quirk != 0, slots);
    if (dropped) *dropped = d;
    return 0;
}
int tetsim_prep_call_tiles(const float* verts, uint32_t nv, const int32_t* tets, uint32_t nt, uint32_t sizes[4], uint32_t* blk_vert_off,
                           int32_t* blk_verts, uint32_t* vp_ell) {
    if (!sizes) return TETSIM_EINVAL;
    std::string e = validate_mesh(verts, nv, tets, nt, false);
    if (!e.empty()) return fail(nullptr, TETSIM_EINVAL, e);
    const std::vector<uint32_t> order = morton_vertex_order(verts, nv, 0, nv);
    std::vector<int32_t> to_dev(nv), ltets(4ull * nt);
    std::vector<float> lverts(3ull * nv);
    for (uint32_t i = 0; i < nv; i++) {
        to_dev[order[i]] = static_cast<int32_t>(i);
        for (int c = 0; c < 3; c++) lverts[3ull * i + c] = verts[3ull * order[i] + c];
    }
    for (uint64_t i = 0; i < 4ull * nt; i++) ltets[i] = to_dev[tets[i]];
    const Incidence inc = build_incidence(ltets.data(), nt, nv, false, false);
    BlockPlan B;
    build_blocks(lverts.data(), ltets.data(), nt, nv, nv, inc, &B);
    sizes[0] = B.num_blocks; sizes[1] = static_cast<uint32_t>(B.blk_verts.size()); sizes[2] = B.vp_cols; sizes[3] = B.nv_pad;
    if (blk_vert_off) std::copy(B.blk_vert_off.begin(), B.blk_vert_off.end(), blk_vert_off);
    if (blk_verts) std::copy(B.blk_verts.begin(), B.blk_verts.end(), blk_verts);
    if (vp_ell) std::copy(B.vp_ell.begin(), B.vp_ell.begin() + static_cast<std::ptrdiff_t>(static_cast<size_t>(B.vp_cols) * B.nv_pad), vp_ell);
    return 0;
}
int tetsim_prep_call_schedule(const int32_t* blk_verts, const uint32_t* blk_vert_off, uint32_t nb, const uint32_t* vp_ell, uint32_t vp_cols,
                              uint32_t nv_pad, uint32_t nv_owned, uint32_t lag, uint32_t* entry, uint32_t capacity, uint32_t* period,
                              uint32_t* tail, int32_t* fell_back) {
    if (!blk_vert_off || (nb && !blk_verts) || (vp_cols && !vp_ell) || !period || !tail) return TETSIM_EINVAL;
    if (nv_owned > nv_pad && vp_cols) return fail(nullptr, TETSIM_EINVAL, "tetsim_prep_call_schedule: nv_owned exceeds the column stride of vp_ell");
    CallSchedule S;
    build_call_schedule(blk_verts, blk_vert_off, nb, vp_ell, vp_cols, nv_pad, nv_owned, lag, &S);
    *period = S.period; *tail = S.tail;
    if (fell_back) *fell_back = S.fell_back ? 1 : 0;
    if (S.fell_back) fail(nullptr, TETSIM_OK, "tetsim_prep_call_schedule: " + S.why + " -- the plain order instead");
    if (entry) {
        if (capacity < S.period) return fail(nullptr, TETSIM_EINVAL, "tetsim_prep_call_schedule: the table needs " + std::to_string(S.period) + " entries");
        std::copy(S.entry.begin(), S.entry.end(), entry);
    }
    return 0;
}
int tetsim_prep_check_call_schedule(const int32_t* blk_verts, const uint32_t* blk_vert_off, uint32_t nb, const uint32_t* vp_ell, uint32_t vp_cols,
                                    uint32_t nv_pad, uint32_t nv_owned, const uint32_t* entry, uint32_t period, uint32_t tail) {
    if (!blk_vert_off || (nb && !blk_verts) || (vp_cols && !vp_ell) || !entry) return TETSIM_EINVAL;
    const std::string bad = check_call_schedule(blk_verts, blk_vert_off, nb, vp_ell, vp_cols, nv_pad, nv_owned, entry, period, tail);
    return bad.empty() ? 0 : fail(nullptr, TETSIM_EINVAL, "call schedule: " + bad);
}
int tetsim_prep_ref_grab_texels(int32_t grab_id, uint32_t num_elems, uint32_t num_particles, int32_t out[2]) {
    if (!out) return TETSIM_EINVAL;
    ref_grab_texels(grab_id, num_elems, num_particles, out);
    return 0;
}
int tetsim_prep_boundary_surface(const float* verts, const int32_t* tets, uint32_t nt, uint32_t nv, float* vis_verts, int32_t* tri_ids,
                                 uint32_t* nrows, uint32_t* ntri) {
    if ((nt && !tets) || !nrows || !ntri || (!vis_verts != !tri_ids)) return fail(nullptr, TETSIM_EINVAL, "tetsim_prep_boundary_surface: null argument");
    if (nt && nv == 0) return fail(nullptr, TETSIM_EINVAL, "tetsim_prep_boundary_surface: tets without particles (nv == 0)");
    std::string e = validate_mesh(reinterpret_cast<const float*>(tets), nv ? nv : 1, tets, nt, false);
    if (!e.empty()) return fail(nullptr, TETSIM_EINVAL, e);
    if (nt > (1u << 24)) return fail(nullptr, TETSIM_EINVAL, "tetsim_prep_boundary_surface: a tet id above 2^24 does not fit the f32 row format");
    static const int kFace[4][3] = {{1, 2, 3}, {0, 3, 2}, {0, 1, 3}, {0, 2, 1}};
    struct Face { int32_t key[3]; uint32_t tet, face; };
    std::vector<Face> faces(4ull * nt);
    for (uint32_t t = 0; t < nt; t++)
        for (uint32_t k = 0; k < 4; k++) {
            Face& f = faces[4ull * t + k];
            for (int j = 0; j < 3; j++) f.key[j] = tets[4 * t + kFace[k][j]];
            std::sort(f.key, f.key + 3);
            f.tet = t; f.face = k;
        }
    std::sort(faces.begin(), faces.end(), [](const Face& a, const Face& b) {
        return std::lexicographical_compare(a.key, a.key + 3, b.key, b.key + 3) || (std::equal(a.key, a.key + 3, b.key) && (a.tet < b.tet || (a.tet == b.tet && a.face < b.face)));
    });
    std::vector<uint64_t> boundary;
    for (size_t i = 0; i < faces.size();) {
        size_t j = i + 1;
        while (j < faces.size() && std::equal(faces[i].key, faces[i].key + 3, faces[j].key)) j++;
        if (j - i == 1) boundary.push_back(4ull * faces[i].tet + faces[i].face);
        i = j;
    }
    std::sort(boundary.begin(), boundary.end());
    std::vector<int32_t> row(nv, -1);
    for (uint64_t b : boundary)
        for (int j = 0; j < 3; j++) row[tets[4 * (b >> 2) + kFace[b & 3][j]]] = 0;
    uint32_t rows = 0;
    for (uint32_t v = 0; v < nv; v++)
        if (row[v] == 0) row[v] = static_cast<int32_t>(rows++);
    *nrows = rows;
    *ntri = static_cast<uint32_t>(boundary.size());
    if (!vis_verts) return 0;
    std::vector<uint8_t> done(rows, 0);
    for (uint32_t t = 0; t < nt; t++)
        for (int k = 0; k < 4; k++) {
            const int32_t r = row[tets[4 * t + k]];
            if (r < 0 || done[r]) continue;
            done[r] = 1;
            vis_verts[4 * r] = static_cast<float>(t);
            for (int j = 0; j < 3; j++) vis_verts[4 * r + 1 + j] = j == k ? 1.0f : 0.0f;
        }
    for (size_t i = 0; i < boundary.size(); i++) {
        const uint32_t t = static_cast<uint32_t>(boundary[i] >> 2), k = static_cast<uint32_t>(boundary[i] & 3);
        bool flip = false;
        if (verts) {
            const int32_t* c = tets + 4 * t;
            double m[3][3];
            for (int a = 0; a < 3; a++)
                for (int x = 0; x < 3; x++) m[a][x] = static_cast<double>(verts[3 * c[a + 1] + x]) - static_cast<double>(verts[3 * c[0] + x]);
            const double det = m[0][0] * (m[1][1] * m[2][2] - m[1][2] * m[2][1]) - m[0][1] * (m[1][0] * m[2][2] - m[1][2] * m[2][0]) +
                               m[0][2] * (m[1][0] * m[2][1] - m[1][1] * m[2][0]);
            flip = det < 0.0;
        }
        const int32_t a = row[tets[4 * t + kFace[k][0]]], b = row[tets[4 * t + kFace[k][1]]], c2 = row[tets[4 * t + kFace[k][2]]];
        tri_ids[3 * i] = a;
        tri_ids[3 * i + 1] = flip ? c2 : b;
        tri_ids[3 * i + 2] = flip ? b : c2;
    }
    return 0;
}
int tetsim_prep_rest(const float* verts, uint32_t nv, const int32_t* tets, uint32_t nt, double density, float* inv_mass, float* inv_rest_pose, float* inv_rest_volume) {
    if (!inv_mass || (nt && (!inv_rest_pose || !inv_rest_volume))) return TETSIM_EINVAL;
    std::string e = validate_mesh(verts, nv, tets, nt, false);
    if (!e.empty()) return fail(nullptr, TETSIM_EINVAL, e);
    prep_rest(verts, nv, tets, nt, density, inv_mass, inv_rest_pose, inv_rest_volume);
    return 0;
}

int tetsim_prep_strain_table(const float* verts, uint32_t nv, const int32_t* tets, uint32_t nt, double density, void* records_out) {
    if (nt && !records_out) return TETSIM_EINVAL;
    std::string e = validate_mesh(verts, nv, tets, nt, false);
    if (!e.empty()) return fail(nullptr, TETSIM_EINVAL, e);
    std::vector<StrainRec> recs(nt);
    build_strain_table(verts, nv, tets, nt, density, recs.data());
    if (nt) std::memcpy(records_out, recs.data(), recs.size() * sizeof(StrainRec));
    return 0;
}

int tetsim_prep_pose_table(const float* verts, uint32_t nv, const int32_t* tets, uint32_t nt, const uint32_t* body_first_vert, const uint32_t* body_first_tet,
                           uint32_t num_bodies, double density, void* records_out, double* centres_out) {
    if (nv && !records_out) return TETSIM_EINVAL;
    if ((body_first_vert == nullptr) != (body_first_tet == nullptr)) return fail(nullptr, TETSIM_EINVAL, "body_first_vert and body_first_tet must both be given or both be NULL");
    std::string e = validate_mesh(verts, nv, tets, nt, false);
    if (!e.empty()) return fail(nullptr, TETSIM_EINVAL, e);
    std::vector<uint32_t> fv = {0u, nv};
    if (body_first_vert) {
        if (!num_bodies) return fail(nullptr, TETSIM_EINVAL, "num_bodies is 0");
        if (body_first_tet[0] != 0 || body_first_vert[0] != 0 || body_first_tet[num_bodies] != nt || body_first_vert[num_bodies] != nv)
            return fail(nullptr, TETSIM_EINVAL, "body ranges must cover the whole mesh");
// ... 129 lines not shown
```

Before: 35180 M tet-solves/s.

## Scatter tet goals into per-slot sorted shared layout, pack tet row metadata

Each tet now writes its corner goal contributions straight to precomputed positions in shared memory, sorted by destination slot. Each slot's reduction then reads a contiguous run instead of indirecting through a shared entry table. Slot lookup for corners goes through a per-block s_slot byte map that each slot fills, and vol plus packed corner positions merge into one 12-byte per-tet row. This cuts a global load stream and the indirect shared reads, at the cost of an extra shared fill loop, scattered shared writes and more host prep.

```diff
diff --git a/include/tetsim.h b/include/tetsim.h
--- a/include/tetsim.h
+++ b/include/tetsim.h
@@ -346,6 +346,9 @@
 int tetsim_prep_tiles(const float *verts, uint32_t nv, const int32_t *tets, uint32_t nt, const uint32_t *body_first_tet,
                       const uint32_t *body_first_vert, uint32_t bodies, int32_t *tile_tets, uint32_t *tile_off,
                       uint8_t *corner_slot, uint32_t *num_tiles);
+int tetsim_prep_tile_tables(const float *verts, uint32_t nv, const int32_t *tets, uint32_t nt, int32_t ref_table, uint32_t sizes[2],
+                            int32_t *tile_tets, uint32_t *tile_off, uint32_t *slot_off, int32_t *slot_particle, uint8_t *corner_slot,
+                            uint16_t *entries, uint32_t *ranges, uint32_t *tet_pos, uint16_t *run_first);
 int tetsim_prep_bvh(const float *positions, uint32_t nvis, const int32_t *tri_ids, uint32_t ntri, const int32_t *tri_body, uint32_t bodies,
                     uint32_t *tri_first, uint32_t *order, uint32_t *node_first, uint32_t *depth, uint32_t *node_range);
 int tetsim_prep_slot_table(const int32_t *tets, uint32_t nt, uint32_t nv, int32_t ref_quirk,
diff --git a/tetsim_amd/_capi.py b/tetsim_amd/_capi.py
--- a/tetsim_amd/_capi.py
+++ b/tetsim_amd/_capi.py
@@ -145,7 +145,7 @@
     "tetsim_comm_unique_id", "tetsim_comm_init", "tetsim_comm_info", "tetsim_comm_selftest", "tetsim_comm_probe", "tetsim_group_step_n", "tetsim_halo_exchange_local", "tetsim_get_halo_plan",
     "tetsim_halo_p2p_export", "tetsim_halo_p2p_connect",
     "tetsim_halo_export", "tetsim_halo_import", "tetsim_prep_levels", "tetsim_prep_colours", "tetsim_prep_clusters",
-    "tetsim_prep_tiles", "tetsim_prep_slot_table", "tetsim_prep_call_tiles", "tetsim_prep_call_schedule", "tetsim_prep_check_call_schedule", "tetsim_prep_ref_grab_texels", "tetsim_prep_rest", "tetsim_prep_partition", "tetsim_prep_partition_quality", "tetsim_plan_create", "tetsim_plan_destroy", "tetsim_plan_sizes",
+    "tetsim_prep_tiles", "tetsim_prep_tile_tables", "tetsim_prep_slot_table", "tetsim_prep_call_tiles", "tetsim_prep_call_schedule", "tetsim_prep_check_call_schedule", "tetsim_prep_ref_grab_texels", "tetsim_prep_rest", "tetsim_prep_partition", "tetsim_prep_partition_quality", "tetsim_plan_create", "tetsim_plan_destroy", "tetsim_plan_sizes",
     "tetsim_plan_arrays", "tetsim_plan_neighbour", "tetsim_plan_neighbour_ids",
     "tetsim_plan_create_deep", "tetsim_plan_layers", "tetsim_plan_neighbour_layer2", "tetsim_plan_neighbour_layer2_ids",
     "tetsim_raycast_visual", "tetsim_start_grab_ray", "tetsim_read_visual_bounding_sphere", "tetsim_prep_boundary_surface",
@@ -318,6 +318,7 @@
     L.tetsim_prep_tiles.argtypes = [fp, u32, ip, u32, C.POINTER(u32), C.POINTER(u32), u32, ip, C.POINTER(u32), C.POINTER(C.c_uint8), C.POINTER(u32)]
     L.tetsim_prep_slot_table.argtypes = [ip, u32, u32, i32, ip, C.POINTER(u32)]
     up = C.POINTER(u32)
+    L.tetsim_prep_tile_tables.argtypes = [fp, u32, ip, u32, C.c_int32, up, ip, up, up, ip, C.POINTER(C.c_uint8), C.POINTER(C.c_uint16), up, up, C.POINTER(C.c_uint16)]
     L.tetsim_prep_call_tiles.argtypes = [fp, u32, ip, u32, up, up, ip, up]
     L.tetsim_prep_call_schedule.argtypes = [ip, up, u32, up, u32, u32, u32, u32, up, u32, up, up, ip]
     L.tetsim_prep_check_call_schedule.argtypes = [ip, up, u32, up, u32, u32, u32, up, u32, u32]
diff --git a/tetsim_amd/csrc/dev_common.h b/tetsim_amd/csrc/dev_common.h
--- a/tetsim_amd/csrc/dev_common.h
+++ b/tetsim_amd/csrc/dev_common.h
@@ -114,6 +114,7 @@
     float rot_exit_w2 = 1.0e-18f;
 };
 
+struct PJTetRow { uint32_t pos_lo, pos_hi, vol; };
 struct PJBlk {
     uint32_t nb = 0, nb_interior = 0, nt = 0, nv_local = 0, nv_owned = 0, nv_boundary = 0;
     const uint32_t* blk_tet_off = nullptr;
@@ -128,6 +129,8 @@
     float4* quat = nullptr;
     const uint32_t* lc_range = nullptr;
     const uint2* lc_ent = nullptr;
+    const PJTetRow* tet_row = nullptr;
+    const uint16_t* lc_first = nullptr;
     float4* partial = nullptr;
     const float* wsum = nullptr;
     const uint32_t* vp_ell = nullptr;
diff --git a/tetsim_amd/csrc/host_prep.cpp b/tetsim_amd/csrc/host_prep.cpp
--- a/tetsim_amd/csrc/host_prep.cpp
+++ b/tetsim_amd/csrc/host_prep.cpp
@@ -413,6 +413,7 @@
 
     B.tet_lidx.resize(4ull * nt);
     B.lc_ent.resize(4ull * nt);
+    B.tet_pos.assign(2ull * nt, 0u);
     B.blk_tet_off.push_back(0);
     B.blk_vert_off.push_back(0);
     std::vector<std::vector<uint32_t>> vert_partials(nv_sum);
@@ -446,6 +447,24 @@
                     const uint32_t u = B.tet_lidx[4ull * (t0 + j) + k];
                     B.lc_ent[4ull * t0 + fillp[u]++] = static_cast<uint16_t>(kMaxTets * k + j);
                 }
+        {
+            std::vector<uint32_t> all(nu + 1, 0);
+            for (uint32_t j = 0; j < ntb; j++)
+                for (int k = 0; k < 4; k++) all[B.tet_lidx[4ull * (t0 + j) + k] + 1]++;
+            for (uint32_t u = 0; u < nu; u++) all[u + 1] += all[u];
+            for (uint32_t u = 0; u <= nu; u++) B.lc_first.push_back(static_cast<uint16_t>(all[u]));
+            std::vector<uint32_t> at(all.begin(), all.end() - 1);
+            for (int pass = 0; pass < 2; pass++)
+                for (uint32_t j = 0; j < ntb; j++)
+                    for (int k = 0; k < 4; k++) {
+                        const bool dropped = !live[4ull * B.tet_perm[t0 + j] + k];
+                        if (dropped != (pass == 1)) continue;
+                        const uint64_t p = static_cast<uint64_t>(at[B.tet_lidx[4ull * (t0 + j) + k]]++) << (10 * k);
+                        uint32_t* w = &B.tet_pos[2ull * (t0 + j)];
+                        w[0] |= static_cast<uint32_t>(p);
+                        w[1] |= static_cast<uint32_t>(p >> 32) | (dropped ? 1u << (8 + k) : 0u);
+                    }
+        }
         for (uint32_t u = 0; u < nu; u++) {
             const int32_t v = touched[u];
             B.blk_verts.push_back(v);
@@ -487,7 +506,7 @@
             const std::vector<uint32_t>& list = vert_partials[v];
             for (size_t j = 0; j < list.size(); j++) B.slot_src[j * B.ns_pad + g] = list[j];
             B.blk_maxsrc[b] = std::max<uint32_t>(B.blk_maxsrc[b], static_cast<uint32_t>(list.size()));
-            if (!list.empty() && list[0] == g) B.lc_range[g] |= 1u << 15;
+            if (!list.empty() && list[0] == g) { B.lc_range[g] |= 1u << 15; B.lc_first[g + b] |= 1u << 15; }
         }
 }
 
diff --git a/tetsim_amd/csrc/host_prep.h b/tetsim_amd/csrc/host_prep.h
--- a/tetsim_amd/csrc/host_prep.h
+++ b/tetsim_amd/csrc/host_prep.h
@@ -90,6 +90,8 @@
     std::vector<uint8_t> tet_lidx;
     std::vector<uint32_t> lc_range;
     std::vector<uint16_t> lc_ent;
+    std::vector<uint32_t> tet_pos;
+    std::vector<uint16_t> lc_first;
     std::vector<uint32_t> vp_off;
     std::vector<uint32_t> vp_idx;
     std::vector<uint32_t> vp_ell;
diff --git a/tetsim_amd/csrc/pj_blocked.hip b/tetsim_amd/csrc/pj_blocked.hip
--- a/tetsim_amd/csrc/pj_blocked.hip
+++ b/tetsim_amd/csrc/pj_blocked.hip
@@ -67,7 +67,7 @@
     __shared__ float s_gx[4 * kTile];
     __shared__ float s_gy[4 * kTile];
     __shared__ float s_gz[4 * kTile];
-    __shared__ uint2 s_ent[kTile];
+    __shared__ uint8_t s_slot[4 * kTile];
 
     constexpr bool kLean = kMode == kModeConstantRest;
     uint32_t block_index = blockIdx.x;
@@ -84,7 +84,12 @@
     const bool has_slot = tid < nu, has_tet = tid < ntb;
     const uint32_t slot = v0 + (has_slot ? tid : 0u), e = t0 + (has_tet ? tid : 0u);
     const uint32_t vid = static_cast<uint32_t>(d.blk_verts[slot]);
-    const uint32_t range = has_slot ? d.lc_range[slot] : 0u;
+    const uint32_t range = has_slot ? d.lc_first[slot + b] : 0u, range_end = has_slot ? d.lc_first[slot + b + 1u] : 0u;
+    const uint32_t first = range & 0x7ffu, last = range_end & 0x7ffu;
+    auto fill_slots = [&]() {
+        if (has_slot)
+            for (uint32_t i = first; i < last; i++) s_slot[i] = static_cast<uint8_t>(tid);
+    };
     uint32_t src[8];
     uint32_t src8 = 0xffffffffu;
     [[maybe_unused]] uint32_t maxsrc = 0;
@@ -95,7 +100,6 @@
         for (uint32_t j = 0; j < 8u; j++) src[j] = (j < maxsrc) ? col[static_cast<size_t>(j) * d.ns_pad] : 0xffffffffu;
         if (maxsrc > 8u) src8 = col[8ull * d.ns_pad];
     }
-    const uchar4 li = d.tet_lidx[e];
     auto rec4 = [](const float4* a, uint32_t i) { if constexpr (kPoll) return load_coherent(a, i); else return a[i]; };
     float4 ra = make_float4(0.0f, 0.0f, 0.0f, 0.0f), rb = ra, rc = ra, q_old = make_float4(0.0f, 0.0f, 0.0f, 1.0f);
     auto load_record = [&]() {
@@ -106,8 +110,10 @@
     bool record_late = false;
     if constexpr (kPoll) record_late = poll->want != 0u;
     if (!record_late) load_record();
-    const float V = d.vol[e];
-    const uint2 ent_row = d.lc_ent[e];
+    const PJTetRow row = d.tet_row[e];
+    const float V = __uint_as_float(row.vol);
+    const uint32_t lp[4] = {row.pos_lo & 1023u, (row.pos_lo >> 10) & 1023u, (row.pos_lo >> 20) & 1023u, (row.pos_lo >> 30) | ((row.pos_hi & 255u) << 2)};
+    const uint32_t dropped = row.pos_hi >> 8;
     float4 pos_stage;
     if constexpr (kFused) {
         f3 g[8];
@@ -119,6 +125,7 @@
         const float4 t8 = d.partial_prev[src8 == 0xffffffffu ? 0u : src8];
         const float4 prev4 = d.fin_in[vid];
         const float wsum = d.wsum[vid];
+        fill_slots();
         f3 acc = F3(0.0f, 0.0f, 0.0f);
 #pragma unroll
         for (uint32_t j = 0; j < 8u; j++) { acc.x += g[j].x; acc.y += g[j].y; acc.z += g[j].z; }
@@ -154,15 +161,18 @@
         __syncthreads();
         const bool ghost = vid >= d.nv_owned;
         const float4 own = load_coherent(d.pos_pred, ghost ? 0u : vid), gh = load_coherent(hw->ghosts, ghost ? vid - d.nv_owned : 0u);
+        fill_slots();
         pos_stage = ghost ? gh : own;
     } else if constexpr (kAlt) {
         const uint32_t g = vid - d.nv_owned;
         const float4* src = vid >= d.nv_owned ? (g < d.n_ghost1 ? d.ghost_alt + g : d.ghost2 + (g - d.n_ghost1)) : d.pos_pred + vid;
         pos_stage = *src;
+        fill_slots();
     } else if constexpr (kPoll) {
         TETSIM_POLL_BEGIN();
         TETSIM_POLL_TILE(1);
         pos_stage = load_coherent(d.pos_pred, vid);
+        fill_slots();
         if (poll->want != 0u) {
             bool pend = has_slot && __float_as_uint(pos_stage.w) != poll->want;
             if (__builtin_amdgcn_ballot_w64(pend) != 0ull) {
@@ -183,9 +193,9 @@
         TETSIM_POLL_TILE_SAVE();
     } else {
         pos_stage = d.pos_pred[vid];
+        fill_slots();
     }
     if (has_slot) s_pos[tid] = pos_stage;
-    if (has_tet) s_ent[tid] = ent_row;
     TETSIM_STAMP(1);
     __builtin_amdgcn_s_waitcnt(0x0F70);
     __syncthreads();
@@ -193,7 +203,10 @@
 
     if (has_tet) {
         f3 cur[4], rest[4], goal[4];
-        cur[0] = xyz(s_pos[li.x]); cur[1] = xyz(s_pos[li.y]); cur[2] = xyz(s_pos[li.z]); cur[3] = xyz(s_pos[li.w]);
+        {
+            const uint32_t l0 = s_slot[lp[0]], l1 = s_slot[lp[1]], l2 = s_slot[lp[2]], l3 = s_slot[lp[3]];
+            cur[0] = xyz(s_pos[l0]); cur[1] = xyz(s_pos[l1]); cur[2] = xyz(s_pos[l2]); cur[3] = xyz(s_pos[l3]);
+        }
         rest[0] = F3(ra.x, ra.y, ra.z); rest[1] = F3(ra.w, rb.x, rb.y);
         rest[2] = F3(rb.z, rb.w, rc.x); rest[3] = F3(rc.y, rc.z, rc.w);
         if constexpr (kMode == kModeLeanState) rest[3] = lean_fourth_corner(rest);
@@ -204,9 +217,10 @@
         const f3 vcc = cc * V;
 #pragma unroll
         for (int k = 0; k < 4; k++) {
-            s_gx[k * kTile + tid] = fmaf(goal[k].x, V, vcc.x);
-            s_gy[k * kTile + tid] = fmaf(goal[k].y, V, vcc.y);
-            s_gz[k * kTile + tid] = fmaf(goal[k].z, V, vcc.z);
+            const bool live = ((dropped >> k) & 1u) == 0u;
+            s_gx[lp[k]] = live ? fmaf(goal[k].x, V, vcc.x) : 0.0f;
+            s_gy[lp[k]] = live ? fmaf(goal[k].y, V, vcc.y) : 0.0f;
+            s_gz[lp[k]] = live ? fmaf(goal[k].z, V, vcc.z) : 0.0f;
         }
         if constexpr (kMode != kModeLeanState) store_wt(d.quat, e, q_new);
         if (!kLean && TETSIM_DBG_STORE_REST) {
@@ -222,25 +236,16 @@
     TETSIM_STAMP(5);
 
     if (tid < nu) {
-        const uint32_t first = range & 0x7ffu, last = range >> 16;
-        const uint16_t* ent = reinterpret_cast<const uint16_t*>(s_ent);
-        auto plane = [](const float* base, uint32_t byte_off) { return *reinterpret_cast<const float*>(reinterpret_cast<const char*>(base) + byte_off); };
         float4 acc = make_float4(0.0f, 0.0f, 0.0f, 0.0f);
         uint32_t i = first;
         for (; i + 4u <= last; i += 4u) {
-            uint32_t o[4];
             float gx[4], gy[4], gz[4];
 #pragma unroll
-            for (uint32_t j = 0; j < 4u; j++) o[j] = static_cast<uint32_t>(ent[i + j]) << 2;
-#pragma unroll
-            for (uint32_t j = 0; j < 4u; j++) { gx[j] = plane(s_gx, o[j]); gy[j] = plane(s_gy, o[j]); gz[j] = plane(s_gz, o[j]); }
+            for (uint32_t j = 0; j < 4u; j++) { gx[j] = s_gx[i + j]; gy[j] = s_gy[i + j]; gz[j] = s_gz[i + j]; }
 #pragma unroll
             for (uint32_t j = 0; j < 4u; j++) { acc.x += gx[j]; acc.y += gy[j]; acc.z += gz[j]; }
         }
-        for (; i < last; i++) {
-            const uint32_t o = static_cast<uint32_t>(ent[i]) << 2;
-            acc.x += plane(s_gx, o); acc.y += plane(s_gy, o); acc.z += plane(s_gz, o);
-        }
+        for (; i < last; i++) { acc.x += s_gx[i]; acc.y += s_gy[i]; acc.z += s_gz[i]; }
         acc.w = __uint_as_float(stamp);
         store_wt(d.partial, v0 + tid, acc);
     }
@@ -303,7 +308,7 @@
     __shared__ float s_gx[4 * kTile];
     __shared__ float s_gy[4 * kTile];
     __shared__ float s_gz[4 * kTile];
-    __shared__ uint2 s_ent[kTile];
+    __shared__ uint8_t s_slot[4 * kTile];
 
     constexpr bool kLean = kMode == kModeConstantRest;
     const int32_t bt = block_tile[blockIdx.x];
@@ -316,7 +321,7 @@
     const bool has_slot = tid < nu, has_tet = tid < ntb;
     const uint32_t slot = v0 + (has_slot ? tid : 0u), e = t0 + (has_tet ? tid : 0u);
     const uint32_t vid = static_cast<uint32_t>(d.blk_verts[slot]);
-    const uint32_t range = has_slot ? d.lc_range[slot] : 0u;
+    const uint32_t range = has_slot ? d.lc_first[slot + b] : 0u, range_end = has_slot ? d.lc_first[slot + b + 1u] : 0u;
     const uint32_t maxsrc = d.blk_maxsrc[b];
     uint32_t src[9];
     {
@@ -324,13 +329,14 @@
 #pragma unroll
         for (uint32_t j = 0; j < 9u; j++) src[j] = (has_slot && j < maxsrc) ? col[static_cast<size_t>(j) * d.ns_pad] : 0xffffffffu;
     }
-    const uchar4 li = d.tet_lidx[e];
+    const PJTetRow row = d.tet_row[e];
     const float4 ra = d.rest_a[e], rb = d.rest_b[e];
     float4 rc = make_float4(0.0f, 0.0f, 0.0f, 0.0f), q = make_float4(0.0f, 0.0f, 0.0f, 1.0f);
     if constexpr (kMode == kModeLeanState) rc.x = d.rest_c1[e];
     else { rc = d.rest_c[e]; q = d.quat[e]; }
-    const float V = d.vol[e];
-    s_ent[tid] = has_tet ? d.lc_ent[e] : make_uint2(0u, 0u);
+    const float V = __uint_as_float(row.vol);
+    const uint32_t lp[4] = {row.pos_lo & 1023u, (row.pos_lo >> 10) & 1023u, (row.pos_lo >> 20) & 1023u, (row.pos_lo >> 30) | ((row.pos_hi & 255u) << 2)};
+    const uint32_t dropped = row.pos_hi >> 8;
     f3 rest[4];
     rest[0] = F3(ra.x, ra.y, ra.z); rest[1] = F3(ra.w, rb.x, rb.y);
     rest[2] = F3(rb.z, rb.w, rc.x); rest[3] = F3(rc.y, rc.z, rc.w);
@@ -338,8 +344,12 @@
     const float wsum = d.wsum[vid];
     f3 stage = xyz(d.pos_pred[vid]);
     const uint32_t epoch = d.epoch ? d.epoch : P.epoch;
-    const uint32_t first = range & 0x7ffu, last = range >> 16;
+    const uint32_t first = range & 0x7ffu, last = range_end & 0x7ffu;
     const bool owner = has_slot && ((range >> 15) & 1u);
+    if (has_slot)
+        for (uint32_t i = first; i < last; i++) s_slot[i] = static_cast<uint8_t>(tid);
+    __syncthreads();
+    const uint32_t li[4] = {s_slot[lp[0]], s_slot[lp[1]], s_slot[lp[2]], s_slot[lp[3]]};
     float4* const pbuf[2] = {pbuf0, pbuf1};
     const long long limit = 100000ll * timeout_ms;
 
@@ -404,7 +414,7 @@
         FRAME_STAMP(2);
         if (has_tet) {
             f3 cur[4], r[4], goal[4];
-            cur[0] = xyz(s_pos[li.x]); cur[1] = xyz(s_pos[li.y]); cur[2] = xyz(s_pos[li.z]); cur[3] = xyz(s_pos[li.w]);
+            cur[0] = xyz(s_pos[li[0]]); cur[1] = xyz(s_pos[li[1]]); cur[2] = xyz(s_pos[li[2]]); cur[3] = xyz(s_pos[li[3]]);
 #pragma unroll
             for (int k = 0; k < 4; k++) r[k] = rest[k];
             if constexpr (kMode == kModeLeanState) r[3] = lean_fourth_corner(rest);
@@ -419,33 +429,26 @@
             const f3 vcc = cc * V;
 #pragma unroll
             for (int k = 0; k < 4; k++) {
-                s_gx[k * kTile + tid] = fmaf(goal[k].x, V, vcc.x);
-                s_gy[k * kTile + tid] = fmaf(goal[k].y, V, vcc.y);
-                s_gz[k * kTile + tid] = fmaf(goal[k].z, V, vcc.z);
+                const bool live = ((dropped >> k) & 1u) == 0u;
+                s_gx[lp[k]] = live ? fmaf(goal[k].x, V, vcc.x) : 0.0f;
+                s_gy[lp[k]] = live ? fmaf(goal[k].y, V, vcc.y) : 0.0f;
+                s_gz[lp[k]] = live ? fmaf(goal[k].z, V, vcc.z) : 0.0f;
             }
         }
         FRAME_STAMP(3);
         __syncthreads();
         FRAME_STAMP(4);
         if (has_slot) {
-            const uint16_t* ent = reinterpret_cast<const uint16_t*>(s_ent);
-            auto plane = [](const float* base, uint32_t byte_off) { return *reinterpret_cast<const float*>(reinterpret_cast<const char*>(base) + byte_off); };
             float4 acc = make_float4(0.0f, 0.0f, 0.0f, 0.0f);
             uint32_t i = first;
             for (; i + 4u <= last; i += 4u) {
-                uint32_t o[4];
                 float gx[4], gy[4], gz[4];
 #pragma unroll
-                for (uint32_t j = 0; j < 4u; j++) o[j] = static_cast<uint32_t>(ent[i + j]) << 2;
-#pragma unroll
-                for (uint32_t j = 0; j < 4u; j++) { gx[j] = plane(s_gx, o[j]); gy[j] = plane(s_gy, o[j]); gz[j] = plane(s_gz, o[j]); }
+                for (uint32_t j = 0; j < 4u; j++) { gx[j] = s_gx[i + j]; gy[j] = s_gy[i + j]; gz[j] = s_gz[i + j]; }
 #pragma unroll
                 for (uint32_t j = 0; j < 4u; j++) { acc.x += gx[j]; acc.y += gy[j]; acc.z += gz[j]; }
             }
-            for (; i < last; i++) {
-                const uint32_t o = static_cast<uint32_t>(ent[i]) << 2;
-                acc.x += plane(s_gx, o); acc.y += plane(s_gy, o); acc.z += plane(s_gz, o);
-            }
+            for (; i < last; i++) { acc.x += s_gx[i]; acc.y += s_gy[i]; acc.z += s_gz[i]; }
             acc.w = __uint_as_float(epoch + s);
             if constexpr (kLocal) store_plain(pbuf[s & 1u], v0 + tid, acc);
             else store_wt(pbuf[s & 1u], v0 + tid, acc);
diff --git a/tetsim_amd/csrc/tetsim_create.hip b/tetsim_amd/csrc/tetsim_create.hip
--- a/tetsim_amd/csrc/tetsim_create.hip
+++ b/tetsim_amd/csrc/tetsim_create.hip
@@ -180,18 +180,20 @@
         k.lean = (o.flags & TETSIM_FLAG_CONSTANT_REST_SHAPE) != 0;
         k.lean_state = lean_state;
         k.rot_exit_w2 = d.rot_exit_w2;
-        uint32_t *bto, *bvo, *lcr, *vpe;
+        uint32_t *bto, *bvo, *lcr = nullptr, *vpe, *trow = nullptr;
         int32_t* bv;
-        uchar4* lidx;
-        float* vol;
-        uint2* lce;
+        uchar4* lidx = nullptr;
+        float* vol = nullptr;
+        uint2* lce = nullptr;
+        uint16_t* lcf = nullptr;
         const size_t nslots = B.blk_verts.size();
         if ((rc = dev_alloc(h, &bto, B.blk_tet_off.size()))) return rc;
         if ((rc = dev_alloc(h, &bvo, B.blk_vert_off.size()))) return rc;
         if ((rc = dev_alloc(h, &bv, nslots))) return rc;
         if (ntl >= kStoreWtMaxIndex || nslots >= kStoreWtMaxIndex || nvl >= kStoreWtMaxIndex)
             return fail(h, TETSIM_EINVAL, "body too large for one handle (2^27 tets / particles / partial sums: 32-bit store offsets, dev_store.h); partition it");
-        if ((rc = dev_alloc(h, &lidx, ntl))) return rc;
+        if (quad && (rc = dev_alloc(h, &lidx, ntl))) return rc;
+        if (!quad && (rc = dev_alloc(h, &trow, 3ull * ntl))) return rc;
         if ((rc = dev_alloc(h, &k.rest_a, ntl))) return rc;
         if ((rc = dev_alloc(h, &k.rest_b, ntl))) return rc;
         if (lean_state) {
@@ -200,16 +202,18 @@
             if ((rc = dev_alloc(h, &h->rest0_b, ntl))) return rc;
             if ((rc = dev_alloc(h, &h->rest0_c, ntl))) return rc;
         } else if ((rc = dev_alloc(h, &k.rest_c, ntl))) return rc;
-        if ((rc = dev_alloc(h, &vol, ntl))) return rc;
+        if (quad && (rc = dev_alloc(h, &vol, ntl))) return rc;
         if ((rc = dev_alloc(h, &k.quat, ntl))) return rc;
-        if ((rc = dev_alloc(h, &lcr, nslots))) return rc;
-        if ((rc = dev_alloc(h, &lce, ntl))) return rc;
+        if (quad && (rc = dev_alloc(h, &lcr, nslots))) return rc;
+        if (quad && (rc = dev_alloc(h, &lce, ntl))) return rc;
+        if (!quad && (rc = dev_alloc(h, &lcf, B.lc_first.size()))) return rc;
         if ((rc = dev_alloc(h, &k.partial, nslots))) return rc;
         if ((rc = dev_alloc(h, &vpe, B.vp_ell.size()))) return rc;
         std::vector<float4> ra(ntl), rb(ntl), rcv(ntl), quat(ntl, make_float4(0, 0, 0, 1));
         std::vector<float> volh(ntl);
         std::vector<uchar4> lidxh(ntl);
         std::vector<uint2> lceh(ntl);
+        std::vector<uint32_t> trowh(3ull * ntl);
         for (uint32_t i = 0; i < ntl; i++) {
             const uint32_t lt = static_cast<uint32_t>(B.tet_perm[i]);
             const int32_t* c = &ltets[4 * lt];
@@ -228,6 +232,8 @@
             lidxh[i] = make_uchar4(B.tet_lidx[4ull * i], B.tet_lidx[4ull * i + 1], B.tet_lidx[4ull * i + 2], B.tet_lidx[4ull * i + 3]);
             const uint16_t* en = &B.lc_ent[4ull * i];
             lceh[i] = make_uint2(en[0] | (static_cast<uint32_t>(en[1]) << 16), en[2] | (static_cast<uint32_t>(en[3]) << 16));
+            trowh[3ull * i] = B.tet_pos[2ull * i]; trowh[3ull * i + 1] = B.tet_pos[2ull * i + 1];
+            memcpy(&trowh[3ull * i + 2], &volh[i], sizeof(float));
         }
         std::vector<float> wsum(std::max<size_t>(B.nv_pad, 1), 0.0f);
         {
@@ -347,7 +353,8 @@
         if ((rc = upload(h, bto, B.blk_tet_off))) return rc;
         if ((rc = upload(h, bvo, B.blk_vert_off))) return rc;
         if ((rc = upload(h, bv, B.blk_verts))) return rc;
-        if ((rc = upload(h, lidx, lidxh))) return rc;
+        if (quad && (rc = upload(h, lidx, lidxh))) return rc;
+        if (!quad && (rc = upload(h, trow, trowh))) return rc;
         if ((rc = upload(h, k.rest_a, ra))) return rc;
         if ((rc = upload(h, k.rest_b, rb))) return rc;
         if (lean_state) {
@@ -358,13 +365,15 @@
             if ((rc = upload(h, h->rest0_b, rb))) return rc;
             if ((rc = upload(h, h->rest0_c, rcv))) return rc;
         } else if ((rc = upload(h, k.rest_c, rcv))) return rc;
-        if ((rc = upload(h, vol, volh))) return rc;
+        if (quad && (rc = upload(h, vol, volh))) return rc;
         if ((rc = upload(h, k.quat, quat))) return rc;
-        if ((rc = upload(h, lcr, B.lc_range))) return rc;
-        if ((rc = upload(h, lce, lceh))) return rc;
+        if (quad && (rc = upload(h, lcr, B.lc_range))) return rc;
+        if (quad && (rc = upload(h, lce, lceh))) return rc;
+        if (!quad && (rc = upload(h, lcf, B.lc_first))) return rc;
         if ((rc = upload(h, vpe, B.vp_ell))) return rc;
         HIPCHK(h, hipMemset(k.partial, 0, std::max<size_t>(nslots, 1) * sizeof(float4)));
         k.blk_tet_off = bto; k.blk_vert_off = bvo; k.blk_verts = bv; k.tet_lidx = lidx; k.vol = vol;
+        k.tet_row = reinterpret_cast<const PJTetRow*>(trow); k.lc_first = lcf;
         k.lc_range = lcr; k.lc_ent = lce; k.vp_ell = vpe; k.vp_cols = B.vp_cols; k.nv_pad = B.nv_pad;
         d.quat = k.quat;
 #ifdef TETSIM_ABLATION
diff --git a/tetsim_amd/csrc/tetsim_host.cpp b/tetsim_amd/csrc/tetsim_host.cpp
--- a/tetsim_amd/csrc/tetsim_host.cpp
+++ b/tetsim_amd/csrc/tetsim_host.cpp
@@ -131,6 +131,27 @@
     if (tile_tets) std::copy(B.tet_perm.begin(), B.tet_perm.end(), tile_tets);
     if (tile_off) std::copy(B.blk_tet_off.begin(), B.blk_tet_off.end(), tile_off);
     if (corner_slot) std::copy(B.tet_lidx.begin(), B.tet_lidx.end(), corner_slot);
+    return 0;
+}
+int tetsim_prep_tile_tables(const float* verts, uint32_t nv, const int32_t* tets, uint32_t nt, int32_t ref_table, uint32_t sizes[2], int32_t* tile_tets,
+                            uint32_t* tile_off, uint32_t* slot_off, int32_t* slot_particle, uint8_t* corner_slot, uint16_t* entries, uint32_t* ranges,
+                            uint32_t* tet_pos, uint16_t* run_first) {
+    if (!sizes) return TETSIM_EINVAL;
+    std::string e = validate_mesh(verts, nv, tets, nt, false);
+    if (!e.empty()) return fail(nullptr, TETSIM_EINVAL, e);
+    const Incidence inc = build_incidence(tets, nt, nv, ref_table != 0, ref_table != 0);
+    BlockPlan B;
+    build_blocks(verts, tets, nt, nv, nv, inc, &B);
+    sizes[0] = B.num_blocks; sizes[1] = static_cast<uint32_t>(B.blk_verts.size());
+    if (tile_tets) std::copy(B.tet_perm.begin(), B.tet_perm.end(), tile_tets);
+    if (tile_off) std::copy(B.blk_tet_off.begin(), B.blk_tet_off.end(), tile_off);
+    if (slot_off) std::copy(B.blk_vert_off.begin(), B.blk_vert_off.end(), slot_off);
+    if (slot_particle) std::copy(B.blk_verts.begin(), B.blk_verts.end(), slot_particle);
+    if (corner_slot) std::copy(B.tet_lidx.begin(), B.tet_lidx.end(), corner_slot);
+    if (entries) std::copy(B.lc_ent.begin(), B.lc_ent.end(), entries);
+    if (ranges) std::copy(B.lc_range.begin(), B.lc_range.end(), ranges);
+    if (tet_pos) std::copy(B.tet_pos.begin(), B.tet_pos.end(), tet_pos);
+    if (run_first) std::copy(B.lc_first.begin(), B.lc_first.end(), run_first);
     return 0;
 }
 int tetsim_prep_slot_table(const int32_t* tets, uint32_t nt, uint32_t nv, int32_t ref_quirk, int32_t* slots, uint32_t* dropped) {
```

New measurement: 35980 M tet-solves/s (median of 6 runs). 1.02x the previous value.
